# soasme/LTX-Video-GPUPoor

Measured on AMD Instinct MI355X. Metric: denoise-steps/sec + VAE-decode frames/sec, LTX-Video 768x512x97f at 1/8 GPU, higher is better.
Workload: dtype bf16

## Files before the change

### include/ltxmi.h

```cpp
#ifndef LTXMI_H
#define LTXMI_H

#include <stddef.h>
#include <stdint.h>

#ifdef __cplusplus
extern "C" {
#endif

typedef enum ltxmi_status {
    LTXMI_OK = 0,
    LTXMI_ERR_INVALID_ARG = -1,
    LTXMI_ERR_UNSUPPORTED = -2,
    LTXMI_ERR_LAUNCH = -3
} ltxmi_status;

const char* ltxmi_version(void);
const char* ltxmi_last_error(void);
const char* ltxmi_arch(void);

typedef enum ltxmi_epilogue {
    LTXMI_EPI_NONE = 0,
    LTXMI_EPI_GELU_TANH = 1,
    LTXMI_EPI_SILU = 2,
    LTXMI_EPI_GATE_RESIDUAL = 3
} ltxmi_epilogue;

typedef struct ltxmi_gemm_args {
    const void* A;  int64_t lda;
    const void* W;  int64_t ldw;
    const void* bias;
    void*       C;  int64_t ldc;
    int32_t M, N, K;
    int32_t epilogue;
    const void* residual; int64_t ldr;
    const void* gate_table;
    const void* gate_temb;
    int64_t     gate_ld;
    int32_t     rows_per_group;
    int32_t     algo;
    float*      rowsumsq; int32_t rowsumsq_cols; int64_t rowsumsq_ld;
    int32_t     a_kblock; int64_t a_kblock_stride;
} ltxmi_gemm_args;

int ltxmi_gemm_bf16(const ltxmi_gemm_args* args, void* stream);

typedef enum ltxmi_norm_kind { LTXMI_NORM_RMS = 0, LTXMI_NORM_LAYER = 1 } ltxmi_norm_kind;

int ltxmi_norm_modulate_bf16(const void* x, int64_t ldx, void* y, int64_t ldy,
                             int32_t rows, int32_t D, float eps, int32_t kind,
                             const void* scale_table, const void* scale_temb,
                             const void* shift_table, const void* shift_temb,
                             int64_t temb_ld, int32_t rows_per_group, void* stream);

int ltxmi_rmsnorm_rope_bf16(void* x, int64_t ldx, int32_t rows, int32_t D,
                            const void* weight, float eps,
                            const void* cos_tab, const void* sin_tab, int64_t ld_tab,
                            int32_t rope_period, void* stream);
int ltxmi_rmsnorm_rope_rstd_bf16(void* x, int64_t ldx, int32_t rows, int32_t D, const void* weight, float eps,
                                 const void* cos_tab, const void* sin_tab, int64_t ld_tab, int32_t rope_period,
                                 const float* rowsumsq, int64_t rowsumsq_ld, int32_t rowsumsq_blocks,
                                 int32_t norm_dim, float norm_eps, float* rstd_out, void* stream);

typedef struct ltxmi_attn_args {
    const void* q; int64_t q_stride_b, q_stride_l;
    const void* k; int64_t k_stride_b, k_stride_l;
    const void* v; int64_t v_stride_b, v_stride_l;
    void*       o; int64_t o_stride_b, o_stride_l;
    const float* key_bias; int64_t bias_stride_b;
    int32_t B, H, Lq, Lk, head_dim;
    float   softmax_scale;
    const float* q_rowsumsq; int64_t q_rowsumsq_stride_b, q_rowsumsq_stride_l; int32_t q_rowsumsq_blocks;
    const void*  q_norm_weight; float q_norm_eps;
    const void*  rope_cos; const void* rope_sin; int64_t rope_stride_b, rope_stride_l;
    int32_t o_segment_len; int64_t o_stride_segment;
    const float* q_rstd; int64_t q_rstd_stride_b, q_rstd_stride_l;
    uint32_t* redo_counter; int32_t force_exact;
    float* lse; int64_t lse_stride_b, lse_stride_h;
} ltxmi_attn_args;

int ltxmi_attention_fwd_bf16(const ltxmi_attn_args* args, void* stream);
int ltxmi_attention_fuses_qnorm(int32_t B, int32_t H, int32_t Lq, int32_t Lk, int32_t head_dim, int32_t has_key_bias);
int ltxmi_attention_kernel_id(int32_t B, int32_t H, int32_t Lq, int32_t Lk, int32_t head_dim, int32_t has_key_bias,
                              int64_t k_stride_l, int64_t v_stride_l);

#define LTXMI_ATTN_MERGE_MAX 8
typedef struct ltxmi_attn_merge_args {
    int32_t n;
    const void*  o_part[LTXMI_ATTN_MERGE_MAX];   int64_t o_part_stride_b[LTXMI_ATTN_MERGE_MAX], o_part_stride_l[LTXMI_ATTN_MERGE_MAX];
    const float* lse_part[LTXMI_ATTN_MERGE_MAX]; int64_t lse_part_stride_b[LTXMI_ATTN_MERGE_MAX], lse_part_stride_h[LTXMI_ATTN_MERGE_MAX];
    void*  o;   int64_t o_stride_b, o_stride_l;
    float* lse; int64_t lse_stride_b, lse_stride_h;
    int32_t B, H, Lq, head_dim;
} ltxmi_attn_merge_args;
int ltxmi_attention_merge_bf16(const ltxmi_attn_merge_args* args, void* stream);

int ltxmi_rowsumsq_rstd_f32(const float* rowsumsq, int64_t rowsumsq_ld, int32_t rowsumsq_blocks, int32_t rows,
                            int32_t norm_dim, float norm_eps, float* rstd_out, void* stream);

int ltxmi_qkv_norm_rope_pack_bf16(const void* qkv, int64_t ld, int32_t B, int32_t Nl, int32_t D, int32_t P,
                                  const void* q_weight, const void* k_weight, float eps, const void* cos_tab,
                                  const void* sin_tab, int64_t ld_tab, int32_t rope_period, void* out, void* stream);

int ltxmi_silu_bf16(const void* x, void* y, int64_t n, void* stream);
int ltxmi_timestep_embedding_bf16(const float* t, void* out, int32_t n, int32_t dim, void* stream);
int ltxmi_stg_blend_bf16(void* a, int64_t lda, const void* v, int64_t ldv,
                         const float* m, int32_t B, int32_t L, int32_t D, void* stream);
int ltxmi_stg_blend_grouped_bf16(void* a, const void* v, int64_t v_stride_g, int64_t v_stride_b, int64_t v_stride_l,
                                 const float* m, int32_t G, int32_t B, int32_t L, int32_t D, void* stream);

typedef struct ltxmi_conv3d_args {
    const void* x; const void* w; const void* bias; void* y;
    int32_t B, T, H, W, Cin, Cout;
    int32_t causal;
    int32_t pad_replicate;
    int32_t d2s;
    const void* residual;
    int32_t res_channels;
    const void* add;
    int32_t stride_t, stride_hw;
    int32_t tpad, out_T;
    int32_t kernel_t, time_pad_zeros;
    int32_t algo;
    int32_t post_norm;
    const float* post_scale;
    const float* post_shift;
    float post_eps;
    void* y_norm;
    void* workspace; int64_t workspace_bytes;
} ltxmi_conv3d_args;

int ltxmi_conv3d_ndhwc_bf16(const ltxmi_conv3d_args* args, void* stream);
int ltxmi_conv3d_fuses_post_norm(const ltxmi_conv3d_args* args);
int64_t ltxmi_conv3d_workspace_bytes(const ltxmi_conv3d_args* args);

int ltxmi_pixelnorm_ada_silu_bf16(const void* x, void* y, int64_t rows, int32_t C,
                                  int64_t rows_per_batch, const float* scale, const float* shift,
                                  int32_t apply_silu, float eps, void* stream);

int ltxmi_add_bf16(const void* a, const void* b, void* y, int64_t n, void* stream);

int ltxmi_layernorm_affine_bf16(const void* x, void* y, int64_t rows, int32_t C,
                                const void* gamma, const void* beta, float eps, void* stream);

int ltxmi_ncdhw_to_ndhwc_bf16(const void* z, void* y, int32_t B, int32_t C, int32_t T, int32_t H,
                              int32_t W, const float* std, const float* mean, void* stream);
int ltxmi_unpatchify_to_ncdhw_bf16(const void* x, void* y, int32_t B, int32_t T, int32_t H, int32_t W,
                                   int32_t C_out, int32_t patch, void* stream);

int ltxmi_patchify_to_ndhwc_bf16(const void* x, void* y, int32_t B, int32_t C, int32_t T, int32_t H,
                                 int32_t W, int32_t patch, int32_t C_pad, void* stream);
int ltxmi_space_to_depth_skip_bf16(const void* conv, const void* x, void* out, int32_t B, int32_t T,
                                   int32_t H, int32_t W, int32_t Cin, int32_t Cconv, int32_t stride_t,
                                   int32_t stride_hw, int32_t group, void* stream);
int ltxmi_ndhwc_to_ncdhw_bf16(const void* x, int64_t ldx, int32_t c0, void* y, int32_t B, int32_t C,
                              int32_t T, int32_t H, int32_t W, const float* std, const float* mean,
                              void* stream);

#define LTXMI_GUIDANCE_WORKSPACE_FLOATS 2048
int ltxmi_guidance_step_bf16(const void* noise_pred, int64_t n, int32_t num_conds,
                             float guidance_scale, float stg_scale, float rescaling_scale,
                             int32_t do_cfg, int32_t do_stg, int32_t do_rescale,
                             void* latents, int32_t latents_bf16, float dt, float* workspace,
                             void* stream);

int ltxmi_guidance_step_masked_bf16(const void* noise_pred, int64_t n, int32_t num_conds,
                                    float guidance_scale, float stg_scale, float rescaling_scale,
                                    int32_t do_cfg, int32_t do_stg, int32_t do_rescale,
                                    void* latents, int32_t latents_bf16, float dt,
                                    const float* cond_mask, int32_t channels, float t,
                                    float* workspace, void* stream);

int ltxmi_image_cond_noise(void* latents, const void* init_latents, const void* noise, int32_t is_bf16,
                           const float* cond_mask, int64_t tokens, int32_t channels, float noise_scale,
                           float t, void* stream);

int ltxmi_groupnorm_silu_bf16(const void* x, void* y, const void* residual, int32_t samples, int64_t S,
                              int32_t C, int32_t groups, const void* gamma, const void* beta, float eps,
                              float* workspace, void* stream);
int ltxmi_pixel_shuffle2d_ndhwc_bf16(const void* x, void* y, int64_t frames, int32_t H, int32_t W, int32_t C,
                                     void* stream);
int ltxmi_tile_blend(const void* a, void* b, int32_t dtype, int64_t outer, int64_t len_a, int64_t len_b,
                     int64_t inner, int32_t extent, void* stream);
int ltxmi_adain_filter(const void* latents, const void* reference, void* out, int32_t is_bf16, int32_t planes,
                       int64_t n, int64_t n_ref, float factor, void* stream);

#ifdef __cplusplus
}
#endif
#endif
```

### ltx-video-gpupoor_amd/csrc/api.hip

```cpp
#include <stdarg.h>
#include <string.h>

#include "common.h"

namespace ltxmi {

static thread_local char g_err[512] = "";

void set_error(const char* fmt, ...) {
    va_list ap;
    va_start(ap, fmt);
    vsnprintf(g_err, sizeof(g_err), fmt, ap);
    va_end(ap);
}

int check_launch(const char* what) {
    const hipError_t e = hipGetLastError();
    if (e != hipSuccess) {
        set_error("%s: launch failed: %s", what, hipGetErrorString(e));
        return LTXMI_ERR_LAUNCH;
    }
    return LTXMI_OK;
}

int reserve_lds(const void* kernel, int bytes, unsigned long long* done, const char* what) {
    int dev = 0;
    if (hipGetDevice(&dev) != hipSuccess) {
        set_error("%s: cannot query the current device", what);
        return LTXMI_ERR_LAUNCH;
    }
    const bool tracked = dev >= 0 && dev < 64;
    const unsigned long long bit = tracked ? (1ull << dev) : 0ull;
    if (tracked && (__atomic_load_n(done, __ATOMIC_ACQUIRE) & bit)) return LTXMI_OK;
    const hipError_t e = hipFuncSetAttribute(kernel, hipFuncAttributeMaxDynamicSharedMemorySize, bytes);
    if (e != hipSuccess) {
        set_error("%s: cannot reserve %d bytes of LDS: %s", what, bytes, hipGetErrorString(e));
        return LTXMI_ERR_LAUNCH;
    }
    if (tracked) __atomic_fetch_or(done, bit, __ATOMIC_RELEASE);
    return LTXMI_OK;
}

int device_cu_count(const char* what) {
    static int cus[64] = {};
    int dev = 0;
    if (hipGetDevice(&dev) != hipSuccess) {
        set_error("%s: cannot query the current device", what);
        return -1;
    }
    const bool tracked = dev >= 0 && dev < 64;
    if (tracked) {
        const int c = __atomic_load_n(&cus[dev], __ATOMIC_ACQUIRE);
        if (c > 0) return c;
    }
    int n = 0;
    if (hipDeviceGetAttribute(&n, hipDeviceAttributeMultiprocessorCount, dev) != hipSuccess || n <= 0) {
        set_error("%s: cannot query the CU count of device %d", what, dev);
        return -1;
    }
    if (tracked) __atomic_store_n(&cus[dev], n, __ATOMIC_RELEASE);
    return n;
}

}

extern "C" const char* ltxmi_version(void) { return "ltxmi 0.6.0 (round 5)"; }
extern "C" const char* ltxmi_last_error(void) { return ltxmi::g_err; }
extern "C" const char* ltxmi_arch(void) { return "gfx950"; }
```

### ltx-video-gpupoor_amd/csrc/attention.h

```cpp
#pragma once
#include "common.h"

namespace ltxmi {

struct AttnParams {
    const uint16_t* q; int64_t q_sb, q_sl;
    const uint16_t* k; int64_t k_sb, k_sl;
    const uint16_t* v; int64_t v_sb, v_sl;
    uint16_t* o; int64_t o_sb, o_sl;
    const float* bias; int64_t bias_sb;
    int B, H, Lq, Lk;
    float scale_log2e;
    int q_tiles;
    const float* q_ss; int64_t q_ss_sb, q_ss_sl; int q_ss_n;
    const float* q_rstd; int64_t q_rstd_sb, q_rstd_sl;
    const uint16_t* q_w; float q_eps;
    const uint16_t* rope_cos; const uint16_t* rope_sin; int64_t rope_sb, rope_sl;
    int o_seg; int64_t o_sseg;
    uint32_t* redo_count; int force_exact;
    float* lse; int64_t lse_sb, lse_sh;

    __host__ __device__ __forceinline__ bool q_on_load() const { return q_ss != nullptr || q_rstd != nullptr; }
    __device__ __forceinline__ float q_row_rstd(int b, int row, int HD) const {
        if (q_rstd) return q_rstd[(int64_t)b * q_rstd_sb + (int64_t)row * q_rstd_sl];
        const float* ss = q_ss + (int64_t)b * q_ss_sb + (int64_t)row * q_ss_sl;
        float s2 = 0.f;
        if ((q_ss_n & 3) == 0 && (((uintptr_t)ss) & 15) == 0) {
            const f32x4* ss4 = (const f32x4*)ss;
            for (int j = 0; j < (q_ss_n >> 2); ++j) {
                const f32x4 v4 = ss4[j];
                s2 += (v4[0] + v4[1]) + (v4[2] + v4[3]);
            }
        } else {
            for (int j = 0; j < q_ss_n; ++j) s2 += ss[j];
        }
        return rsqrtf(s2 / (float)HD + q_eps);
    }

    __device__ __forceinline__ void store_lse(int b, int head, int row, float m_log2, float l, bool removed) const {
        constexpr float LN2 = 0.6931471805599453f;
        lse[(int64_t)b * lse_sb + (int64_t)head * lse_sh + row] = removed ? -INFINITY : (m_log2 + __log2f(l)) * LN2;
    }

    __device__ __forceinline__ int64_t o_row(int row) const {
        if (o_seg <= 0) return (int64_t)row * o_sl;
        const int sg = row / o_seg;
        return (int64_t)sg * o_sseg + (int64_t)(row - sg * o_seg) * o_sl;
    }
};

enum AttnKernel : int {
    ATTN_DH64 = 0, ATTN_DH64_BIAS = 1, ATTN_DH64_QB2 = 2, ATTN_PIPE = 3,
    ATTN_DH128 = 4, ATTN_DH128_BIAS = 5, ATTN_PIPE128 = 6, ATTN_CROSS = 7,
};
constexpr int ATTN_CROSS_MAX_KEYS = 256;
constexpr float ATTN_BIAS_FLOOR = -1e30f;
constexpr float ATTN_ROW_REMOVED = 0.99f * ATTN_BIAS_FLOOR;

int launch_attn_pipe(AttnParams p, hipStream_t stream);
int launch_attn_pipe128(AttnParams p, hipStream_t stream);
int launch_attn_cross(AttnParams p, hipStream_t stream);

}
```

### ltx-video-gpupoor_amd/csrc/attention.hip

```cpp
#include <type_traits>

#include "attention.h"

namespace ltxmi {

constexpr int KV_TILE = 64;
constexpr int Q_PER_WAVE = 32;
constexpr int Q_PER_WG = 128;
constexpr float LOG2E = 1.4426950408889634f;
constexpr int ATTN_QB_BIG = 2;

template <int DH>
struct AttnCfg {
    static constexpr int ROW_BYTES = DH * 2;
    static constexpr int TILE_BYTES = KV_TILE * DH * 2;
    static constexpr int CHUNKS_PER_ROW = DH / 8;
    static constexpr int LD_PER_THREAD = (KV_TILE * CHUNKS_PER_ROW) / 256;
    static constexpr int KSTEPS = DH / 16;
    static constexpr int DBLK = DH / 32;
    static constexpr int BIAS_BYTES = KV_TILE * 4;
    static constexpr int STAGE_BYTES = 2 * TILE_BYTES + BIAS_BYTES;
    static constexpr int SMEM = 2 * STAGE_BYTES;
    __device__ static __forceinline__ int k_swz(int row) {
        return DH == 64 ? ((row >> 1) & 7) : (row & 15);
    }
};


template <int DH, bool HAS_BIAS, int QB>
__global__ __launch_bounds__(256, (QB == 2 || DH == 128) ? 2 : 1) void attn_fwd_kernel(AttnParams p) {
    using C = AttnCfg<DH>;
    constexpr int QW = Q_PER_WAVE * QB;
    constexpr bool FOLD = !HAS_BIAS && DH == 128;
    extern __shared__ __attribute__((aligned(16))) char smem[];

    const int tid = threadIdx.x;
    const int lane = tid & 63;
    const int wave = __builtin_amdgcn_readfirstlane(tid >> 6);
    const int r = lane & 31;
    const int hh = lane >> 5;

    const int nwg = gridDim.x, orig = blockIdx.x;
    const int xcd = orig & 7, qn = nwg >> 3, rn = nwg & 7;
    const int work = (xcd < rn ? xcd * (qn + 1) : rn * (qn + 1) + (xcd - rn) * qn) + (orig >> 3);
    const int bh = work / p.q_tiles, qt = work % p.q_tiles;
    const int b = bh / p.H, head = bh % p.H;

    const uint16_t* qb = p.q + (int64_t)b * p.q_sb + head * DH;
    const uint16_t* kb_ = p.k + (int64_t)b * p.k_sb + head * DH;
    const uint16_t* vb = p.v + (int64_t)b * p.v_sb + head * DH;
    uint16_t* ob = p.o + (int64_t)b * p.o_sb + head * DH;
    const float* biasb = HAS_BIAS ? p.bias + (int64_t)b * p.bias_sb : nullptr;

    int q_row[QB];
    bf16x8 qf[QB][C::KSTEPS];
#pragma unroll
    for (int i = 0; i < QB; ++i) {
        q_row[i] = qt * (4 * QW) + wave * QW + 32 * i + r;
        const int q_ld = q_row[i] < p.Lq ? q_row[i] : p.Lq - 1;
        const float rstd = p.q_on_load() ? p.q_row_rstd(b, q_ld, p.H * DH) : 0.f;
#pragma unroll
        for (int s = 0; s < C::KSTEPS; ++s) {
            qf[i][s] = *(const bf16x8*)(qb + (int64_t)q_ld * p.q_sl + 16 * s + 8 * hh);
            if (p.q_on_load()) {
                const int col = head * DH + 16 * s + 8 * hh;
                const bf16x8 wv = *(const bf16x8*)(p.q_w + col);
                float o[8];
#pragma unroll
                for (int e = 0; e < 8; ++e) o[e] = (float)qf[i][s][e] * rstd * (float)wv[e];
                if (p.rope_cos) {
                    const int64_t trow = (int64_t)b * p.rope_sb + (int64_t)q_ld * p.rope_sl;
                    const bf16x8 cv = *(const bf16x8*)(p.rope_cos + trow + col), sv = *(const bf16x8*)(p.rope_sin + trow + col);
#pragma unroll
                    for (int e = 0; e < 8; e += 2) {
                        const float r0 = o[e] * (float)cv[e] - o[e + 1] * (float)sv[e];
                        const float r1 = o[e + 1] * (float)cv[e + 1] + o[e] * (float)sv[e + 1];
                        o[e] = r0;
                        o[e + 1] = r1;
                    }
                }
#pragma unroll
                for (int e = 0; e < 8; ++e) qf[i][s][e] = (__bf16)o[e];
            }
            if (FOLD) {
#pragma unroll
                for (int e = 0; e < 8; ++e) qf[i][s][e] = (__bf16)((float)qf[i][s][e] * p.scale_log2e);
            }
        }
    }

    int st_key[C::LD_PER_THREAD], st_koff[C::LD_PER_THREAD], st_voff[C::LD_PER_THREAD], st_col[C::LD_PER_THREAD];
#pragma unroll
    for (int i = 0; i < C::LD_PER_THREAD; ++i) {
        const int c = tid + 256 * i;
        const int key = c / C::CHUNKS_PER_ROW, dc = c % C::CHUNKS_PER_ROW;
        st_key[i] = key;
        st_col[i] = dc * 8;
        st_koff[i] = key * C::ROW_BYTES + ((dc ^ C::k_swz(key)) << 4);
        st_voff[i] = C::TILE_BYTES + ((key >> 3) * C::DBLK + (dc >> 2)) * 512 + (key & 7) * 64 + (dc & 3) * 16;
    }
    u32x4 kreg[C::LD_PER_THREAD], vreg[C::LD_PER_THREAD];
    float breg = 0.f;

    uint32_t k_goff[C::LD_PER_THREAD], v_goff[C::LD_PER_THREAD];
#pragma unroll
    for (int i = 0; i < C::LD_PER_THREAD; ++i) {
        k_goff[i] = (uint32_t)(((int64_t)st_key[i] * p.k_sl + st_col[i]) * 2);
        v_goff[i] = (uint32_t)(((int64_t)st_key[i] * p.v_sl + st_col[i]) * 2);
    }
    auto load_tile = [&](int k0, auto tail_tag) {
        constexpr bool TAIL = decltype(tail_tag)::value;
        if (!TAIL) {
            const char* kt = (const char*)(kb_ + (int64_t)k0 * p.k_sl);
            const char* vt = (const char*)(vb + (int64_t)k0 * p.v_sl);
#pragma unroll
            for (int i = 0; i < C::LD_PER_THREAD; ++i) {
                kreg[i] = *(const u32x4*)(kt + k_goff[i]);
                vreg[i] = *(const u32x4*)(vt + v_goff[i]);
            }
        } else {
#pragma unroll
            for (int i = 0; i < C::LD_PER_THREAD; ++i) {
                int key = k0 + st_key[i];
                key = key < p.Lk ? key : p.Lk - 1;
                kreg[i] = *(const u32x4*)(kb_ + (int64_t)key * p.k_sl + st_col[i]);
                vreg[i] = *(const u32x4*)(vb + (int64_t)key * p.v_sl + st_col[i]);
            }
        }
        if (HAS_BIAS && tid < KV_TILE) {
            const int key = k0 + tid;
            breg = key < p.Lk ? fmaxf(biasb[key] * LOG2E, ATTN_BIAS_FLOOR) : 0.f;
        }
    };
    auto write_tile = [&](int buf) {
        char* s = smem + buf * C::STAGE_BYTES;
#pragma unroll
        for (int i = 0; i < C::LD_PER_THREAD; ++i) {
            *(u32x4*)(s + st_koff[i]) = kreg[i];
            *(u32x4*)(s + st_voff[i]) = vreg[i];
        }
        if (HAS_BIAS && tid < KV_TILE) *(float*)(s + 2 * C::TILE_BYTES + tid * 4) = breg;
    };

    int k_rd[2];
#pragma unroll
    for (int kb = 0; kb < 2; ++kb) k_rd[kb] = (32 * kb + r) * C::ROW_BYTES;
    const int k_sw0 = C::k_swz(r);
    const int g16 = lane >> 4, i16 = lane & 15;
    const int v_rd = C::TILE_BYTES + (4 * (g16 >> 1) + (i16 >> 2)) * 64 + (16 * (g16 & 1) + 4 * (i16 & 3)) * 2;

    f32x16 oT[QB][C::DBLK];
    float m_run[QB];
    f32x4 lT[QB];
    bf16x8 ones;
    {
        const bool on = ((lane & 15) == 0 && ((lane >> 4) & 1) == 0) || ((lane & 15) == 1 && ((lane >> 4) & 1) == 1);
#pragma unroll
        for (int e = 0; e < 8; ++e) ones[e] = on ? (__bf16)1.0f : (__bf16)0.0f;
    }
    bf16x8 kaug, maug[QB];
#pragma unroll
    for (int e = 0; e < 8; ++e) kaug[e] = (hh == 0 && e < 2) ? (__bf16)1.0f : (__bf16)0.0f;
#pragma unroll
    for (int i = 0; i < QB; ++i) {
        m_run[i] = FOLD ? 0.f : -INFINITY;
#pragma unroll
        for (int e = 0; e < 8; ++e) maug[i][e] = (__bf16)0.0f;
        lT[i] = f32x4{0.f, 0.f, 0.f, 0.f};
#pragma unroll
        for (int d = 0; d < C::DBLK; ++d)
#pragma unroll
            for (int e = 0; e < 16; ++e) oT[i][d][e] = 0.f;
    }
    const float c = p.scale_log2e;

    const int nt = (p.Lk + KV_TILE - 1) / KV_TILE;
    const int n_full = p.Lk / KV_TILE;

    auto tile_body = [&](int t, auto tail_tag) {
        constexpr bool TAIL = decltype(tail_tag)::value;
        const int cur = t & 1;
        const char* s = smem + cur * C::STAGE_BYTES;

        f32x16 sT[QB][2];
#pragma unroll
        for (int i = 0; i < QB; ++i)
#pragma unroll
            for (int kb = 0; kb < 2; ++kb) {
#pragma unroll
                for (int e = 0; e < 16; ++e) sT[i][kb][e] = 0.f;
                if (FOLD) sT[i][kb] = __builtin_amdgcn_mfma_f32_32x32x16_bf16(kaug, maug[i], sT[i][kb], 0, 0, 0);
#pragma unroll
                for (int ks = 0; ks < C::KSTEPS; ++ks) {
                    const bf16x8 kf = *(const bf16x8*)(s + k_rd[kb] + (((2 * ks + hh) ^ k_sw0) << 4));
                    sT[i][kb] = __builtin_amdgcn_mfma_f32_32x32x16_bf16(kf, qf[i][ks], sT[i][kb], 0, 0, 0);
                }
            }

#pragma unroll
// ... 20 lines not shown
                        if (key >= p.Lk) sT[i][kb][e] = -INFINITY;
                    }
            }
            float mt;
            {
                auto max3 = [](float a, float b, float c3) { return fmaxf(fmaxf(a, b), c3); };
                float l1[11];
#pragma unroll
                for (int g = 0; g < 5; ++g) {
                    l1[g] = max3(sT[i][0][3 * g], sT[i][0][3 * g + 1], sT[i][0][3 * g + 2]);
                    l1[5 + g] = max3(sT[i][1][3 * g], sT[i][1][3 * g + 1], sT[i][1][3 * g + 2]);
                }
                l1[10] = max3(sT[i][0][15], sT[i][1][15], l1[0]);
                const float a = max3(l1[1], l1[2], l1[3]), b2 = max3(l1[4], l1[5], l1[6]), c2 = max3(l1[7], l1[8], l1[9]);
                mt = fmaxf(max3(a, b2, c2), l1[10]);
            }
            {
                const auto sw = __builtin_amdgcn_permlane32_swap(__float_as_uint(mt), __float_as_uint(mt), false, false);
                mt = fmaxf(__uint_as_float(sw[0]), __uint_as_float(sw[1]));
            }
            float nmoff = 0.f;
            if (FOLD) {
                const bool first = (t == 0);
                if (first || __any(mt > 0.f)) {
                    asm volatile("; max-moved branch (kept a real branch: not if-converted)" ::: "memory");
                    const float dq = (first || mt > 0.f) ? ceilf(mt * 4.0f) * 0.25f : 0.f;
#pragma unroll
                    for (int kb = 0; kb < 2; ++kb)
#pragma unroll
                        for (int e = 0; e < 16; ++e) sT[i][kb][e] -= dq;
                    if (!first) {
                        const float alpha = fast_exp2(-dq);
                        lT[i][0] *= alpha;
                        lT[i][1] *= __shfl(alpha, (lane + 16) & 63, 64);
#pragma unroll
                        for (int d = 0; d < C::DBLK; ++d)
#pragma unroll
                            for (int e = 0; e < 16; ++e) oT[i][d][e] *= alpha;
                    }
                    m_run[i] += dq;
                    const float nm = -m_run[i];
                    const __bf16 mh = (__bf16)nm;
                    const __bf16 ml = (__bf16)(nm - (float)mh);
                    maug[i][0] = hh == 0 ? mh : (__bf16)0.0f;
                    maug[i][1] = hh == 0 ? ml : (__bf16)0.0f;
                }
            } else {
                const float m_new = fmaxf(m_run[i], mt);
                if (__any(m_new != m_run[i])) {
                    asm volatile("; rescale branch (kept a real branch: not if-converted)" ::: "memory");
                    const float alpha = HAS_BIAS ? fast_exp2(m_run[i] - m_new) : fast_exp2((m_run[i] - m_new) * c);
                    lT[i][0] *= alpha;
                    lT[i][1] *= __shfl(alpha, (lane + 16) & 63, 64);
#pragma unroll
                    for (int d = 0; d < C::DBLK; ++d)
#pragma unroll
                        for (int e = 0; e < 16; ++e) oT[i][d][e] *= alpha;
                    m_run[i] = m_new;
                }
                nmoff = HAS_BIAS ? -m_run[i] : -m_run[i] * c;
            }

            bf16x8 pf[4];
#pragma unroll
            for (int kb = 0; kb < 2; ++kb) {
#pragma unroll
                for (int e = 0; e < 16; ++e) {
                    sT[i][kb][e] = fast_exp2(FOLD ? sT[i][kb][e] : (HAS_BIAS ? sT[i][kb][e] + nmoff : __builtin_fmaf(sT[i][kb][e], c, nmoff)));
                }
#pragma unroll
                for (int h2 = 0; h2 < 2; ++h2)
#pragma unroll
                    for (int e = 0; e < 8; ++e) pf[2 * kb + h2][e] = (__bf16)sT[i][kb][8 * h2 + e];
            }

#pragma unroll
            for (int sp = 0; sp < 4; ++sp) {
                lT[i] = __builtin_amdgcn_mfma_f32_16x16x32_bf16(ones, pf[sp], lT[i], 0, 0, 0);
#pragma unroll
                for (int d = 0; d < C::DBLK; ++d) {
                    const char* base = s + v_rd + (2 * sp * C::DBLK + d) * 512;
                    const s16x4 lo = __builtin_amdgcn_ds_read_tr16_b64_v4i16(
                        (__attribute__((address_space(3))) s16x4*)(base));
                    const s16x4 hi = __builtin_amdgcn_ds_read_tr16_b64_v4i16(
                        (__attribute__((address_space(3))) s16x4*)(base + C::DBLK * 512));
                    typedef __attribute__((ext_vector_type(8))) short s16x8;
                    const s16x8 both = __builtin_shufflevector(lo, hi, 0, 1, 2, 3, 4, 5, 6, 7);
                    const bf16x8 vf = __builtin_bit_cast(bf16x8, both);
                    oT[i][d] = __builtin_amdgcn_mfma_f32_32x32x16_bf16(vf, pf[sp], oT[i][d], 0, 0, 0);
                }
            }
        }
    };

    using no_tail = std::integral_constant<bool, false>;
    using with_tail = std::integral_constant<bool, true>;
    if (n_full > 0) load_tile(0, no_tail{}); else load_tile(0, with_tail{});
    write_tile(0);
    __syncthreads();

    for (int t = 0; t < n_full; ++t) {
        const bool has_next = t + 1 < nt;
        if (has_next) {
            if (t + 1 < n_full) load_tile((t + 1) * KV_TILE, no_tail{});
            else load_tile((t + 1) * KV_TILE, with_tail{});
        }
        tile_body(t, no_tail{});
        if (has_next) write_tile((t & 1) ^ 1);
        __syncthreads();
    }
    if (n_full < nt) tile_body(n_full, with_tail{});

#pragma unroll
    for (int i = 0; i < QB; ++i) {
        const float l0 = __shfl(lT[i][0], r & 15, 64), l1 = __shfl(lT[i][1], r & 15, 64);
        const float l = (r & 16) ? l1 : l0;
        const float inv = 1.0f / l;
        if (p.lse != nullptr) {
            const float m2 = (HAS_BIAS || FOLD) ? m_run[i] : m_run[i] * c;
            if (hh == 0 && q_row[i] < p.Lq) p.store_lse(b, head, q_row[i], m2, l, HAS_BIAS && m_run[i] <= ATTN_ROW_REMOVED);
        }
        char* scr = smem + wave * (32 * C::ROW_BYTES);
        if (i == 0) __syncthreads();
#pragma unroll
        for (int d = 0; d < C::DBLK; ++d)
#pragma unroll
            for (int g = 0; g < 4; ++g) {
                u32x2 w;
                w[0] = pack_bf16(oT[i][d][4 * g + 0] * inv, oT[i][d][4 * g + 1] * inv);
                w[1] = pack_bf16(oT[i][d][4 * g + 2] * inv, oT[i][d][4 * g + 3] * inv);
                const int chunk = 4 * d + g;
                *(u32x2*)(scr + r * C::ROW_BYTES + ((chunk ^ (r & 7)) << 4) + hh * 8) = w;
            }
        constexpr int LPR = C::CHUNKS_PER_ROW;
        constexpr int RPI = 64 / LPR;
        const int q0 = qt * (4 * QW) + wave * QW + 32 * i;
#pragma unroll
        for (int t = 0; t < 32 / RPI; ++t) {
            const int row = t * RPI + lane / LPR, chunk = lane % LPR;
            const u32x4 w = *(const u32x4*)(scr + row * C::ROW_BYTES + ((chunk ^ (row & 7)) << 4));
            if (q0 + row < p.Lq) *(u32x4*)(ob + p.o_row(q0 + row) + chunk * 8) = w;
        }
    }
}

template <int DH, bool HAS_BIAS, int QB>
static int launch(AttnParams p, hipStream_t stream) {
    using C = AttnCfg<DH>;
    auto kern = attn_fwd_kernel<DH, HAS_BIAS, QB>;
    static unsigned long long lds_done = 0;
    if (const int rc = reserve_lds((const void*)kern, C::SMEM, &lds_done, "ltxmi_attention_fwd_bf16")) return rc;
    const int q_per_wg = Q_PER_WG * QB;
    p.q_tiles = (p.Lq + q_per_wg - 1) / q_per_wg;
    const int64_t grid = (int64_t)p.B * p.H * p.q_tiles;
    hipLaunchKernelGGL(kern, dim3((unsigned)grid), dim3(256), C::SMEM, stream, p);
    return check_launch("ltxmi_attention_fwd_bf16");
}

static AttnKernel attn_select(int B, int H, int Lq, int Lk, int head_dim, bool has_bias, int64_t k_sl, int64_t v_sl) {
    const int64_t wg256 = (int64_t)B * H * ((Lq + 255) / 256);
    const int64_t rows = (int64_t)Lk + 4 * 64;
    const bool span_ok = (rows * k_sl + head_dim) * 2 < (1ll << 31) && (rows * v_sl + head_dim) * 2 < (1ll << 31);
    if (head_dim == 128) {
        if (!has_bias && wg256 >= 128 && Lk >= 1024 && span_ok) return ATTN_PIPE128;
        return has_bias ? ATTN_DH128_BIAS : ATTN_DH128;
    }
    if (Lk <= ATTN_CROSS_MAX_KEYS && Lq >= 1024) return ATTN_CROSS;
    if (!has_bias && wg256 >= 192 && span_ok) return ATTN_PIPE;
    if (!has_bias && wg256 >= 512) return ATTN_DH64_QB2;
    return has_bias ? ATTN_DH64_BIAS : ATTN_DH64;
}

}

using namespace ltxmi;

extern "C" int ltxmi_attention_fwd_bf16(const ltxmi_attn_args* a, void* stream) {
    LTXMI_REQUIRE(a && a->q && a->k && a->v && a->o, LTXMI_ERR_INVALID_ARG, "ltxmi_attention_fwd_bf16: NULL argument");
    LTXMI_REQUIRE(a->B > 0 && a->H > 0 && a->Lq > 0 && a->Lk > 0, LTXMI_ERR_INVALID_ARG,
                  "ltxmi_attention_fwd_bf16: non-positive shape B=%d H=%d Lq=%d Lk=%d", a->B, a->H, a->Lq, a->Lk);
    LTXMI_REQUIRE(a->head_dim == 64 || a->head_dim == 128, LTXMI_ERR_UNSUPPORTED,
                  "ltxmi_attention_fwd_bf16: head_dim %d not in {64, 128}", a->head_dim);
    const int64_t strides[] = {a->q_stride_b, a->q_stride_l, a->k_stride_b, a->k_stride_l,
                               a->v_stride_b, a->v_stride_l, a->o_stride_b, a->o_stride_l};
    for (int64_t s : strides)
        LTXMI_REQUIRE(s % 8 == 0, LTXMI_ERR_UNSUPPORTED, "ltxmi_attention_fwd_bf16: strides must be multiples of 8 elements");
    LTXMI_REQUIRE((((uintptr_t)a->q | (uintptr_t)a->k | (uintptr_t)a->v | (uintptr_t)a->o) & 15) == 0,
                  LTXMI_ERR_UNSUPPORTED, "ltxmi_attention_fwd_bf16: q/k/v/o must be 16-byte aligned");
    LTXMI_REQUIRE((int64_t)a->B * a->H * ((a->Lq + Q_PER_WG - 1) / Q_PER_WG) < (1ll << 31), LTXMI_ERR_UNSUPPORTED,
                  "ltxmi_attention_fwd_bf16: grid too large");
    AttnParams p;
    p.q = (const uint16_t*)a->q; p.q_sb = a->q_stride_b; p.q_sl = a->q_stride_l;
    p.k = (const uint16_t*)a->k; p.k_sb = a->k_stride_b; p.k_sl = a->k_stride_l;
    p.v = (const uint16_t*)a->v; p.v_sb = a->v_stride_b; p.v_sl = a->v_stride_l;
    p.o = (uint16_t*)a->o; p.o_sb = a->o_stride_b; p.o_sl = a->o_stride_l;
    p.bias = a->key_bias; p.bias_sb = a->bias_stride_b;
    p.B = a->B; p.H = a->H; p.Lq = a->Lq; p.Lk = a->Lk;
    p.scale_log2e = a->softmax_scale * LOG2E;
    p.q_tiles = (a->Lq + Q_PER_WG - 1) / Q_PER_WG;
    p.q_ss = a->q_rowsumsq; p.q_ss_sb = a->q_rowsumsq_stride_b; p.q_ss_sl = a->q_rowsumsq_stride_l;
    p.q_ss_n = a->q_rowsumsq_blocks;
    p.q_rstd = a->q_rstd; p.q_rstd_sb = a->q_rstd_stride_b; p.q_rstd_sl = a->q_rstd_stride_l;
    p.q_w = (const uint16_t*)a->q_norm_weight; p.q_eps = a->q_norm_eps;
    p.rope_cos = (const uint16_t*)a->rope_cos; p.rope_sin = (const uint16_t*)a->rope_sin;
    p.rope_sb = a->rope_stride_b; p.rope_sl = a->rope_stride_l;
    p.o_seg = a->o_segment_len; p.o_sseg = a->o_stride_segment;
    p.redo_count = a->redo_counter; p.force_exact = a->force_exact != 0;
    LTXMI_REQUIRE(a->o_segment_len >= 0 && a->o_stride_segment % 8 == 0, LTXMI_ERR_INVALID_ARG,
                  "ltxmi_attention_fwd_bf16: bad output segment geometry");
    p.lse = a->lse; p.lse_sb = a->lse_stride_b; p.lse_sh = a->lse_stride_h;
    if (a->lse)
        LTXMI_REQUIRE((((uintptr_t)a->lse) & 3) == 0 && a->lse_stride_h >= a->Lq &&
                          (a->B == 1 ? a->lse_stride_b >= 0 : a->lse_stride_b >= (int64_t)a->H * a->lse_stride_h),
                      LTXMI_ERR_INVALID_ARG,
                      "ltxmi_attention_fwd_bf16: lse must be 4-byte aligned with lse_stride_h >= Lq and lse_stride_b >= H * lse_stride_h");
    if (a->q_rowsumsq || a->q_rstd) {
        LTXMI_REQUIRE(a->q_norm_weight && (((uintptr_t)a->q_norm_weight) & 15) == 0 &&
                          (a->q_rstd ? (((uintptr_t)a->q_rstd) & 3) == 0
                                     : (a->q_rowsumsq_blocks == a->H * a->head_dim / 64 && (((uintptr_t)a->q_rowsumsq) & 3) == 0)),
                      LTXMI_ERR_INVALID_ARG, "ltxmi_attention_fwd_bf16: bad q_rowsumsq / q_rstd / q_norm_weight geometry");
        LTXMI_REQUIRE((a->rope_cos == nullptr) == (a->rope_sin == nullptr), LTXMI_ERR_INVALID_ARG,
                      "ltxmi_attention_fwd_bf16: rope_cos and rope_sin must both be given or both be NULL");
        if (a->rope_cos)
            LTXMI_REQUIRE((((uintptr_t)a->rope_cos | (uintptr_t)a->rope_sin) & 15) == 0 && a->rope_stride_l % 8 == 0 &&
                              a->rope_stride_b % 8 == 0,
                          LTXMI_ERR_INVALID_ARG, "ltxmi_attention_fwd_bf16: RoPE tables must be 16-byte aligned rows");
    }
    hipStream_t s = (hipStream_t)stream;
    switch (attn_select(a->B, a->H, a->Lq, a->Lk, a->head_dim, a->key_bias != nullptr, a->k_stride_l, a->v_stride_l)) {
        case ATTN_DH64: return launch<64, false, 1>(p, s);
        case ATTN_DH64_BIAS: return launch<64, true, 1>(p, s);
        case ATTN_DH64_QB2: return launch<64, false, ATTN_QB_BIG>(p, s);
        case ATTN_PIPE: return launch_attn_pipe(p, s);
        case ATTN_DH128: return launch<128, false, 1>(p, s);
        case ATTN_DH128_BIAS: return launch<128, true, 1>(p, s);
        case ATTN_PIPE128: return launch_attn_pipe128(p, s);
        case ATTN_CROSS: return launch_attn_cross(p, s);
    }
}

extern "C" int ltxmi_attention_kernel_id(int32_t B, int32_t H, int32_t Lq, int32_t Lk, int32_t head_dim, int32_t has_key_bias,
                                         int64_t k_stride_l, int64_t v_stride_l) {
    if (B <= 0 || H <= 0 || Lq <= 0 || Lk <= 0 || k_stride_l <= 0 || v_stride_l <= 0) return -1;
    if (head_dim != 64 && head_dim != 128) return -1;
    return attn_select(B, H, Lq, Lk, head_dim, has_key_bias != 0, k_stride_l, v_stride_l);
}

extern "C" int ltxmi_attention_fuses_qnorm(int32_t B, int32_t H, int32_t Lq, int32_t Lk, int32_t head_dim, int32_t has_key_bias) {
    return (B > 0 && H > 0 && Lq > 0 && Lk > 0 && (head_dim == 64 || head_dim == 128) && (H * head_dim) % 64 == 0) ? 1 : 0;
}
```

### ltx-video-gpupoor_amd/csrc/attention_cross.hip

```cpp
#include <type_traits>

#include "attention.h"

namespace ltxmi {

namespace cross {

#ifndef LTXMI_XATTN_STAGGER
#define LTXMI_XATTN_STAGGER 32
#endif

constexpr int DH = 64;
constexpr int KV_TILE = 64;
constexpr int MAX_TILES = 4;
constexpr int ROW_BYTES = DH * 2;
constexpr int TILE_BYTES = KV_TILE * DH * 2;
constexpr int K_OFF = 0, V_OFF = MAX_TILES * TILE_BYTES, BIAS_OFF = 2 * MAX_TILES * TILE_BYTES;
constexpr int SCR_OFF = BIAS_OFF + MAX_TILES * KV_TILE * 16;
constexpr int SCR_BYTES = 32 * 64;
constexpr int QW_OFF = SCR_OFF + 4 * SCR_BYTES;
constexpr int SMEM = QW_OFF + DH * 2;
constexpr int ROWS_PER_IT = 128;
constexpr float LOG2E = 1.4426950408889634f;

__device__ __forceinline__ int k_swz(int row) { return (row >> 1) & 7; }

template <int NT>
__global__ __launch_bounds__(256, 2) void attn_cross_kernel(AttnParams p, int groups, int rows_per_group, int stagger_from) {
    extern __shared__ __attribute__((aligned(16))) char smem[];
    const int tid = threadIdx.x;
    const int lane = tid & 63;
    const int wave = __builtin_amdgcn_readfirstlane(tid >> 6);
    const int r = lane & 31, hh = lane >> 5;

    const int nwg = gridDim.x, orig = blockIdx.x;
    const int xcd = orig & 7, qn = nwg >> 3, rn = nwg & 7;
    const int work = (xcd < rn ? xcd * (qn + 1) : rn * (qn + 1) + (xcd - rn) * qn) + (orig >> 3);
    const int bh = work / groups, grp = work % groups;
    const int b = bh / p.H, head = bh % p.H;
    const int row_begin = grp * rows_per_group;
    const int row_end = min(p.Lq, row_begin + rows_per_group);
    if (row_begin >= row_end) return;
    const int n_it = (row_end - row_begin + ROWS_PER_IT - 1) / ROWS_PER_IT;

    const uint16_t* qb = p.q + (int64_t)b * p.q_sb + head * DH;
    const uint16_t* kb_ = p.k + (int64_t)b * p.k_sb + head * DH;
    const uint16_t* vb = p.v + (int64_t)b * p.v_sb + head * DH;
    uint16_t* ob = p.o + (int64_t)b * p.o_sb + head * DH;
    constexpr int nt = NT;

    {
        u32x4 kreg[NT][2], vreg[NT][2];
#pragma unroll
        for (int t = 0; t < NT; ++t) {
#pragma unroll
                for (int i = 0; i < 2; ++i) {
                    const int c = tid + 256 * i;
                    int key = t * KV_TILE + (c >> 3);
                    key = key < p.Lk ? key : p.Lk - 1;
                    kreg[t][i] = *(const u32x4*)(kb_ + (int64_t)key * p.k_sl + (c & 7) * 8);
                    vreg[t][i] = *(const u32x4*)(vb + (int64_t)key * p.v_sl + (c & 7) * 8);
                }
            }
        if (tid < MAX_TILES * KV_TILE) {
            float bv = ATTN_BIAS_FLOOR;
            if (tid < p.Lk) bv = p.bias ? fmaxf(p.bias[(int64_t)b * p.bias_sb + tid] * (LOG2E / p.scale_log2e), ATTN_BIAS_FLOOR) : 0.f;
            const __bf16 hi = (__bf16)bv;
            const __bf16 lo = (__bf16)(bv - (float)hi);
            u32x4 w = {0u, 0u, 0u, 0u};
            w[0] = (uint32_t)__builtin_bit_cast(uint16_t, hi) | ((uint32_t)__builtin_bit_cast(uint16_t, lo) << 16);
            *(u32x4*)(smem + BIAS_OFF + tid * 16) = w;
        }
#pragma unroll
        for (int t = 0; t < NT; ++t) {
#pragma unroll
                for (int i = 0; i < 2; ++i) {
                    const int c = tid + 256 * i;
                    const int key = c >> 3, dc = c & 7;
                    *(u32x4*)(smem + K_OFF + t * TILE_BYTES + key * ROW_BYTES + ((dc ^ k_swz(key)) << 4)) = kreg[t][i];
                    *(u32x4*)(smem + V_OFF + t * TILE_BYTES + ((key >> 3) * 2 + (dc >> 2)) * 512 + (key & 7) * 64 + (dc & 3) * 16) = vreg[t][i];
                }
            }
    }
    if (p.q_on_load() && tid < 8) *(u32x4*)(smem + QW_OFF + tid * 16) = *(const u32x4*)(p.q_w + head * DH + tid * 8);
    __syncthreads();

    const int k_rd0 = r * ROW_BYTES, k_rd1 = (32 + r) * ROW_BYTES;
    const int k_sw0 = k_swz(r);
    const int g16 = lane >> 4, i16 = lane & 15;
    const int v_rd = (4 * (g16 >> 1) + (i16 >> 2)) * 64 + (16 * (g16 & 1) + 4 * (i16 & 3)) * 2;
    bf16x8 ones;
    {
        const bool on = ((lane & 15) == 0 && ((lane >> 4) & 1) == 0) || ((lane & 15) == 1 && ((lane >> 4) & 1) == 1);
#pragma unroll
        for (int e = 0; e < 8; ++e) ones[e] = on ? (__bf16)1.0f : (__bf16)0.0f;
    }
    const float c = p.scale_log2e;
    char* scr = smem + SCR_OFF + wave * SCR_BYTES;

    bf16x8 qraw[4], qf[4];
    float q_rstd = 0.f;
    int q_ld = 0;
    auto load_q = [&](int it) {
        const int row = row_begin + it * ROWS_PER_IT + wave * 32 + r;
        q_ld = row < p.Lq ? row : p.Lq - 1;
#pragma unroll
        for (int s = 0; s < 4; ++s) qraw[s] = *(const bf16x8*)(qb + (int64_t)q_ld * p.q_sl + 16 * s + 8 * hh);
        if (p.q_on_load()) q_rstd = p.q_row_rstd(b, q_ld, p.H * DH);
    };
    auto finish_q = [&]() {
        if (p.q_on_load()) {
            const int64_t trow = (int64_t)b * p.rope_sb + (int64_t)q_ld * p.rope_sl;
#pragma unroll
            for (int s = 0; s < 4; ++s) {
                const bf16x8 wv = *(const bf16x8*)(smem + QW_OFF + (16 * s + 8 * hh) * 2);
                float o[8];
#pragma unroll
                for (int e = 0; e < 8; ++e) o[e] = (float)qraw[s][e] * q_rstd * (float)wv[e];
                if (p.rope_cos) {
                    const int col = head * DH + 16 * s + 8 * hh;
                    const bf16x8 cv = *(const bf16x8*)(p.rope_cos + trow + col), sv = *(const bf16x8*)(p.rope_sin + trow + col);
#pragma unroll
                    for (int e = 0; e < 8; e += 2) {
                        const float r0 = o[e] * (float)cv[e] - o[e + 1] * (float)sv[e];
                        const float r1 = o[e + 1] * (float)cv[e + 1] + o[e] * (float)sv[e + 1];
                        o[e] = r0;
                        o[e + 1] = r1;
                    }
                }
#pragma unroll
                for (int e = 0; e < 8; ++e) qf[s][e] = (__bf16)o[e];
            }
        } else {
#pragma unroll
            for (int s = 0; s < 4; ++s) qf[s] = qraw[s];
        }
    };
    load_q(0);
    finish_q();
    if (n_it > 1) load_q(1);
    if (blockIdx.x >= (unsigned)stagger_from) __builtin_amdgcn_s_sleep(LTXMI_XATTN_STAGGER);

    for (int it = 0; it < n_it; ++it) {
        const int q0 = row_begin + it * ROWS_PER_IT + wave * 32;

        constexpr int NG = 2 * NT;
        f32x16 sT[NG];
        bf16x8 kfr[5];
        bf16x8 qaug;
        {
            uint32_t w0 = hh == 0 ? 0x3f803f80u : 0u, w1 = 0u;
            asm volatile("" : "+v"(w0), "+v"(w1));
            const u32x4 w = {w0, w1, w1, w1};
            qaug = __builtin_bit_cast(bf16x8, w);
        }
        auto read_k1 = [&](int g, int j) {
            if (j == 0) {
                kfr[0] = *(const bf16x8*)(smem + BIAS_OFF + (32 * g + r) * 16);
            } else {
                const char* ks = smem + K_OFF + (g >> 1) * TILE_BYTES + ((g & 1) ? k_rd1 : k_rd0);
                kfr[j] = *(const bf16x8*)(ks + (((2 * (j - 1) + hh) ^ k_sw0) << 4));
            }
        };
        auto max3 = [](float a, float b2, float c3) { return fmaxf(fmaxf(a, b2), c3); };
        float mt = -INFINITY;
        auto group_max = [&](int g) {
            const f32x16& x = sT[g];
            const float a = max3(x[0], x[1], x[2]), b2 = max3(x[3], x[4], x[5]), c2 = max3(x[6], x[7], x[8]);
            const float d2 = max3(x[9], x[10], x[11]), e2 = max3(x[12], x[13], x[14]);
            mt = max3(max3(a, b2, c2), max3(d2, e2, x[15]), mt);
            asm volatile("" : "+v"(mt));
        };
#pragma unroll
        for (int j = 0; j < 5; ++j) read_k1(0, j);
#pragma unroll
        for (int g = 0; g < NG; ++g) {
#pragma unroll
            for (int j = 0; j < 5; ++j) {
                if (j == 0) {
                    const f32x16 z16 = {0.f, 0.f, 0.f, 0.f, 0.f, 0.f, 0.f, 0.f, 0.f, 0.f, 0.f, 0.f, 0.f, 0.f, 0.f, 0.f};
                    sT[g] = __builtin_amdgcn_mfma_f32_32x32x16_bf16(kfr[0], qaug, z16, 0, 0, 0);
                } else {
                    sT[g] = __builtin_amdgcn_mfma_f32_32x32x16_bf16(kfr[j], qf[j - 1], sT[g], 0, 0, 0);
                }
                if (g + 1 < NG) read_k1(g + 1, j);
                __builtin_amdgcn_sched_barrier(0);
            }
            if (g >= 1) group_max(g - 1);
        }
        if (it + 1 < n_it) finish_q();
        if (it + 2 < n_it) load_q(it + 2);
        group_max(NG - 1);
        {
            const auto sw = __builtin_amdgcn_permlane32_swap(__float_as_uint(mt), __float_as_uint(mt), false, false);
            mt = fmaxf(__uint_as_float(sw[0]), __uint_as_float(sw[1]));
        }
        const float nmc = -mt * c;

        f32x16 oT[2];
        f32x4 lT;
        const f32x16 z16 = {0.f, 0.f, 0.f, 0.f, 0.f, 0.f, 0.f, 0.f, 0.f, 0.f, 0.f, 0.f, 0.f, 0.f, 0.f, 0.f};
        const f32x4 z4 = {0.f, 0.f, 0.f, 0.f};
        typedef __attribute__((ext_vector_type(8))) short s16x8;
        auto read_v = [&](int t, int sp, bf16x8 (&dst)[2]) {
            const char* vs = smem + V_OFF + t * TILE_BYTES + v_rd;
#pragma unroll
            for (int d = 0; d < 2; ++d) {
                const char* base = vs + (2 * sp * 2 + d) * 512;
                const s16x4 lo = __builtin_amdgcn_ds_read_tr16_b64_v4i16((__attribute__((address_space(3))) s16x4*)(base));
                const s16x4 hi = __builtin_amdgcn_ds_read_tr16_b64_v4i16((__attribute__((address_space(3))) s16x4*)(base + 2 * 512));
                const s16x8 both = __builtin_shufflevector(lo, hi, 0, 1, 2, 3, 4, 5, 6, 7);
                dst[d] = __builtin_bit_cast(bf16x8, both);
            }
        };
        auto make_p = [&](int t, int sp2, bf16x8& dst) {
            const f32x16& x = sT[2 * t + (sp2 >> 1)];
            const f32x2 c2v = {c, c}, m2v = {nmc, nmc};
#pragma unroll
            for (int e = 0; e < 8; e += 2) {
                const f32x2 y = f32x2{x[8 * (sp2 & 1) + e], x[8 * (sp2 & 1) + e + 1]} * c2v + m2v;
                dst[e] = (__bf16)fast_exp2(y[0]);
                dst[e + 1] = (__bf16)fast_exp2(y[1]);
            }
            asm volatile("" : "+v"(dst));
        };
        bf16x8 pfr[2][4], vfr[2][2];
#pragma unroll
        for (int sp = 0; sp < 4; ++sp) make_p(0, sp, pfr[0][sp]);
        read_v(0, 0, vfr[0]);
#pragma unroll
        for (int t = 0; t < NT; ++t) {
#pragma unroll
            for (int sp = 0; sp < 4; ++sp) {
                const int st = 4 * t + sp;
                if (st + 1 < 4 * NT) read_v((st + 1) >> 2, (st + 1) & 3, vfr[(st + 1) & 1]);
                const bf16x8& pf = pfr[t & 1][sp];
                lT = __builtin_amdgcn_mfma_f32_16x16x32_bf16(ones, pf, st == 0 ? z4 : lT, 0, 0, 0);
                oT[0] = __builtin_amdgcn_mfma_f32_32x32x16_bf16(vfr[st & 1][0], pf, st == 0 ? z16 : oT[0], 0, 0, 0);
                oT[1] = __builtin_amdgcn_mfma_f32_32x32x16_bf16(vfr[st & 1][1], pf, st == 0 ? z16 : oT[1], 0, 0, 0);
                if (t + 1 < NT) make_p(t + 1, sp, pfr[(t + 1) & 1][sp]);
                __builtin_amdgcn_sched_barrier(0);
            }
        }

        const float l0 = __shfl(lT[0], r & 15, 64), l1v = __shfl(lT[1], r & 15, 64);
        const float lrow = (r & 16) ? l1v : l0;
        const float inv = 1.0f / lrow;
        if (p.lse != nullptr) {
            if (hh == 0 && q0 + r < row_end) p.store_lse(b, head, q0 + r, -nmc, lrow, -nmc / c <= ATTN_ROW_REMOVED);
        }
#pragma unroll
        for (int d = 0; d < 2; ++d) {
#pragma unroll
            for (int g = 0; g < 4; ++g) {
                u32x2 w;
                w[0] = pack_bf16(oT[d][4 * g + 0] * inv, oT[d][4 * g + 1] * inv);
                w[1] = pack_bf16(oT[d][4 * g + 2] * inv, oT[d][4 * g + 3] * inv);
                *(u32x2*)(scr + r * 64 + ((g ^ (r & 3)) << 4) + hh * 8) = w;
            }
#pragma unroll
            for (int t2 = 0; t2 < 2; ++t2) {
                const int row = t2 * 16 + (lane >> 2), chunk = lane & 3;
                const u32x4 w = *(const u32x4*)(scr + row * 64 + ((chunk ^ (row & 3)) << 4));
                if (q0 + row < row_end) *(u32x4*)(ob + p.o_row(q0 + row) + 32 * d + chunk * 8) = w;
            }
        }
    }
}

}

static_assert(cross::MAX_TILES * cross::KV_TILE == ATTN_CROSS_MAX_KEYS, "attn_select hands this kernel up to ATTN_CROSS_MAX_KEYS keys");

int launch_attn_cross(AttnParams p, hipStream_t stream) {
    const int n_cu = device_cu_count("ltxmi_attention_fwd_bf16");
    if (n_cu <= 0) return LTXMI_ERR_LAUNCH;
    const int slots = 2 * n_cu, bh = p.B * p.H;
    int groups = slots / bh;
    if (groups < 1) groups = 1;
    const int max_groups = (p.Lq + 2 * cross::ROWS_PER_IT - 1) / (2 * cross::ROWS_PER_IT);
    if (groups > max_groups) groups = max_groups;
    int rows = (p.Lq + groups - 1) / groups;
    rows = (rows + cross::ROWS_PER_IT - 1) / cross::ROWS_PER_IT * cross::ROWS_PER_IT;
    groups = (p.Lq + rows - 1) / rows;
    const int64_t grid = (int64_t)bh * groups;
    const int nt = (p.Lk + cross::KV_TILE - 1) / cross::KV_TILE;
#define LTXMI_XATTN_LAUNCH(N)                                                                                              \
    {                                                                                                                      \
        static unsigned long long lds_done = 0;                                                                            \
        if (const int rc = reserve_lds((const void*)cross::attn_cross_kernel<N>, cross::SMEM, &lds_done,                   \
                                       "ltxmi_attention_fwd_bf16"))                                                        \
            return rc;                                                                                                     \
        hipLaunchKernelGGL(cross::attn_cross_kernel<N>, dim3((unsigned)grid), dim3(256), cross::SMEM, stream, p, groups,   \
                           rows, n_cu);                                                                                    \
    }
    switch (nt) {
        case 1: LTXMI_XATTN_LAUNCH(1) break;
        case 2: LTXMI_XATTN_LAUNCH(2) break;
        case 3: LTXMI_XATTN_LAUNCH(3) break;
        default: LTXMI_XATTN_LAUNCH(4) break;
    }
#undef LTXMI_XATTN_LAUNCH
    return check_launch("ltxmi_attention_fwd_bf16");
}

}
```

### ltx-video-gpupoor_amd/csrc/attention_pipe.hip

```cpp
#include <type_traits>

#include "attention.h"

namespace ltxmi {

namespace pipe {

#ifdef LTXMI_ATTN_STAMPS
#define STAMP(i)                                                                               \
    do {                                                                                       \
        unsigned long long t_;                                                                 \
        __builtin_amdgcn_sched_barrier(0);                                                     \
        asm volatile("s_memtime %0\n\ts_waitcnt lgkmcnt(0)" : "=s"(t_)::"memory");             \
        __builtin_amdgcn_sched_barrier(0);                                                     \
        st.acc[i] += t_ - st.prev;                                                             \
        st.prev = t_;                                                                          \
    } while (0)
struct Stamps { unsigned long long prev; unsigned long long acc[8]; };
__device__ unsigned long long* g_attn_stamps = nullptr;
#else
#define STAMP(i) do { } while (0)
struct Stamps {};
#endif

constexpr int DH = 64;
constexpr int KV_TILE = 64;
constexpr int ROW_BYTES = DH * 2;
constexpr int TILE_BYTES = KV_TILE * DH * 2;
constexpr int RING = 4;
constexpr int SMEM = 2 * RING * TILE_BYTES;
constexpr int Q_PER_WG = 256;

struct Blk {
    f32x16 s[2];
    f32x16 o[2];
    u32x4 pf[4];
    bf16x8 q[4];
    f32x4 l;
    float m;
};

struct Lane {
    int lane, r, hh;
    int k_rd[2];
    int k_sw0;
    int v_rd;
};

__device__ __forceinline__ bf16x8 k_fragment(const char* slot, const Lane& L, int j) {
    return *(const bf16x8*)(slot + L.k_rd[j >> 2] + (((2 * (j & 3) + L.hh) ^ L.k_sw0) << 4));
}

template <bool STEADY, bool QSCALED, typename Hook>
__device__ __forceinline__ void segment(Blk& X, Blk& Y, bf16x8 (&kf)[8], const char* ks_next, const char* vs, const Lane& L,
                                        const bf16x8& ones, float c, int key0, int Lk, Stamps& st, int st0, Hook&& hook) {
#pragma unroll
    for (int sp = 0; sp < 4; ++sp) Y.l = __builtin_amdgcn_mfma_f32_16x16x32_bf16(ones, __builtin_bit_cast(bf16x8, Y.pf[sp]), Y.l, 0, 0, 0);

    if (key0 + KV_TILE > Lk) {
        asm volatile("; ragged key tile (a wave-uniform branch, not a template instance)" ::: "memory");
#pragma unroll
        for (int kb = 0; kb < 2; ++kb)
#pragma unroll
            for (int e = 0; e < 16; ++e) {
                const int key = key0 + 32 * kb + (e & 3) + 8 * (e >> 2) + 4 * L.hh;
                if (key >= Lk) X.s[kb][e] = -INFINITY;
            }
    }
    if (!STEADY) {
        float mt;
        {
            auto max3 = [](float a, float b, float c3) { return fmaxf(fmaxf(a, b), c3); };
            float l1[11];
#pragma unroll
            for (int g = 0; g < 5; ++g) {
                l1[g] = max3(X.s[0][3 * g], X.s[0][3 * g + 1], X.s[0][3 * g + 2]);
                l1[5 + g] = max3(X.s[1][3 * g], X.s[1][3 * g + 1], X.s[1][3 * g + 2]);
            }
            l1[10] = max3(X.s[0][15], X.s[1][15], l1[0]);
            const float a = max3(l1[1], l1[2], l1[3]), b2 = max3(l1[4], l1[5], l1[6]), c2 = max3(l1[7], l1[8], l1[9]);
            mt = fmaxf(max3(a, b2, c2), l1[10]);
            const auto sw = __builtin_amdgcn_permlane32_swap(__float_as_uint(mt), __float_as_uint(mt), false, false);
            mt = fmaxf(__uint_as_float(sw[0]), __uint_as_float(sw[1]));
        }
        const float m_new = fmaxf(X.m, mt);
        if (__any(m_new != X.m)) {
            asm volatile("; rescale branch (kept a real branch: not if-converted)" ::: "memory");
            const float alpha = fast_exp2(QSCALED ? X.m - m_new : (X.m - m_new) * c);
            X.l[0] *= alpha;
            X.l[1] *= __shfl(alpha, (L.lane + 16) & 63, 64);
#pragma unroll
            for (int d = 0; d < 2; ++d)
#pragma unroll
                for (int e = 0; e < 16; ++e) X.o[d][e] *= alpha;
            X.m = m_new;
        }
    }
    const float nmoff = STEADY ? 0.f : QSCALED ? -X.m : -X.m * c;
    __builtin_amdgcn_sched_barrier(0);
    STAMP(st0);

    bf16x8 vf[8];
    float pp0 = 0.f, pp1 = 0.f;
    typedef __attribute__((ext_vector_type(8))) short s16x8;
#pragma unroll
    for (int j = 0; j < 16; ++j) {
        if (j < 8) {
            const int kb = j >> 2, s = j & 3;
            if (s == 0) {
#pragma unroll
                for (int e = 0; e < 16; ++e) Y.s[kb][e] = 0.f;
            }
            Y.s[kb] = __builtin_amdgcn_mfma_f32_32x32x16_bf16(kf[j], Y.q[s], Y.s[kb], 0, 0, 0);
            const char* base = vs + L.v_rd + (2 * (j >> 1) * 2 + (j & 1)) * 512;
            const s16x4 lo = __builtin_amdgcn_ds_read_tr16_b64_v4i16((__attribute__((address_space(3))) s16x4*)(base));
            const s16x4 hi = __builtin_amdgcn_ds_read_tr16_b64_v4i16((__attribute__((address_space(3))) s16x4*)(base + 2 * 512));
            const s16x8 both = __builtin_shufflevector(lo, hi, 0, 1, 2, 3, 4, 5, 6, 7);
            vf[j] = __builtin_bit_cast(bf16x8, both);
        } else {
            const int jj = j - 8, sp = jj >> 1, d = jj & 1;
            Y.o[d] = __builtin_amdgcn_mfma_f32_32x32x16_bf16(vf[jj], __builtin_bit_cast(bf16x8, Y.pf[sp]), Y.o[d], 0, 0, 0);
            kf[jj] = k_fragment(ks_next, L, jj);
        }
        hook(j);
        const int kb = j >> 3, e0 = 2 * (j & 7);
        auto bits = [&](float sc) { return QSCALED ? (STEADY ? sc : sc + nmoff) : (STEADY ? sc * c : __builtin_fmaf(sc, c, nmoff)); };
        const float p0 = fast_exp2(bits(X.s[kb][e0]));
        const float p1 = fast_exp2(bits(X.s[kb][e0 + 1]));
        if (j > 0) {
            const int jp = j - 1, kbp = jp >> 3, ep = 2 * (jp & 7);
            uint32_t pw = pack_bf16(pp0, pp1);
            asm volatile("" : "+v"(pw));
            X.pf[2 * kbp + (ep >> 3)][(ep & 7) >> 1] = pw;
        }
        pp0 = p0;
        pp1 = p1;
        __builtin_amdgcn_sched_barrier(0);
    }
    X.pf[3][3] = pack_bf16(pp0, pp1);
    STAMP(st0 + 1);
}

template <bool REDO, bool QSCALED>
__device__ __forceinline__ bool attn_pipe_item(const AttnParams& p, const int tid, char* smem) {
    char* kring = smem;
    char* vring = smem + RING * TILE_BYTES;

    Lane L;
    L.lane = tid & 63;
    const int wave = __builtin_amdgcn_readfirstlane(tid >> 6);
    L.r = L.lane & 31;
    L.hh = L.lane >> 5;

    const int nwg = gridDim.x, orig = blockIdx.x;
    const int xcd = orig & 7, qn = nwg >> 3, rn = nwg & 7;
    const int work = (xcd < rn ? xcd * (qn + 1) : rn * (qn + 1) + (xcd - rn) * qn) + (orig >> 3);
    const int bh = work / p.q_tiles, qt = work % p.q_tiles;
    const int b = bh / p.H, head = bh % p.H;

    const uint16_t* qb = p.q + (int64_t)b * p.q_sb + head * DH;
    const uint16_t* kb_ = p.k + (int64_t)b * p.k_sb + head * DH;
    const uint16_t* vb = p.v + (int64_t)b * p.v_sb + head * DH;
    uint16_t* ob = p.o + (int64_t)b * p.o_sb + head * DH;

    auto make_desc = [](const void* base, int64_t bytes) {
        const uint64_t a = (uint64_t)base;
        return u32x4{(uint32_t)a, (uint32_t)(a >> 32) & 0xffffu, (uint32_t)bytes, 0x00020000u};
    };
    const u32x4 k_desc = make_desc(kb_, ((int64_t)(p.Lk - 1) * p.k_sl + DH) * 2);
    const u32x4 v_desc = make_desc(vb, ((int64_t)(p.Lk - 1) * p.v_sl + DH) * 2);
    uint32_t k_voff[2], v_voff[2];
#pragma unroll
    for (int j = 0; j < 2; ++j) {
        const int piece = 2 * wave + j;
        const int krow = 8 * piece + (L.lane >> 3);
        const int kchunk = (L.lane & 7) ^ ((krow >> 1) & 7);
        k_voff[j] = (uint32_t)((krow * (int)p.k_sl + 8 * kchunk) * 2);
        const int vrow = 8 * piece + ((L.lane >> 2) & 7);
        const int vchunk = 4 * (L.lane >> 5) + (L.lane & 3);
        v_voff[j] = (uint32_t)((vrow * (int)p.v_sl + 8 * vchunk) * 2);
    }
    const uint32_t k_tile_step = (uint32_t)(KV_TILE * (int)p.k_sl * 2), v_tile_step = (uint32_t)(KV_TILE * (int)p.v_sl * 2);
    const uint32_t lds0 = (uint32_t)(uintptr_t)((__attribute__((address_space(3))) char*)smem);
    auto dma2 = [&](const u32x4& desc, uint32_t lds_addr, uint32_t voff0, uint32_t voff1) {
        uint32_t keep;
        asm volatile(
            "s_mov_b32 %0, m0\n\t"
            "s_mov_b32 m0, %3\n\t"
            "s_nop 0\n\t"
            "buffer_load_dwordx4 %1, %4, 0 offen lds\n\t"
            "s_add_u32 m0, m0, 0x400\n\t"
            "s_nop 0\n\t"
            "buffer_load_dwordx4 %2, %4, 0 offen lds\n\t"
            "s_mov_b32 m0, %0"
            : "=&s"(keep)
            : "v"(voff0), "v"(voff1), "s"(lds_addr), "s"(desc)
            : "memory", "scc");
    };
    auto dma1 = [&](const u32x4& desc, uint32_t lds_addr, uint32_t voff) {
        uint32_t keep;
        asm volatile(
            "s_mov_b32 %0, m0\n\t"
            "s_mov_b32 m0, %2\n\t"
            "s_nop 0\n\t"
            "buffer_load_dwordx4 %1, %3, 0 offen lds\n\t"
            "s_mov_b32 m0, %0"
            : "=&s"(keep)
            : "v"(voff), "s"(lds_addr), "s"(desc)
            : "memory");
    };
    auto dma_k1 = [&](int t, int i) {
        const uint32_t dst = lds0 + (uint32_t)((t & (RING - 1)) * TILE_BYTES + (2 * wave + i) * 1024);
        dma1(k_desc, dst, k_voff[i] + (uint32_t)t * k_tile_step);
    };
    auto dma_v1 = [&](int t, int i) {
        const uint32_t dst = lds0 + (uint32_t)((RING + (t & (RING - 1))) * TILE_BYTES + (2 * wave + i) * 1024);
        dma1(v_desc, dst, v_voff[i] + (uint32_t)t * v_tile_step);
    };
    auto dma_k = [&](int t) {
        const uint32_t dst = lds0 + (uint32_t)((t & (RING - 1)) * TILE_BYTES + 2 * wave * 1024);
        const uint32_t toff = (uint32_t)t * k_tile_step;
        dma2(k_desc, dst, k_voff[0] + toff, k_voff[1] + toff);
    };
    auto dma_v = [&](int t) {
        const uint32_t dst = lds0 + (uint32_t)((RING + (t & (RING - 1))) * TILE_BYTES + 2 * wave * 1024);
        const uint32_t toff = (uint32_t)t * v_tile_step;
        dma2(v_desc, dst, v_voff[0] + toff, v_voff[1] + toff);
    };

    const int nt = (p.Lk + KV_TILE - 1) / KV_TILE;

    L.k_rd[0] = L.r * ROW_BYTES;
    L.k_rd[1] = (32 + L.r) * ROW_BYTES;
    L.k_sw0 = (L.r >> 1) & 7;
    {
        const int g16 = L.lane >> 4, i16 = L.lane & 15;
        L.v_rd = (4 * (g16 >> 1) + (i16 >> 2)) * 64 + (16 * (g16 & 1) + 4 * (i16 & 3)) * 2;
    }

    Blk A, Bk;
    bf16x8 ones;
    {
        const bool on = ((L.lane & 15) == 0 && ((L.lane >> 4) & 1) == 0) || ((L.lane & 15) == 1 && ((L.lane >> 4) & 1) == 1);
#pragma unroll
        for (int e = 0; e < 8; ++e) ones[e] = on ? (__bf16)1.0f : (__bf16)0.0f;
    }
    const float c = p.scale_log2e;
    auto init = [&](Blk& X, int blk) {
        const int row = qt * Q_PER_WG + wave * 64 + 32 * blk + L.r;
        const int q_ld = row < p.Lq ? row : p.Lq - 1;
#pragma unroll
        for (int s = 0; s < 4; ++s) X.q[s] = *(const bf16x8*)(qb + (int64_t)q_ld * p.q_sl + 16 * s + 8 * L.hh);
        if (QSCALED) {
            const float rstd = p.q_row_rstd(b, q_ld, p.H * DH);
            const int64_t trow = (int64_t)b * p.rope_sb + (int64_t)q_ld * p.rope_sl;
#pragma unroll
            for (int s = 0; s < 4; ++s) {
                const int col = head * DH + 16 * s + 8 * L.hh;
                const bf16x8 wv = *(const bf16x8*)(p.q_w + col);
                float o[8];
#pragma unroll
                for (int e = 0; e < 8; ++e) o[e] = (float)X.q[s][e] * rstd * (float)wv[e];
                if (p.rope_cos) {
                    const bf16x8 cv = *(const bf16x8*)(p.rope_cos + trow + col), sv = *(const bf16x8*)(p.rope_sin + trow + col);
#pragma unroll
                    for (int e = 0; e < 8; e += 2) {
                        const float r0 = o[e] * (float)cv[e] - o[e + 1] * (float)sv[e];
                        const float r1 = o[e + 1] * (float)cv[e + 1] + o[e] * (float)sv[e + 1];
                        o[e] = r0;
                        o[e + 1] = r1;
                    }
                }
#pragma unroll
                for (int e = 0; e < 8; ++e) X.q[s][e] = (__bf16)(QSCALED ? o[e] * c : o[e]);
            }
        }
        X.m = -INFINITY;
        X.l = f32x4{0.f, 0.f, 0.f, 0.f};
#pragma unroll
        for (int i = 0; i < 4; ++i) X.pf[i] = u32x4{0u, 0u, 0u, 0u};
#pragma unroll
        for (int d = 0; d < 2; ++d)
#pragma unroll
            for (int e = 0; e < 16; ++e) { X.o[d][e] = 0.f; X.s[d][e] = 0.f; }
    };
    volatile int* redo_flag = (volatile int*)(smem + SMEM);
    if (!REDO && tid == 0) *redo_flag = 0;
    const bool wave_idle = qt * Q_PER_WG + wave * 64 >= p.Lq;
    if ((blockIdx.x >> 8) & 1) __builtin_amdgcn_s_setprio(1);
    Stamps st;
#ifdef LTXMI_ATTN_STAMPS
    unsigned long long rt0_ = 0;
#endif
    dma_k(0); dma_v(0); dma_k(1); dma_v(1); dma_k(2);
    init(A, 0);
    init(Bk, 1);
    {
        const u32x4 z = {0u, 0u, 0u, 0u};
        *(u32x4*)(vring + 3 * TILE_BYTES + tid * 32) = z;
        *(u32x4*)(vring + 3 * TILE_BYTES + tid * 32 + 16) = z;
    }
    __builtin_amdgcn_s_waitcnt(0x0070);
    __builtin_amdgcn_s_barrier();
    __builtin_amdgcn_sched_barrier(0);

#ifdef LTXMI_ATTN_STAMPS
    for (int i = 0; i < 8; ++i) st.acc[i] = 0;
    { unsigned long long t0_; asm volatile("s_memtime %0\n\ts_waitcnt lgkmcnt(0)" : "=s"(t0_)::"memory"); st.prev = t0_; }
    asm volatile("s_memrealtime %0\n\ts_waitcnt lgkmcnt(0)" : "=s"(rt0_)::"memory");
#endif
    const int t_exact = REDO ? nt : 0;
// ... 7 lines not shown
    } else {
        bf16x8 kf[8];
#pragma unroll
        for (int j = 0; j < 8; ++j) kf[j] = k_fragment(kring, L, j);
#pragma unroll
        for (int j = 0; j < 8; ++j) A.s[j >> 2] = __builtin_amdgcn_mfma_f32_32x32x16_bf16(kf[j], A.q[j & 3], A.s[j >> 2], 0, 0, 0);

        using exact_form = std::integral_constant<bool, false>;
        using steady_form = std::integral_constant<bool, true>;
        auto iteration = [&](int t, auto steady_tag) {
            constexpr bool STEADY = decltype(steady_tag)::value;
            __builtin_amdgcn_s_barrier();
            __builtin_amdgcn_sched_barrier(0);
            STAMP(0);
            STAMP(1);
            segment<STEADY, QSCALED>(A, Bk, kf, kring + ((t + 1) & 3) * TILE_BYTES, vring + ((t + 3) & 3) * TILE_BYTES, L, ones, c, t * KV_TILE, p.Lk, st, 2,
                          [&](int j) { if (j == 3) dma_k1(t + 3, 0); else if (j == 11) dma_k1(t + 3, 1); });
            segment<STEADY, QSCALED>(Bk, A, kf, kring + ((t + 1) & 3) * TILE_BYTES, vring + (t & 3) * TILE_BYTES, L, ones, c, t * KV_TILE, p.Lk, st, 4,
                          [&](int j) { if (j == 3) dma_v1(t + 2, 0); else if (j == 11) dma_v1(t + 2, 1); });
            asm volatile("s_waitcnt vmcnt(4)" ::: "memory");
            __builtin_amdgcn_sched_barrier(0);
            STAMP(6);
        };
        int t = 0;
        for (; t < t_exact; ++t) iteration(t, exact_form{});
        if (!REDO)
            for (; t < nt; ++t) iteration(t, steady_form{});
    }

#ifdef LTXMI_ATTN_STAMPS
    unsigned long long rt1_;
    asm volatile("s_memrealtime %0\n\ts_waitcnt lgkmcnt(0)" : "=s"(rt1_)::"memory");
    if (g_attn_stamps && L.lane == 0 && blockIdx.x < 4096 && !wave_idle) {
        for (int i = 0; i < 7; ++i) g_attn_stamps[(blockIdx.x * 4 + wave) * 8 + i] = st.acc[i];
        g_attn_stamps[(blockIdx.x * 4 + wave) * 8 + 7] = (unsigned long long)nt | ((rt1_ - rt0_) << 32);
    }
#endif
    if (!wave_idle) {
        const char* vs = vring + ((nt - 1) & 3) * TILE_BYTES;
#pragma unroll
        for (int sp = 0; sp < 4; ++sp) Bk.l = __builtin_amdgcn_mfma_f32_16x16x32_bf16(ones, __builtin_bit_cast(bf16x8, Bk.pf[sp]), Bk.l, 0, 0, 0);
        typedef __attribute__((ext_vector_type(8))) short s16x8;
#pragma unroll
        for (int sp = 0; sp < 4; ++sp)
#pragma unroll
            for (int d = 0; d < 2; ++d) {
                const char* base = vs + L.v_rd + (2 * sp * 2 + d) * 512;
                const s16x4 lo = __builtin_amdgcn_ds_read_tr16_b64_v4i16((__attribute__((address_space(3))) s16x4*)(base));
                const s16x4 hi = __builtin_amdgcn_ds_read_tr16_b64_v4i16((__attribute__((address_space(3))) s16x4*)(base + 2 * 512));
                const s16x8 both = __builtin_shufflevector(lo, hi, 0, 1, 2, 3, 4, 5, 6, 7);
                Bk.o[d] = __builtin_amdgcn_mfma_f32_32x32x16_bf16(__builtin_bit_cast(bf16x8, both), __builtin_bit_cast(bf16x8, Bk.pf[sp]), Bk.o[d], 0, 0, 0);
            }
    }
    asm volatile("s_waitcnt vmcnt(0) lgkmcnt(0)" ::: "memory");
    if (!REDO) {
    bool outgrown = false;
    if (t_exact < nt && !wave_idle) {
        constexpr uint32_t OUTGROWN_EXP = (127u + 100u) << 23, VANISHED_EXP = (127u - 100u) << 23;
        uint32_t worst = 0;
        auto scan = [&](const Blk& X) {
            worst |= (uint32_t)((__float_as_uint(X.l[0]) & 0x7f800000u) >= OUTGROWN_EXP);
            worst |= (uint32_t)((__float_as_uint(X.l[1]) & 0x7f800000u) >= OUTGROWN_EXP);
            if (L.lane < 16) {
                worst |= (uint32_t)((__float_as_uint(X.l[0]) & 0x7f800000u) < VANISHED_EXP);
                worst |= (uint32_t)((__float_as_uint(X.l[1]) & 0x7f800000u) < VANISHED_EXP);
            }
#pragma unroll
            for (int d = 0; d < 2; ++d)
#pragma unroll
                for (int e = 0; e < 16; ++e) worst |= (uint32_t)((__float_as_uint(X.o[d][e]) & 0x7f800000u) >= OUTGROWN_EXP);
        };
        scan(A);
        scan(Bk);
        outgrown = __any(worst != 0);
    }
    if (outgrown && L.lane == 0) *redo_flag = 1;
    __builtin_amdgcn_s_barrier();
    __builtin_amdgcn_sched_barrier(0);
    const int redo = *redo_flag;
    __builtin_amdgcn_s_barrier();
    if (redo != 0) return true;
    } else {
        __builtin_amdgcn_s_barrier();
        __builtin_amdgcn_sched_barrier(0);
    }

    auto store = [&](Blk& X, int blk) {
        const float l0 = __shfl(X.l[0], L.r & 15, 64), l1 = __shfl(X.l[1], L.r & 15, 64);
        const float lrow = (L.r & 16) ? l1 : l0;
        const float inv = 1.0f / lrow;
        if (p.lse != nullptr) {
            const int row = qt * Q_PER_WG + wave * 64 + 32 * blk + L.r;
            if (L.hh == 0 && row < p.Lq) p.store_lse(b, head, row, REDO ? (QSCALED ? X.m : X.m * c) : 0.f, lrow, false);
        }
        char* scr = smem + (wave * 2 + blk) * (32 * ROW_BYTES);
#pragma unroll
        for (int d = 0; d < 2; ++d)
#pragma unroll
            for (int g = 0; g < 4; ++g) {
                u32x2 w;
                w[0] = pack_bf16(X.o[d][4 * g + 0] * inv, X.o[d][4 * g + 1] * inv);
                w[1] = pack_bf16(X.o[d][4 * g + 2] * inv, X.o[d][4 * g + 3] * inv);
                const int chunk = 4 * d + g;
                *(u32x2*)(scr + L.r * ROW_BYTES + ((chunk ^ (L.r & 7)) << 4) + L.hh * 8) = w;
            }
        const int q0 = qt * Q_PER_WG + wave * 64 + 32 * blk;
#pragma unroll
        for (int t = 0; t < 4; ++t) {
            const int row = t * 8 + (L.lane >> 3), chunk = L.lane & 7;
            const u32x4 w = *(const u32x4*)(scr + row * ROW_BYTES + ((chunk ^ (row & 7)) << 4));
            if (q0 + row < p.Lq) *(u32x4*)(ob + p.o_row(q0 + row) + chunk * 8) = w;
        }
    };
    store(A, 0);
    store(Bk, 1);
    return false;
}

template <int OCC, bool QSCALED, bool FORCE_EXACT>
__global__ __launch_bounds__(256, OCC) void attn_pipe_kernel(AttnParams p) {
    extern __shared__ __attribute__((aligned(16))) char smem[];
    const int tid = threadIdx.x;
    if (FORCE_EXACT) {
        attn_pipe_item<true, QSCALED>(p, tid, smem);
        return;
    }
    if (!attn_pipe_item<false, QSCALED>(p, tid, smem)) return;
    int tid2 = tid;
    asm volatile("" : "+v"(tid2));
    if (p.redo_count != nullptr && tid2 == 0) atomicAdd(p.redo_count, 1u);
    attn_pipe_item<true, QSCALED>(p, tid2, smem);
}

}

#ifdef LTXMI_ATTN_STAMPS
extern "C" int ltxmi_debug_set_attn_stamps(void* buf) {
    unsigned long long* b = (unsigned long long*)buf;
    return (int)hipMemcpyToSymbol(HIP_SYMBOL(pipe::g_attn_stamps), &b, sizeof(b));
}
#endif

#ifndef LTXMI_ATTN_PIPE_OCC
#define LTXMI_ATTN_PIPE_OCC 2
#endif

int launch_attn_pipe(AttnParams p, hipStream_t stream) {
    const bool qscaled = p.q_on_load();
    auto kern = p.force_exact ? (qscaled ? pipe::attn_pipe_kernel<LTXMI_ATTN_PIPE_OCC, true, true> : pipe::attn_pipe_kernel<LTXMI_ATTN_PIPE_OCC, false, true>)
                              : (qscaled ? pipe::attn_pipe_kernel<LTXMI_ATTN_PIPE_OCC, true, false> : pipe::attn_pipe_kernel<LTXMI_ATTN_PIPE_OCC, false, false>);
    static unsigned long long lds_done[4] = {0, 0, 0, 0};
    if (const int rc = reserve_lds((const void*)kern, pipe::SMEM + 16, &lds_done[(p.force_exact ? 2 : 0) + qscaled], "ltxmi_attention_fwd_bf16")) return rc;
    p.q_tiles = (p.Lq + pipe::Q_PER_WG - 1) / pipe::Q_PER_WG;
    const int64_t grid = (int64_t)p.B * p.H * p.q_tiles;
    hipLaunchKernelGGL(kern, dim3((unsigned)grid), dim3(256), pipe::SMEM + 16, stream, p);
    return check_launch("ltxmi_attention_fwd_bf16");
}

}
```

### ltx-video-gpupoor_amd/csrc/attention_pipe128.hip

```cpp
#include <type_traits>

#include "attention.h"

namespace ltxmi {

namespace pipe128 {

constexpr int DH = 128;
constexpr int KV_TILE = 64;
constexpr int ROW_BYTES = DH * 2;
constexpr int TILE_BYTES = KV_TILE * DH * 2;
constexpr int RING = 4;
constexpr int SMEM = 2 * RING * TILE_BYTES;
constexpr int Q_PER_WG = 256;
constexpr int NS = DH / 16;
constexpr int ND = DH / 32;
constexpr int NCH = 2 * NS + 4 * ND;
constexpr int PIECES = TILE_BYTES / 1024 / 4;

struct Blk {
    f32x16 s[2];
    f32x16 o[ND];
    u32x4 pf[4];
    bf16x8 q[NS];
    f32x4 l;
    float m;
    float mt;
};

struct Lane {
    int lane, r, hh;
    int koff[8];
    int v_rd;
};

__device__ __forceinline__ bf16x8 kread(const char* slot, const Lane& L, int i) {
    return *(const bf16x8*)(slot + L.koff[i & 7] + (i >> 3) * (32 * ROW_BYTES));
}
__device__ __forceinline__ bf16x8 vread(const char* slot, const Lane& L, int i) {
    typedef __attribute__((ext_vector_type(8))) short s16x8;
    const char* base = slot + L.v_rd + ((2 * (i >> 2)) * 4 + (i & 3)) * 512;
    const s16x4 lo = __builtin_amdgcn_ds_read_tr16_b64_v4i16((__attribute__((address_space(3))) s16x4*)(base));
    const s16x4 hi = __builtin_amdgcn_ds_read_tr16_b64_v4i16((__attribute__((address_space(3))) s16x4*)(base + 4 * 512));
    const s16x8 both = __builtin_shufflevector(lo, hi, 0, 1, 2, 3, 4, 5, 6, 7);
    return __builtin_bit_cast(bf16x8, both);
}

__device__ __forceinline__ void mfma_s0(f32x16& acc, const bf16x8& k, const bf16x8& q) {
    asm("v_mfma_f32_32x32x16_bf16 %0, %1, %2, 0" : "=&v"(acc) : "v"(k), "a"(q));
}
__device__ __forceinline__ void mfma_s(f32x16& acc, const bf16x8& k, const bf16x8& q) {
    asm("v_mfma_f32_32x32x16_bf16 %0, %1, %2, %0" : "+v"(acc) : "v"(k), "a"(q));
}
__device__ __forceinline__ void mfma_o(f32x16& acc, const bf16x8& vt, const bf16x8& pt) {
    asm("v_mfma_f32_32x32x16_bf16 %0, %1, %2, %0" : "+a"(acc) : "v"(vt), "v"(pt));
}
template <int N>
__device__ __forceinline__ void settle_o(f32x16 (&o)[N]) {
    static_assert(N == 4, "four O^T blocks");
    asm volatile("s_nop 15\n\ts_nop 7" : "+a"(o[0]), "+a"(o[1]), "+a"(o[2]), "+a"(o[3]));
}
template <bool EXACT, typename Hook>
__device__ __forceinline__ void segment(Blk& X, Blk& Y, bf16x8 (&kq)[4], const char* ks_cur, const char* ks_next, const char* vs,
                                        const Lane& L, const bf16x8& ones, float c, int key0_y, int Lk, Hook&& hook) {
    if (EXACT) {
        const float m_new = fmaxf(X.m, X.mt);
        if (__any(m_new != X.m)) {
            asm volatile("; rescale branch (kept a real branch: not if-converted)" ::: "memory");
            const float alpha = fast_exp2((X.m - m_new) * c);
            X.l[0] *= alpha;
            X.l[1] *= __shfl(alpha, (L.lane + 16) & 63, 64);
            settle_o(X.o);
#pragma unroll
            for (int d = 0; d < ND; ++d)
#pragma unroll
                for (int e = 0; e < 16; ++e) X.o[d][e] *= alpha;
            X.m = m_new;
        }
    }
    const float nmoff = -X.m * c;
    __builtin_amdgcn_sched_barrier(0);

    bf16x8 f[NCH];
#pragma unroll
    for (int i = 0; i < 4; ++i) f[i] = kq[i];
    float pa = 0.f, pb = 0.f;
    float mt = -INFINITY;
#pragma unroll
    for (int j = 0; j < NCH; ++j) {
        if (j < 2 * NS) {
            const int kb = j / NS, s = j % NS;
            if (s == 0) mfma_s0(Y.s[kb], f[j], Y.q[s]);
            else mfma_s(Y.s[kb], f[j], Y.q[s]);
        } else {
            const int jj = j - 2 * NS, sp = jj / ND, d = jj % ND;
            mfma_o(Y.o[d], f[j], __builtin_bit_cast(bf16x8, Y.pf[sp]));
        }
        {
            const int cn = j + 4;
            if (cn < 2 * NS) f[cn] = kread(ks_cur, L, cn);
            else if (cn < NCH) f[cn] = vread(vs, L, cn - 2 * NS);
            else kq[cn - NCH] = kread(ks_next, L, cn - NCH);
        }
        if (j == 1) Y.l = __builtin_amdgcn_mfma_f32_16x16x32_bf16(ones, __builtin_bit_cast(bf16x8, Y.pf[3]), Y.l, 0, 0, 0);
        if (j == 9 || j == 17 || j == 25)
            X.l = __builtin_amdgcn_mfma_f32_16x16x32_bf16(ones, __builtin_bit_cast(bf16x8, X.pf[(j - 9) >> 3]), X.l, 0, 0, 0);
        hook(j);
        const float p = fast_exp2(__builtin_fmaf(X.s[j >> 4][j & 15], c, nmoff));
        if ((j & 1) == 0) {
            if (j >= 2) {
                const int jp = j / 2 - 1;
                uint32_t pw = pack_bf16(pa, pb);
                asm volatile("" : "+v"(pw));
                X.pf[2 * (jp >> 3) + ((jp & 7) >> 2)][jp & 3] = pw;
            }
            pa = p;
        } else {
            pb = p;
        }
        if (j >= 2 * NS) {
            const int jm = j - 2 * NS, kbm = jm >> 3, em = 2 * (jm & 7);
            if (em == 0 && key0_y + KV_TILE > Lk) {
                asm volatile("; ragged key tile (kept a real branch)" ::: "memory");
#pragma unroll
                for (int e = 0; e < 16; ++e) {
                    const int key = key0_y + 32 * kbm + (e & 3) + 8 * (e >> 2) + 4 * L.hh;
                    if (key >= Lk) Y.s[kbm][e] = -INFINITY;
                }
            }
            if (EXACT) {
                mt = fmaxf(fmaxf(mt, Y.s[kbm][em]), Y.s[kbm][em + 1]);
                asm volatile("" : "+v"(mt));
            }
        }
        __builtin_amdgcn_sched_barrier(0);
    }
    X.pf[3][3] = pack_bf16(pa, pb);
    if (EXACT) {
        const auto sw = __builtin_amdgcn_permlane32_swap(__float_as_uint(mt), __float_as_uint(mt), false, false);
        Y.mt = fmaxf(__uint_as_float(sw[0]), __uint_as_float(sw[1]));
    }
}

__global__ __launch_bounds__(256, 1) void attn_pipe128_kernel(AttnParams p) {
    extern __shared__ __attribute__((aligned(16))) char smem[];
    char* kring = smem;
    char* vring = smem + RING * TILE_BYTES;

    const int tid = threadIdx.x;
    Lane L;
    L.lane = tid & 63;
    const int wave = __builtin_amdgcn_readfirstlane(tid >> 6);
    L.r = L.lane & 31;
    L.hh = L.lane >> 5;

    const int nwg = gridDim.x, orig = blockIdx.x;
    const int xcd = orig & 7, qn = nwg >> 3, rn = nwg & 7;
    const int work = (xcd < rn ? xcd * (qn + 1) : rn * (qn + 1) + (xcd - rn) * qn) + (orig >> 3);
    const int bh = work / p.q_tiles, qt = work % p.q_tiles;
    const int b = bh / p.H, head = bh % p.H;

    const uint16_t* qb = p.q + (int64_t)b * p.q_sb + head * DH;
    const uint16_t* kb_ = p.k + (int64_t)b * p.k_sb + head * DH;
    const uint16_t* vb = p.v + (int64_t)b * p.v_sb + head * DH;
    uint16_t* ob = p.o + (int64_t)b * p.o_sb + head * DH;

    auto make_desc = [](const void* base, int64_t bytes) {
        const uint64_t a = (uint64_t)base;
        return u32x4{(uint32_t)a, (uint32_t)(a >> 32) & 0xffffu, (uint32_t)bytes, 0x00020000u};
    };
    const u32x4 k_desc = make_desc(kb_, ((int64_t)(p.Lk - 1) * p.k_sl + DH) * 2);
    const u32x4 v_desc = make_desc(vb, ((int64_t)(p.Lk - 1) * p.v_sl + DH) * 2);
    uint32_t k_voff[PIECES], v_voff[PIECES];
#pragma unroll
    for (int j = 0; j < PIECES; ++j) {
        const int piece = PIECES * wave + j;
        const int krow = 4 * piece + (L.lane >> 4);
        const int kchunk = (L.lane & 15) ^ (krow & 15);
        k_voff[j] = (uint32_t)((krow * (int)p.k_sl + 8 * kchunk) * 2);
        const int vrow = 8 * (piece >> 1) + ((L.lane >> 2) & 7);
        const int vchunk = 8 * (piece & 1) + 4 * (L.lane >> 5) + (L.lane & 3);
        v_voff[j] = (uint32_t)((vrow * (int)p.v_sl + 8 * vchunk) * 2);
    }
    const uint32_t k_tile_step = (uint32_t)(KV_TILE * (int)p.k_sl * 2), v_tile_step = (uint32_t)(KV_TILE * (int)p.v_sl * 2);
    const uint32_t lds0 = (uint32_t)(uintptr_t)((__attribute__((address_space(3))) char*)smem);
    auto dma1 = [&](const u32x4& desc, uint32_t lds_addr, uint32_t voff) {
        uint32_t keep;
        asm volatile(
            "s_mov_b32 %0, m0\n\t"
            "s_mov_b32 m0, %2\n\t"
            "s_nop 0\n\t"
            "buffer_load_dwordx4 %1, %3, 0 offen lds\n\t"
            "s_mov_b32 m0, %0"
            : "=&s"(keep)
            : "v"(voff), "s"(lds_addr), "s"(desc)
            : "memory");
    };
    auto dma_k1 = [&](int t, int i) {
        const uint32_t dst = lds0 + (uint32_t)((t & (RING - 1)) * TILE_BYTES + (PIECES * wave + i) * 1024);
        dma1(k_desc, dst, k_voff[i] + (uint32_t)t * k_tile_step);
    };
    auto dma_v1 = [&](int t, int i) {
        const uint32_t dst = lds0 + (uint32_t)((RING + (t & (RING - 1))) * TILE_BYTES + (PIECES * wave + i) * 1024);
        dma1(v_desc, dst, v_voff[i] + (uint32_t)t * v_tile_step);
    };
    auto dma_k = [&](int t) {
#pragma unroll
        for (int i = 0; i < PIECES; ++i) dma_k1(t, i);
    };
    auto dma_v = [&](int t) {
#pragma unroll
        for (int i = 0; i < PIECES; ++i) dma_v1(t, i);
    };

    const int nt = (p.Lk + KV_TILE - 1) / KV_TILE;
#pragma unroll
    for (int s8 = 0; s8 < 8; ++s8) L.koff[s8] = L.r * ROW_BYTES + (((2 * s8 + L.hh) ^ (L.r & 15)) << 4);
    {
        const int g16 = L.lane >> 4, i16 = L.lane & 15;
        L.v_rd = (4 * (g16 >> 1) + (i16 >> 2)) * 64 + (16 * (g16 & 1) + 4 * (i16 & 3)) * 2;
    }

    Blk A, Bk;
    bf16x8 ones;
    {
        const bool on = ((L.lane & 15) == 0 && ((L.lane >> 4) & 1) == 0) || ((L.lane & 15) == 1 && ((L.lane >> 4) & 1) == 1);
#pragma unroll
        for (int e = 0; e < 8; ++e) ones[e] = on ? (__bf16)1.0f : (__bf16)0.0f;
    }
    auto init = [&](Blk& X, int blk) {
        const int row = qt * Q_PER_WG + wave * 64 + 32 * blk + L.r;
        const int q_ld = row < p.Lq ? row : p.Lq - 1;
#pragma unroll
        for (int s = 0; s < NS; ++s) X.q[s] = *(const bf16x8*)(qb + (int64_t)q_ld * p.q_sl + 16 * s + 8 * L.hh);
        if (p.q_on_load()) {
            const float rstd = p.q_row_rstd(b, q_ld, p.H * DH);
            const int64_t trow = (int64_t)b * p.rope_sb + (int64_t)q_ld * p.rope_sl;
#pragma unroll
            for (int s = 0; s < NS; ++s) {
                const int col = head * DH + 16 * s + 8 * L.hh;
                const bf16x8 wv = *(const bf16x8*)(p.q_w + col);
                float o[8];
#pragma unroll
                for (int e = 0; e < 8; ++e) o[e] = (float)X.q[s][e] * rstd * (float)wv[e];
                if (p.rope_cos) {
                    const bf16x8 cv = *(const bf16x8*)(p.rope_cos + trow + col), sv = *(const bf16x8*)(p.rope_sin + trow + col);
#pragma unroll
                    for (int e = 0; e < 8; e += 2) {
                        const float r0 = o[e] * (float)cv[e] - o[e + 1] * (float)sv[e];
                        const float r1 = o[e + 1] * (float)cv[e + 1] + o[e] * (float)sv[e + 1];
                        o[e] = r0;
                        o[e + 1] = r1;
                    }
                }
#pragma unroll
                for (int e = 0; e < 8; ++e) X.q[s][e] = (__bf16)o[e];
            }
        }
        X.m = -INFINITY;
        X.mt = -INFINITY;
        X.l = f32x4{0.f, 0.f, 0.f, 0.f};
#pragma unroll
        for (int i = 0; i < 4; ++i) X.pf[i] = u32x4{0u, 0u, 0u, 0u};
#pragma unroll
        for (int d = 0; d < ND; ++d)
#pragma unroll
            for (int e = 0; e < 16; ++e) X.o[d][e] = 0.f;
#pragma unroll
        for (int kb = 0; kb < 2; ++kb)
#pragma unroll
            for (int e = 0; e < 16; ++e) X.s[kb][e] = 0.f;
    };
    const float c = p.scale_log2e;
    volatile int* redo_flag = (volatile int*)(smem + SMEM);
    if (tid == 0) *redo_flag = 0;
    for (int attempt = p.force_exact ? 1 : 0; attempt < 2; ++attempt) {
        if (attempt == 1 && !p.force_exact && p.redo_count != nullptr && tid == 0) atomicAdd(p.redo_count, 1u);
        dma_k(0); dma_v(0); dma_k(1); dma_v(1); dma_k(2);
        init(A, 0);
        init(Bk, 1);
#pragma unroll
        for (int s8 = 0; s8 < NS; ++s8) {
            asm volatile("" : "+a"(A.q[s8]));
            asm volatile("" : "+a"(Bk.q[s8]));
        }
        {
            const u32x4 z = {0u, 0u, 0u, 0u};
#pragma unroll
            for (int i = 0; i < TILE_BYTES / (256 * 16); ++i) *(u32x4*)(vring + 3 * TILE_BYTES + (i * 256 + tid) * 16) = z;
        }
        __builtin_amdgcn_s_waitcnt(0x0070);
        __builtin_amdgcn_s_barrier();
        __builtin_amdgcn_sched_barrier(0);

        bf16x8 kq[4];
#pragma unroll
        for (int j = 0; j < 2 * NS; ++j) {
            const bf16x8 kfj = kread(kring, L, j);
            if (j % NS == 0) mfma_s0(A.s[j / NS], kfj, A.q[j % NS]);
            else mfma_s(A.s[j / NS], kfj, A.q[j % NS]);
            if (j < 4) kq[j] = kfj;
        }
        {
            float mt = -INFINITY;
            asm volatile("s_nop 15\n\ts_nop 7" : "+v"(A.s[0]), "+v"(A.s[1]));
#pragma unroll
            for (int kb2 = 0; kb2 < 2; ++kb2)
#pragma unroll
                for (int e = 0; e < 16; ++e) {
                    if (p.Lk < KV_TILE) {
                        const int key = 32 * kb2 + (e & 3) + 8 * (e >> 2) + 4 * L.hh;
                        if (key >= p.Lk) A.s[kb2][e] = -INFINITY;
                    }
                    mt = fmaxf(mt, A.s[kb2][e]);
                }
            const auto sw = __builtin_amdgcn_permlane32_swap(__float_as_uint(mt), __float_as_uint(mt), false, false);
            A.mt = fmaxf(__uint_as_float(sw[0]), __uint_as_float(sw[1]));
        }

        auto iteration = [&](int t, auto exact_tag) __attribute__((always_inline)) {
            constexpr bool EXACT = decltype(exact_tag)::value;
            __builtin_amdgcn_s_barrier();
            __builtin_amdgcn_sched_barrier(0);
            const char* k_t = kring + (t & 3) * TILE_BYTES;
            const char* k_t1 = kring + ((t + 1) & 3) * TILE_BYTES;
            segment<EXACT>(A, Bk, kq, k_t, k_t1, vring + ((t + 3) & 3) * TILE_BYTES, L, ones, c, t * KV_TILE, p.Lk,
                           [&](int j) { if ((j & 7) == 3) dma_k1(t + 3, j >> 3); });
            segment<EXACT>(Bk, A, kq, k_t1, k_t1, vring + (t & 3) * TILE_BYTES, L, ones, c, (t + 1) * KV_TILE, p.Lk,
                           [&](int j) { if ((j & 7) == 3) dma_v1(t + 2, j >> 3); });
            asm volatile("s_waitcnt vmcnt(8)" ::: "memory");
            __builtin_amdgcn_sched_barrier(0);
        };
        const int t_exact = attempt == 0 ? (nt < 2 ? nt : 2) : nt;
        int t = 0;
        for (; t < t_exact; ++t) iteration(t, std::integral_constant<bool, true>{});
        for (; t < nt; ++t) iteration(t, std::integral_constant<bool, false>{});

        {
            const char* vs = vring + ((nt - 1) & 3) * TILE_BYTES;
            Bk.l = __builtin_amdgcn_mfma_f32_16x16x32_bf16(ones, __builtin_bit_cast(bf16x8, Bk.pf[3]), Bk.l, 0, 0, 0);
#pragma unroll
            for (int i = 0; i < 4 * ND; ++i) mfma_o(Bk.o[i % ND], vread(vs, L, i), __builtin_bit_cast(bf16x8, Bk.pf[i / ND]));
        }
        asm volatile("s_waitcnt vmcnt(0) lgkmcnt(0)" ::: "memory");
        bool outgrown = false;
        if (attempt == 0 && t_exact < nt) {
            constexpr uint32_t OUTGROWN_EXP = (127u + 100u) << 23;
            settle_o(A.o);
            settle_o(Bk.o);
            uint32_t worst = 0;
            auto scan = [&](const Blk& X) {
                worst |= (uint32_t)((__float_as_uint(X.l[0]) & 0x7f800000u) >= OUTGROWN_EXP);
                worst |= (uint32_t)((__float_as_uint(X.l[1]) & 0x7f800000u) >= OUTGROWN_EXP);
#pragma unroll
                for (int d = 0; d < ND; ++d)
#pragma unroll
                    for (int e = 0; e < 16; ++e) worst |= (uint32_t)((__float_as_uint(X.o[d][e]) & 0x7f800000u) >= OUTGROWN_EXP);
            };
            scan(A);
            scan(Bk);
            outgrown = __any(worst != 0);
        }
        if (outgrown && L.lane == 0) *redo_flag = 1;
        __builtin_amdgcn_s_barrier();
        __builtin_amdgcn_sched_barrier(0);
        const int redo = *redo_flag;
        __builtin_amdgcn_s_barrier();
        if (attempt == 1 || redo == 0) break;
    }


    auto store = [&](Blk& X, int blk) {
        settle_o(X.o);
        const float l0 = __shfl(X.l[0], L.r & 15, 64), l1 = __shfl(X.l[1], L.r & 15, 64);
        const float lrow = (L.r & 16) ? l1 : l0;
        const float inv = 1.0f / lrow;
        if (p.lse != nullptr) {
            const int row = qt * Q_PER_WG + wave * 64 + 32 * blk + L.r;
            if (L.hh == 0 && row < p.Lq) p.store_lse(b, head, row, X.m * c, lrow, false);
        }
        char* scr = smem + (wave * 2 + blk) * (32 * ROW_BYTES);
#pragma unroll
        for (int d = 0; d < ND; ++d)
#pragma unroll
            for (int g = 0; g < 4; ++g) {
                u32x2 w;
                w[0] = pack_bf16(X.o[d][4 * g + 0] * inv, X.o[d][4 * g + 1] * inv);
                w[1] = pack_bf16(X.o[d][4 * g + 2] * inv, X.o[d][4 * g + 3] * inv);
                const int chunk = 4 * d + g;
                *(u32x2*)(scr + L.r * ROW_BYTES + ((chunk ^ (L.r & 15)) << 4) + L.hh * 8) = w;
            }
        const int q0 = qt * Q_PER_WG + wave * 64 + 32 * blk;
#pragma unroll
        for (int t = 0; t < 8; ++t) {
            const int row = t * 4 + (L.lane >> 4), chunk = L.lane & 15;
            const u32x4 w = *(const u32x4*)(scr + row * ROW_BYTES + ((chunk ^ (row & 15)) << 4));
            if (q0 + row < p.Lq) *(u32x4*)(ob + p.o_row(q0 + row) + chunk * 8) = w;
        }
    };
    store(A, 0);
    store(Bk, 1);
}

}

int launch_attn_pipe128(AttnParams p, hipStream_t stream) {
    auto kern = pipe128::attn_pipe128_kernel;
    static unsigned long long lds_done = 0;
    if (const int rc = reserve_lds((const void*)kern, pipe128::SMEM + 16, &lds_done, "ltxmi_attention_fwd_bf16")) return rc;
    p.q_tiles = (p.Lq + pipe128::Q_PER_WG - 1) / pipe128::Q_PER_WG;
    const int64_t grid = (int64_t)p.B * p.H * p.q_tiles;
    hipLaunchKernelGGL(kern, dim3((unsigned)grid), dim3(256), pipe128::SMEM + 16, stream, p);
    return check_launch("ltxmi_attention_fwd_bf16");
}

}
```

### ltx-video-gpupoor_amd/ltxmi/_lib.py

```python
import ctypes
import os

import torch

_HERE = os.path.dirname(os.path.abspath(__file__))
LIB_PATH = os.environ.get("LTXMI_LIB") or os.path.join(_HERE, "libltxmi.so")

c_void_p, c_int, c_int64, c_float = ctypes.c_void_p, ctypes.c_int32, ctypes.c_int64, ctypes.c_float


class GemmArgs(ctypes.Structure):
    _fields_ = [("A", c_void_p), ("lda", c_int64), ("W", c_void_p), ("ldw", c_int64), ("bias", c_void_p),
                ("C", c_void_p), ("ldc", c_int64), ("M", c_int), ("N", c_int), ("K", c_int),
                ("epilogue", c_int), ("residual", c_void_p), ("ldr", c_int64), ("gate_table", c_void_p),
                ("gate_temb", c_void_p), ("gate_ld", c_int64), ("rows_per_group", c_int), ("algo", c_int),
                ("rowsumsq", c_void_p), ("rowsumsq_cols", c_int), ("rowsumsq_ld", c_int64),
                ("a_kblock", c_int), ("a_kblock_stride", c_int64)]


class AttnArgs(ctypes.Structure):
    _fields_ = [("q", c_void_p), ("q_stride_b", c_int64), ("q_stride_l", c_int64),
                ("k", c_void_p), ("k_stride_b", c_int64), ("k_stride_l", c_int64),
                ("v", c_void_p), ("v_stride_b", c_int64), ("v_stride_l", c_int64),
                ("o", c_void_p), ("o_stride_b", c_int64), ("o_stride_l", c_int64),
                ("key_bias", c_void_p), ("bias_stride_b", c_int64),
                ("B", c_int), ("H", c_int), ("Lq", c_int), ("Lk", c_int), ("head_dim", c_int),
                ("softmax_scale", c_float),
                ("q_rowsumsq", c_void_p), ("q_rowsumsq_stride_b", c_int64), ("q_rowsumsq_stride_l", c_int64),
                ("q_rowsumsq_blocks", c_int), ("q_norm_weight", c_void_p), ("q_norm_eps", c_float),
                ("rope_cos", c_void_p), ("rope_sin", c_void_p), ("rope_stride_b", c_int64), ("rope_stride_l", c_int64),
                ("o_segment_len", c_int), ("o_stride_segment", c_int64),
                ("q_rstd", c_void_p), ("q_rstd_stride_b", c_int64), ("q_rstd_stride_l", c_int64),
                ("redo_counter", c_void_p), ("force_exact", c_int),
                ("lse", c_void_p), ("lse_stride_b", c_int64), ("lse_stride_h", c_int64)]


ATTN_MERGE_MAX = 8


class AttnMergeArgs(ctypes.Structure):
    _fields_ = [("n", c_int),
                ("o_part", c_void_p * ATTN_MERGE_MAX), ("o_part_stride_b", c_int64 * ATTN_MERGE_MAX),
                ("o_part_stride_l", c_int64 * ATTN_MERGE_MAX),
                ("lse_part", c_void_p * ATTN_MERGE_MAX), ("lse_part_stride_b", c_int64 * ATTN_MERGE_MAX),
                ("lse_part_stride_h", c_int64 * ATTN_MERGE_MAX),
                ("o", c_void_p), ("o_stride_b", c_int64), ("o_stride_l", c_int64),
                ("lse", c_void_p), ("lse_stride_b", c_int64), ("lse_stride_h", c_int64),
                ("B", c_int), ("H", c_int), ("Lq", c_int), ("head_dim", c_int)]


class Conv3dArgs(ctypes.Structure):
    _fields_ = [("x", c_void_p), ("w", c_void_p), ("bias", c_void_p), ("y", c_void_p),
                ("B", c_int), ("T", c_int), ("H", c_int), ("W", c_int), ("Cin", c_int), ("Cout", c_int),
                ("causal", c_int), ("pad_replicate", c_int), ("d2s", c_int), ("residual", c_void_p),
                ("res_channels", c_int), ("add", c_void_p),
                ("stride_t", c_int), ("stride_hw", c_int), ("tpad", c_int), ("out_T", c_int),
                ("kernel_t", c_int), ("time_pad_zeros", c_int), ("algo", c_int),
                ("post_norm", c_int), ("post_scale", c_void_p), ("post_shift", c_void_p), ("post_eps", c_float),
                ("y_norm", c_void_p), ("workspace", c_void_p), ("workspace_bytes", c_int64)]


SIGNATURES = {
    "ltxmi_version": (ctypes.c_char_p, []),
    "ltxmi_last_error": (ctypes.c_char_p, []),
    "ltxmi_arch": (ctypes.c_char_p, []),
    "ltxmi_gemm_bf16": (c_int, [ctypes.POINTER(GemmArgs), c_void_p]),
    "ltxmi_norm_modulate_bf16": (c_int, [c_void_p, c_int64, c_void_p, c_int64, c_int, c_int, c_float, c_int,
                                         c_void_p, c_void_p, c_void_p, c_void_p, c_int64, c_int, c_void_p]),
    "ltxmi_rmsnorm_rope_bf16": (c_int, [c_void_p, c_int64, c_int, c_int, c_void_p, c_float, c_void_p, c_void_p,
                                        c_int64, c_int, c_void_p]),
    "ltxmi_rmsnorm_rope_rstd_bf16": (c_int, [c_void_p, c_int64, c_int, c_int, c_void_p, c_float, c_void_p, c_void_p,
                                             c_int64, c_int, c_void_p, c_int64, c_int, c_int, c_float, c_void_p, c_void_p]),
    "ltxmi_rowsumsq_rstd_f32": (c_int, [c_void_p, c_int64, c_int, c_int, c_int, c_float, c_void_p, c_void_p]),
    "ltxmi_qkv_norm_rope_pack_bf16": (c_int, [c_void_p, c_int64, c_int, c_int, c_int, c_int, c_void_p, c_void_p, c_float,
                                              c_void_p, c_void_p, c_int64, c_int, c_void_p, c_void_p]),
    "ltxmi_attention_fwd_bf16": (c_int, [ctypes.POINTER(AttnArgs), c_void_p]),
    "ltxmi_attention_merge_bf16": (c_int, [ctypes.POINTER(AttnMergeArgs), c_void_p]),
    "ltxmi_attention_fuses_qnorm": (c_int, [c_int, c_int, c_int, c_int, c_int, c_int]),
    "ltxmi_attention_kernel_id": (c_int, [c_int, c_int, c_int, c_int, c_int, c_int, c_int64, c_int64]),
    "ltxmi_silu_bf16": (c_int, [c_void_p, c_void_p, c_int64, c_void_p]),
    "ltxmi_timestep_embedding_bf16": (c_int, [c_void_p, c_void_p, c_int, c_int, c_void_p]),
    "ltxmi_stg_blend_bf16": (c_int, [c_void_p, c_int64, c_void_p, c_int64, c_void_p, c_int, c_int, c_int, c_void_p]),
    "ltxmi_stg_blend_grouped_bf16": (c_int, [c_void_p, c_void_p, c_int64, c_int64, c_int64, c_void_p, c_int, c_int, c_int, c_int,
                                             c_void_p]),
    "ltxmi_conv3d_ndhwc_bf16": (c_int, [ctypes.POINTER(Conv3dArgs), c_void_p]),
    "ltxmi_conv3d_fuses_post_norm": (c_int, [ctypes.POINTER(Conv3dArgs)]),
    "ltxmi_conv3d_workspace_bytes": (c_int64, [ctypes.POINTER(Conv3dArgs)]),
    "ltxmi_pixelnorm_ada_silu_bf16": (c_int, [c_void_p, c_void_p, c_int64, c_int, c_int64, c_void_p, c_void_p,
                                              c_int, c_float, c_void_p]),
    "ltxmi_add_bf16": (c_int, [c_void_p, c_void_p, c_void_p, c_int64, c_void_p]),
    "ltxmi_layernorm_affine_bf16": (c_int, [c_void_p, c_void_p, c_int64, c_int, c_void_p, c_void_p, c_float,
                                            c_void_p]),
    "ltxmi_ncdhw_to_ndhwc_bf16": (c_int, [c_void_p, c_void_p, c_int, c_int, c_int, c_int, c_int, c_void_p,
                                          c_void_p, c_void_p]),
    "ltxmi_unpatchify_to_ncdhw_bf16": (c_int, [c_void_p, c_void_p, c_int, c_int, c_int, c_int, c_int, c_int,
                                               c_void_p]),
    "ltxmi_guidance_step_masked_bf16": (c_int, [c_void_p, c_int64, c_int, c_float, c_float, c_float, c_int, c_int,
                                                c_int, c_void_p, c_int, c_float, c_void_p, c_int, c_float, c_void_p,
                                                c_void_p]),
    "ltxmi_image_cond_noise": (c_int, [c_void_p, c_void_p, c_void_p, c_int, c_void_p, c_int64, c_int, c_float,
                                       c_float, c_void_p]),
    "ltxmi_groupnorm_silu_bf16": (c_int, [c_void_p, c_void_p, c_void_p, c_int, c_int64, c_int, c_int, c_void_p,
                                          c_void_p, c_float, c_void_p, c_void_p]),
    "ltxmi_pixel_shuffle2d_ndhwc_bf16": (c_int, [c_void_p, c_void_p, c_int64, c_int, c_int, c_int, c_void_p]),
    "ltxmi_adain_filter": (c_int, [c_void_p, c_void_p, c_void_p, c_int, c_int, c_int64, c_int64, c_float, c_void_p]),
    "ltxmi_tile_blend": (c_int, [c_void_p, c_void_p, c_int, c_int64, c_int64, c_int64, c_int64, c_int, c_void_p]),
    "ltxmi_patchify_to_ndhwc_bf16": (c_int, [c_void_p, c_void_p, c_int, c_int, c_int, c_int, c_int, c_int, c_int,
                                             c_void_p]),
    "ltxmi_space_to_depth_skip_bf16": (c_int, [c_void_p, c_void_p, c_void_p, c_int, c_int, c_int, c_int, c_int,
                                               c_int, c_int, c_int, c_int, c_void_p]),
    "ltxmi_ndhwc_to_ncdhw_bf16": (c_int, [c_void_p, c_int64, c_int, c_void_p, c_int, c_int, c_int, c_int, c_int,
                                          c_void_p, c_void_p, c_void_p]),
    "ltxmi_guidance_step_bf16": (c_int, [c_void_p, c_int64, c_int, c_float, c_float, c_float, c_int, c_int, c_int,
                                         c_void_p, c_int, c_float, c_void_p, c_void_p]),
}


def _load():
    if not os.path.exists(LIB_PATH):
        raise ImportError(
            f"ltxmi: {LIB_PATH} is missing -- build it with `make -C ltx-video-gpupoor_amd/csrc` "
            "(or `python -c 'import __graft_entry__ as g; g.build()'`). There is no fallback path.")
    lib = ctypes.CDLL(LIB_PATH)
    for name, (res, args) in SIGNATURES.items():
        fn = getattr(lib, name)
        fn.restype = res
        fn.argtypes = args
    return lib


lib = _load()


class LtxmiError(RuntimeError):
    pass


def check(status, what):
    if status != 0:
        raise LtxmiError(f"{what} failed ({status}): {lib.ltxmi_last_error().decode()}")
```

### ltx-video-gpupoor_amd/ltxmi/attention.py

```python
from enum import Enum, auto
from typing import Optional

import torch
from torch import nn

from . import ops
from .attention_seam import pay_attention

BF16 = torch.bfloat16


FUSE_CROSS_ATTENTION_Q = True


class SkipLayerStrategy(Enum):
    AttentionSkip = auto()
    AttentionValues = auto()
    Residual = auto()
    TransformerBlock = auto()


def reshape_hidden_states(hidden_states, latent_frames):
    return hidden_states.reshape(hidden_states.shape[0], latent_frames, -1, hidden_states.shape[-1])


def restore_hidden_states_shape(hidden_states):
    return hidden_states.reshape(hidden_states.shape[0], -1, hidden_states.shape[-1])


class RMSNorm(nn.Module):

    def __init__(self, dim, eps: float, elementwise_affine: bool = True):
        super().__init__()
        self.eps = eps
        self.dim = dim
        if elementwise_affine:
            self.weight = nn.Parameter(torch.ones(dim))
        else:
            self.register_parameter("weight", None)


class _NoAffineLayerNorm(nn.Module):
    def __init__(self, dim, eps: float, elementwise_affine: bool = False):
        super().__init__()
        if elementwise_affine:
            raise NotImplementedError("ltxmi: standardisation norms with affine parameters are not on this path")
        self.eps = eps
        self.dim = dim


class GELUProj(nn.Module):

    def __init__(self, dim_in, dim_out, approximate="tanh", bias=True):
        super().__init__()
        self.proj = nn.Linear(dim_in, dim_out, bias=bias)
        self.approximate = approximate


class FeedForward(nn.Module):

    def __init__(self, dim, dim_out=None, mult=4, dropout=0.0, activation_fn="geglu", final_dropout=False,
                 inner_dim=None, bias=True):
        super().__init__()
        if activation_fn != "gelu-approximate":
            raise NotImplementedError(f"ltxmi: activation_fn '{activation_fn}' is not on this path "
                                      "(LTX-Video uses 'gelu-approximate')")
        inner_dim = int(dim * mult) if inner_dim is None else inner_dim
        dim_out = dim if dim_out is None else dim_out
        self.net = nn.ModuleList([GELUProj(dim, inner_dim, "tanh", bias), nn.Dropout(dropout),
                                  nn.Linear(inner_dim, dim_out, bias=bias)])

    def forward(self, hidden_states, scale: float = 1.0):
        h = ops.gemm(hidden_states, self.net[0].proj.weight, self.net[0].proj.bias, epilogue=ops.EPI_GELU_TANH)
        out = ops.gemm(h, self.net[2].weight, self.net[2].bias)
        return out.view(*hidden_states.shape[:-1], out.shape[-1])


class Attention(nn.Module):

    def __init__(self, query_dim, cross_attention_dim=None, heads=8, dim_head=64, dropout=0.0, bias=False,
                 upcast_attention=False, upcast_softmax=False, out_bias=True, scale_qk=True, qk_norm=None,
                 eps=1e-5, rescale_output_factor=1.0, residual_connection=False, processor=None, out_dim=None,
                 use_tpu_flash_attention=False, use_rope=False, **unsupported):
        super().__init__()
        for k, v in unsupported.items():
            if v not in (None, False, 32):
                raise NotImplementedError(f"ltxmi.Attention: argument {k}={v} is not on this path")
        if use_tpu_flash_attention:
            raise NotImplementedError("ltxmi.Attention: TPU flash attention does not exist on MI355X")
        self.inner_dim = out_dim if out_dim is not None else dim_head * heads
        self.query_dim = query_dim
        self.use_bias = bias
        self.is_cross_attention = cross_attention_dim is not None
        self.cross_attention_dim = cross_attention_dim if cross_attention_dim is not None else query_dim
        self.rescale_output_factor = rescale_output_factor
        self.residual_connection = residual_connection
        self.out_dim = out_dim if out_dim is not None else query_dim
        self.use_tpu_flash_attention = False
        self.use_rope = use_rope
        self.scale = dim_head ** -0.5 if scale_qk else 1.0
        self.heads = out_dim // dim_head if out_dim is not None else heads
        if qk_norm is None:
            self.q_norm, self.k_norm = nn.Identity(), nn.Identity()
        elif qk_norm == "rms_norm":
            self.q_norm = RMSNorm(dim_head * heads, eps=1e-5)
            self.k_norm = RMSNorm(dim_head * heads, eps=1e-5)
        else:
            raise NotImplementedError(f"ltxmi.Attention: qk_norm '{qk_norm}' is not on this path")
        self.to_q = nn.Linear(query_dim, self.inner_dim, bias=bias)
        self.to_k = nn.Linear(self.cross_attention_dim, self.inner_dim, bias=bias)
        self.to_v = nn.Linear(self.cross_attention_dim, self.inner_dim, bias=bias)
        self.to_out = nn.ModuleList([nn.Linear(self.inner_dim, self.out_dim, bias=out_bias), nn.Dropout(dropout)])
        self._packs = {}
        self.set_processor(processor if processor is not None else AttnProcessor2_0())

    def set_processor(self, processor) -> None:
        self.processor = processor

    def get_processor(self, return_deprecated_lora: bool = False):
        return self.processor

    def _pack(self, slot, mods):
        srcs = [t for m in mods for t in (m.weight, m.bias) if t is not None]
        key = tuple((t.data_ptr(), ops.tensor_version(t), t.dtype, t.device) for t in srcs)
        hit = self._packs.get(slot)
        if hit is None or hit[0] != key:
            with torch.no_grad():
                w = torch.cat([m.weight for m in mods], dim=0).contiguous()
                b = torch.cat([m.bias for m in mods], dim=0).contiguous() if mods[0].bias is not None else None
            hit = (key, w, b)
            self._packs[slot] = hit
        return hit[1], hit[2]

    def packed_qkv(self):
        if self.cross_attention_dim != self.query_dim:
            raise ValueError("ltxmi.Attention.packed_qkv: query and key/value inputs differ")
        return self._pack("qkv", [self.to_q, self.to_k, self.to_v])

    def packed_kv(self):
        return self._pack("kv", [self.to_k, self.to_v])

    def invalidate_packed(self):
        self._packs = {}
        self.__dict__.pop("_text_kv_cache", None)

    def _load_from_state_dict(self, *a, **k):
        self.invalidate_packed()
        return super()._load_from_state_dict(*a, **k)

    def _apply(self, fn, *a, **k):
        self.invalidate_packed()
        return super()._apply(fn, *a, **k)

    def forward(self, hidden_states, freqs_cis=None, encoder_hidden_states=None, attention_mask=None,
                skip_layer_mask=None, skip_layer_strategy=None, fused_residual=None, **cross_attention_kwargs):
        wrapper = hidden_states if isinstance(hidden_states, list) else [hidden_states]
        return self.processor(self, wrapper, freqs_cis=freqs_cis, encoder_hidden_states=encoder_hidden_states,
                              attention_mask=attention_mask, skip_layer_mask=skip_layer_mask,
                              skip_layer_strategy=skip_layer_strategy, fused_residual=fused_residual)


def _host_mask(mask):
    if mask is None:
        return None
    host = getattr(mask, "_ltxmi_host", None)
    return host if host is not None else [float(x) for x in mask.flatten().tolist()]


class AttnProcessor2_0:

    def attend(self, qkv_list, is_cross, **kw):
        return pay_attention(qkv_list, **kw)

    def __call__(self, attn: Attention, hidden_states_wrapper, freqs_cis, encoder_hidden_states=None,
                 attention_mask=None, temb=None, skip_layer_mask=None, skip_layer_strategy=None,
                 fused_residual=None, *args, **kwargs):
        hidden_states = hidden_states_wrapper[0]
        hidden_states_wrapper.clear()
        if hidden_states.dim() != 3:
            raise NotImplementedError("ltxmi.AttnProcessor2_0: only [B, N, D] inputs are on this path")
        B, N, _ = hidden_states.shape
        D = attn.inner_dim
        H = attn.heads
        dh = D // H
        x2 = hidden_states.reshape(B * N, -1)
        is_cross = encoder_hidden_states is not None
        if is_cross:
            wkv, bkv = attn.packed_kv()
        else:
            wqkv, bqkv = attn.packed_qkv()
        if not isinstance(attn.q_norm, RMSNorm):
            raise NotImplementedError("ltxmi.AttnProcessor2_0: qk_norm=None is not on this path")

        q_fused = None
        if not is_cross:
            fuse_q = ops.attention_fuses_qnorm(B, H, N, N, dh) and D % 64 == 0 and attention_mask is None
            ss = torch.empty((B * N, D // 64), dtype=torch.float32, device=x2.device) if fuse_q else None
            qkv = ops.gemm(x2, wqkv, bqkv, rowsumsq=ss, rowsumsq_cols=D if fuse_q else 0)
            q2, k2, v2 = qkv[:, :D], qkv[:, D:2 * D], qkv[:, 2 * D:]
            cos = sin = None
            period = 0
            if attn.use_rope:
                cos, sin = freqs_cis
                if cos.shape[0] not in (1, B):
                    raise ValueError("freqs_cis batch must be 1 or the batch size")
                cos2, sin2 = cos.reshape(-1, D), sin.reshape(-1, D)
                period = cos2.shape[0]
                cos, sin = cos2, sin2
            if fuse_q:
                rstd = torch.empty((B * N,), dtype=torch.float32, device=x2.device)
                ops.rmsnorm_rope_(k2, attn.k_norm.weight, attn.k_norm.eps, cos, sin, period,
                                  rstd_of=(ss, D, attn.q_norm.eps, rstd))
                q_fused = ((rstd, attn.q_norm.weight, attn.q_norm.eps), (cos, sin, period) if cos is not None else None)
            else:
                ops.rmsnorm_rope_(q2, attn.q_norm.weight, attn.q_norm.eps, cos, sin, period)
                ops.rmsnorm_rope_(k2, attn.k_norm.weight, attn.k_norm.eps, cos, sin, period)
            Lk = N
            q4 = qkv.view(B, N, 3, H, dh)[:, :, 0]
            k4 = qkv.view(B, N, 3, H, dh)[:, :, 1]
            v4 = qkv.view(B, N, 3, H, dh)[:, :, 2]
            v3 = qkv.view(B, N, 3 * D)[:, :, 2 * D:]
        else:
            Bk, Lk, _ = encoder_hidden_states.shape
            fuse_q = FUSE_CROSS_ATTENTION_Q and D % 64 == 0 and bool(ops.attention_fuses_qnorm(B, H, N, Lk, dh, attention_mask is not None))
            ss = torch.empty((B * N, D // 64), dtype=torch.float32, device=x2.device) if fuse_q else None
            q2 = ops.gemm(x2, attn.to_q.weight, attn.to_q.bias, rowsumsq=ss, rowsumsq_cols=D if fuse_q else 0)
            ehs = encoder_hidden_states
            key = (ehs.data_ptr(), tuple(ehs.shape), ops.tensor_version(ehs), wkv.data_ptr(), ops.tensor_version(wkv),
                   attn.k_norm.weight.data_ptr(), ops.tensor_version(attn.k_norm.weight))
            cache = attn.__dict__.setdefault("_text_kv_cache", {})
            hit = cache.get(key) if ops.STEP_INVARIANT_CACHING else None
            if hit is None:
                ready = attn.__dict__.get("_text_kv_ready")
                if ready is not None:
                    full, full_version, kv_full = ready
                    row_bytes = full.stride(0) * full.element_size()
                    off = ehs.data_ptr() - full.data_ptr()
                    if (row_bytes > 0 and off >= 0 and off % row_bytes == 0 and ehs.shape[1:] == full.shape[1:]
                            and off // row_bytes + Bk <= full.shape[0] and ehs.dtype == full.dtype and ehs.is_contiguous()
                            and ops.tensor_version(full) == full_version):
                        r0 = off // row_bytes
                        hit = (kv_full[r0 * Lk:(r0 + Bk) * Lk],)
            if hit is None:
                kv = ops.gemm(ehs.reshape(Bk * Lk, -1), wkv, bkv)
                ops.rmsnorm_rope_(kv[:, :D], attn.k_norm.weight, attn.k_norm.eps)
                if len(cache) >= 4:
                    cache.clear()
                if ops.STEP_INVARIANT_CACHING:
                    cache[key] = (kv, ehs, wkv)
            else:
                kv = hit[0]
            if fuse_q:
                q_fused = ((ops.rowsumsq_rstd(ss, D, attn.q_norm.eps), attn.q_norm.weight, attn.q_norm.eps), None)
            else:
                ops.rmsnorm_rope_(q2, attn.q_norm.weight, attn.q_norm.eps)
            q4 = q2.view(B, N, H, dh)
            k4 = kv.view(Bk, Lk, 2, H, dh)[:, :, 0]
            v4 = kv.view(Bk, Lk, 2, H, dh)[:, :, 1]
            v3 = kv.view(Bk, Lk, 2 * D)[:, :, D:]

        host_mask = _host_mask(skip_layer_mask) if skip_layer_mask is not None else None
        skip_attention = (host_mask is not None and skip_layer_strategy == SkipLayerStrategy.AttentionValues
                          and len(host_mask) == 1 and host_mask[0] == 0)
        if skip_attention:
            a3 = v3.contiguous()
        else:
            mask4 = None
            if attention_mask is not None:
                if attention_mask.dim() != 3 or attention_mask.shape[1] != 1:
                    raise NotImplementedError("ltxmi.AttnProcessor2_0: attention_mask must be a [B,1,Lk] bias")
                mask4 = attention_mask.reshape(B, 1, 1, Lk)
            a4 = self.attend([q4, k4, v4], is_cross, attention_mask=mask4, softmax_scale=attn.scale,
                             q_norm=q_fused[0] if q_fused else None, rope=q_fused[1] if q_fused else None)
            a3 = a4.view(B, N, D)
            if host_mask is not None and any(m != 1.0 for m in host_mask):
                m_dev = skip_layer_mask.reshape(B).to(torch.float32)
                if skip_layer_strategy == SkipLayerStrategy.AttentionValues:
                    ops.stg_blend_(a3, v3, m_dev)
                elif skip_layer_strategy == SkipLayerStrategy.AttentionSkip:
                    ops.stg_blend_(a3, hidden_states, m_dev)

        w_o, b_o = attn.to_out[0].weight, attn.to_out[0].bias
        if fused_residual is not None:
            residual, gate_table, gate_temb, rpg = fused_residual
            ops.gemm(a3.reshape(B * N, D), w_o, b_o, out=residual.reshape(B * N, -1),
                     epilogue=ops.EPI_GATE_RESIDUAL, residual=residual.reshape(B * N, -1),
                     gate_table=gate_table, gate_temb=gate_temb, rows_per_group=rpg)
            return residual
        out = ops.gemm(a3.reshape(B * N, D), w_o, b_o).view(B, N, -1)
        if attn.residual_connection or attn.rescale_output_factor != 1.0:
            raise NotImplementedError("ltxmi.AttnProcessor2_0: residual_connection / rescale_output_factor")
        return out


class BasicTransformerBlock(nn.Module):

    def __init__(self, dim, num_attention_heads, attention_head_dim, dropout=0.0, cross_attention_dim=None,
                 activation_fn="geglu", num_embeds_ada_norm=None, attention_bias=False, only_cross_attention=False,
                 double_self_attention=False, upcast_attention=False, norm_elementwise_affine=True,
                 adaptive_norm="single_scale_shift", standardization_norm="layer_norm", norm_eps=1e-5,
                 qk_norm=None, final_dropout=False, attention_type="default", ff_inner_dim=None, ff_bias=True,
                 attention_out_bias=True, use_tpu_flash_attention=False, use_rope=False):
        super().__init__()
        if adaptive_norm != "single_scale_shift" or only_cross_attention or double_self_attention:
            raise NotImplementedError("ltxmi.BasicTransformerBlock: only the AdaLN-Zero "
                                      "(single_scale_shift) self+cross block is on this path")
        assert standardization_norm in ("layer_norm", "rms_norm")
        self.adaptive_norm = adaptive_norm
        self.norm_kind = ops.NORM_RMS if standardization_norm == "rms_norm" else ops.NORM_LAYER
        make_norm = RMSNorm if standardization_norm == "rms_norm" else _NoAffineLayerNorm
        if norm_elementwise_affine:
            raise NotImplementedError("ltxmi.BasicTransformerBlock: norm_elementwise_affine=True is not on this path")
        self.norm1 = make_norm(dim, eps=norm_eps, elementwise_affine=False)
        self.attn1 = Attention(query_dim=dim, heads=num_attention_heads, dim_head=attention_head_dim,
                               dropout=dropout, bias=attention_bias, cross_attention_dim=None,
                               out_bias=attention_out_bias, qk_norm=qk_norm, use_rope=use_rope)
        if cross_attention_dim is not None:
            self.attn2 = Attention(query_dim=dim, cross_attention_dim=cross_attention_dim,
                                   heads=num_attention_heads, dim_head=attention_head_dim, dropout=dropout,
                                   bias=attention_bias, out_bias=attention_out_bias, qk_norm=qk_norm,
                                   use_rope=use_rope)
        else:
            self.attn2 = None
        self.norm2 = make_norm(dim, norm_eps, False)
        self.ff = FeedForward(dim, dropout=dropout, activation_fn=activation_fn, final_dropout=final_dropout,
                              inner_dim=ff_inner_dim, bias=ff_bias)
        self.scale_shift_table = nn.Parameter(torch.randn(6, dim) / dim ** 0.5)

    def prepare_shared_state(self):
        self.attn1.packed_qkv()
        if self.attn2 is not None:
            self.attn2.packed_kv()

    def forward(self, hidden_states, freqs_cis=None, attention_mask=None, encoder_hidden_states=None,
                encoder_attention_mask=None, timestep=None, cross_attention_kwargs=None, class_labels=None,
                added_cond_kwargs=None, skip_layer_mask=None, skip_layer_strategy: Optional[SkipLayerStrategy] = None):
        if attention_mask is not None:
            raise NotImplementedError("ltxmi.BasicTransformerBlock: a self-attention mask is not on this path")
        B, N, D = hidden_states.shape
        assert timestep.ndim == 3
        T1 = timestep.shape[1]
        if N % T1 != 0:
            raise ValueError(f"per-frame modulation needs tokens ({N}) divisible by frames ({T1})")
        rpg = N // T1
        host_mask = _host_mask(skip_layer_mask)
        if host_mask is not None and min(host_mask) == 1.0:
            skip_layer_mask, host_mask = None, None
        table = self.scale_shift_table
        temb = timestep.reshape(B * T1, 6 * D)
        h2 = hidden_states.view(B * N, D)

        def chunk(i):
            return table[i], temb[:, i * D:(i + 1) * D]

        norm_h = torch.empty_like(hidden_states)
        sc_t, sc_e = chunk(1)
        sh_t, sh_e = chunk(0)
        ops.norm_modulate(h2, norm_h.view(B * N, D), self.norm1.eps, self.norm_kind, sc_t, sc_e, sh_t, sh_e, rpg)
        g_t, g_e = chunk(2)
        self.attn1([norm_h], freqs_cis=freqs_cis, skip_layer_mask=skip_layer_mask,
                   skip_layer_strategy=skip_layer_strategy, fused_residual=(hidden_states, g_t, g_e, rpg))
        del norm_h

        if self.attn2 is not None:
            self.attn2([hidden_states], freqs_cis=freqs_cis, encoder_hidden_states=encoder_hidden_states,
                       attention_mask=encoder_attention_mask, fused_residual=(hidden_states, None, None, 1))

        block_skip = (host_mask is not None and skip_layer_strategy == SkipLayerStrategy.TransformerBlock)
        if block_skip:
            original = hidden_states.clone()

        norm_h = torch.empty_like(hidden_states)
        sc_t, sc_e = chunk(4)
        sh_t, sh_e = chunk(3)
        ops.norm_modulate(h2, norm_h.view(B * N, D), self.norm2.eps, self.norm_kind, sc_t, sc_e, sh_t, sh_e, rpg)
        ff1 = ops.gemm(norm_h.view(B * N, D), self.ff.net[0].proj.weight, self.ff.net[0].proj.bias,
                       epilogue=ops.EPI_GELU_TANH)
        del norm_h
        g_t, g_e = chunk(5)
        ops.gemm(ff1, self.ff.net[2].weight, self.ff.net[2].bias, out=h2, epilogue=ops.EPI_GATE_RESIDUAL,
                 residual=h2, gate_table=g_t, gate_temb=g_e, rows_per_group=rpg)
        del ff1

        if block_skip:
            ops.stg_blend_(hidden_states, original, skip_layer_mask.reshape(B).to(torch.float32))
        return hidden_states
```

### ltx-video-gpupoor_amd/ltxmi/attention_seam.py

```python
import torch

from . import ops


def _key_bias_from_mask(attention_mask, B, Lk):
    m = attention_mask
    if m.dim() != 4 or m.shape[0] != B or m.shape[-1] != Lk:
        raise ValueError(f"pay_attention: attention_mask must be [B, 1|Lq, 1|H, Lk], got {tuple(m.shape)}")
    for d in (1, 2):
        if m.shape[d] != 1 and m.stride(d) != 0:
            raise NotImplementedError(
                "pay_attention: only key biases broadcast over queries and heads are supported "
                f"(mask dim {d} has size {m.shape[d]} with stride {m.stride(d)})")
    key = (m.data_ptr(), tuple(m.shape), tuple(m.stride()), m.dtype, ops.tensor_version(m))
    hit = _BIAS_CACHE.get(key)
    if hit is None:
        if len(_BIAS_CACHE) >= 4:
            _BIAS_CACHE.clear()
        hit = _BIAS_CACHE[key] = (m[:, 0, 0, :].to(torch.float32).contiguous(), m)
    return hit[0]


_BIAS_CACHE = {}


@torch.compiler.disable()
def pay_attention(qkv_list, dropout_p=0., softmax_scale=None, causal=False, window_size=(-1, -1),
                  deterministic=False, version=None, force_attention=None, attention_mask=None,
                  cross_attn=False, q_lens=None, k_lens=None, q_norm=None, rope=None):
    q, k, v = qkv_list
    qkv_list.clear()
    if (q_norm is not None or rope is not None) and (q_lens is not None or k_lens is not None):
        raise NotImplementedError("pay_attention: q_norm / rope on load with q_lens / k_lens")
    if causal or tuple(window_size) != (-1, -1) or dropout_p != 0.:
        raise NotImplementedError("pay_attention: causal / windowed / dropout attention is not on this path")
    if force_attention not in (None, "sdpa"):
        raise NotImplementedError(f"pay_attention: backend '{force_attention}' does not exist here (single HIP backend)")
    out_dtype = q.dtype
    if v.dtype != torch.bfloat16:
        raise TypeError(f"pay_attention: bf16 only on this path, got {v.dtype}")
    q = q.to(v.dtype)
    k = k.to(v.dtype)
    b, lq, lk = q.size(0), q.size(1), k.size(1)
    final_padding = 0

    if b > 1 and k_lens is not None:
        assert attention_mask is None and q_lens is None
        k_lens = [int(x) for x in k_lens]
        chunk_sizes, k_sizes = [], []
        cur, cnt = k_lens[0], 1
        for kl in k_lens[1:]:
            if kl == cur:
                cnt += 1
            else:
                chunk_sizes.append(cnt)
                k_sizes.append(cur)
                cur, cnt = kl, 1
        chunk_sizes.append(cnt)
        k_sizes.append(cur)
        if len(chunk_sizes) > 1 or k_lens[0] != k.shape[1]:
            outs = []
            for sq, sk, sv, sz in zip(torch.split(q, chunk_sizes), torch.split(k, chunk_sizes),
                                      torch.split(v, chunk_sizes), k_sizes):
                outs.append(pay_attention([sq, sk[:, :sz], sv[:, :sz]], softmax_scale=softmax_scale))
            return torch.cat(outs, dim=0)
    elif q_lens is not None or k_lens is not None:
        assert b == 1
        szq = int(q_lens[0]) if q_lens is not None else lq
        szk = int(k_lens[0]) if k_lens is not None else lk
        final_padding = lq - szq
        q, k, v = q[:, :szq], k[:, :szk], v[:, :szk]

    bias = None if attention_mask is None else _key_bias_from_mask(attention_mask, b, k.size(1))
    x = ops.attention(q, k, v, key_bias=bias, softmax_scale=softmax_scale, q_norm=q_norm, rope=rope)
    x = x.type(out_dtype)
    if final_padding > 0:
        x = torch.cat([x, torch.empty((x.shape[0], final_padding, *x.shape[-2:]), dtype=x.dtype, device=x.device)], 1)
    return x
```

### ltx-video-gpupoor_amd/ltxmi/ops.py

```python
import ctypes
import math

import torch

from . import _lib
from ._lib import lib, check

BF16 = torch.bfloat16

EPI_NONE, EPI_GELU_TANH, EPI_SILU, EPI_GATE_RESIDUAL = 0, 1, 2, 3
NORM_RMS, NORM_LAYER = 0, 1


def _stream():
    return ctypes.c_void_p(torch.cuda.current_stream().cuda_stream)


_watch = None
_events = {}


def watch_launches(keys):
    global _watch
    _watch = set(keys) if keys else None
# ... 10 lines not shown

def launch_times_ms():
    return {k: [a.elapsed_time(b) for a, b in v] for k, v in _events.items()}


def _prof_begin(key, key2=None):
    if _watch is None:
        return None
    if key not in _watch:
        if key2 is None or key2 not in _watch:
            return None
        key = key2
    e0, e1 = torch.cuda.Event(enable_timing=True), torch.cuda.Event(enable_timing=True)
    e0.record()
    return key, e0, e1


def _prof_end(tok):
    if tok is not None:
        tok[2].record()
        _events.setdefault(tok[0], []).append((tok[1], tok[2]))


def _ptr(t):
    return None if t is None else ctypes.c_void_p(t.data_ptr())


def _chk_bf16(*ts):
    for t in ts:
        if t is None:
            continue
        if t.dtype != BF16 or not t.is_cuda:
            raise TypeError(f"ltxmi: expected a CUDA bfloat16 tensor, got {t.dtype} on {t.device}")


def _rows(t):
    if t.stride(-1) != 1:
        raise ValueError("ltxmi: innermost dimension must be contiguous")
    t2 = t.reshape(-1, t.shape[-1]) if t.is_contiguous() else t
    if t2.dim() != 2:
        raise ValueError("ltxmi: expected a 2-D tensor or a contiguous N-D tensor")
    return t2, t2.shape[0], t2.stride(0)


def tensor_version(t):
    try:
        return t._version
    except RuntimeError:
        return -1


def gemm(a, w, bias=None, out=None, epilogue=EPI_NONE, residual=None, gate_table=None, gate_temb=None,
         rows_per_group=1, algo=0, rowsumsq=None, rowsumsq_cols=0, a_kblock=0, a_kblock_stride=0):
    _chk_bf16(a, w, bias, out, residual, gate_table, gate_temb)
    a2, M, lda = _rows(a)
    N, K = w.shape
    if a_kblock:
        if a2.shape[1] != a_kblock or K % a_kblock:
            raise ValueError(f"ltxmi.gemm: K-blocked a must be [M, {a_kblock}] with K={K} a multiple of the block")
    elif a2.shape[1] != K:
        raise ValueError(f"ltxmi.gemm: a is [{M},{a2.shape[1]}] but w is [{N},{K}]")
    if out is None:
        out = torch.empty((M, N), dtype=BF16, device=a.device)
    o2, Mo, ldc = _rows(out)
    if Mo != M or o2.shape[1] != N:
        raise ValueError("ltxmi.gemm: bad out shape")
    args = _lib.GemmArgs()
    args.A, args.lda = a2.data_ptr(), lda
    args.W, args.ldw = w.data_ptr(), w.stride(0)
    args.bias = bias.data_ptr() if bias is not None else None
    args.C, args.ldc = o2.data_ptr(), ldc
    args.M, args.N, args.K = M, N, K
    args.epilogue = epilogue
    if residual is not None:
        r2, Mr, ldr = _rows(residual)
        args.residual, args.ldr = r2.data_ptr(), ldr
    if gate_table is not None:
        args.gate_table = gate_table.data_ptr()
        args.gate_temb = gate_temb.data_ptr()
        args.gate_ld = gate_temb.stride(0) if gate_temb.dim() == 2 else 0
    args.rows_per_group = rows_per_group
    args.algo = algo
    args.a_kblock, args.a_kblock_stride = a_kblock, a_kblock_stride
    if rowsumsq is not None:
        if rowsumsq.dtype != torch.float32 or rowsumsq.dim() != 2 or rowsumsq.shape[0] != M or rowsumsq.stride(1) != 1 \
                or rowsumsq.shape[1] * 64 < rowsumsq_cols:
            raise ValueError("ltxmi.gemm: rowsumsq must be fp32 [M, >= rowsumsq_cols/64]")
        args.rowsumsq, args.rowsumsq_cols, args.rowsumsq_ld = rowsumsq.data_ptr(), rowsumsq_cols, rowsumsq.stride(0)
    tok = _prof_begin(("gemm", M, N, K, epilogue))
    check(lib.ltxmi_gemm_bf16(ctypes.byref(args), _stream()), "ltxmi_gemm_bf16")
    _prof_end(tok)
    return out


def norm_modulate(x, out, eps, kind, scale_table, scale_temb, shift_table, shift_temb, rows_per_group):
    _chk_bf16(x, out, scale_table, scale_temb, shift_table, shift_temb)
    x2, rows, ldx = _rows(x)
    o2, _, ldy = _rows(out)
    D = x2.shape[1]
    if scale_temb.stride(0) != shift_temb.stride(0):
        raise ValueError("ltxmi.norm_modulate: scale/shift tables must share a row stride")
    check(lib.ltxmi_norm_modulate_bf16(_ptr(x2), ldx, _ptr(o2), ldy, rows, D, eps, kind,
                                       _ptr(scale_table), _ptr(scale_temb), _ptr(shift_table), _ptr(shift_temb),
                                       scale_temb.stride(0), rows_per_group, _stream()),
          "ltxmi_norm_modulate_bf16")
    return out


def rmsnorm_rope_(x, weight, eps, cos=None, sin=None, rope_period=0, rstd_of=None):
    _chk_bf16(x, weight, cos, sin)
    x2, rows, ldx = _rows(x)
    D = x2.shape[1]
    ld_tab = 0
    if cos is not None:
        if cos.dim() != 2 or cos.shape != sin.shape or cos.stride(0) != sin.stride(0):
            raise ValueError("ltxmi.rmsnorm_rope_: cos/sin must be matching 2-D tables")
        ld_tab = cos.stride(0)
        rope_period = rope_period or cos.shape[0]
    if rstd_of is not None:
        ss, norm_dim, norm_eps, out = rstd_of
        if ss.dtype != torch.float32 or out.dtype != torch.float32 or ss.dim() != 2 or ss.shape[0] != rows or \
                ss.stride(1) != 1 or out.shape != (rows,) or not out.is_contiguous():
            raise ValueError("ltxmi.rmsnorm_rope_: rstd_of needs fp32 sums [rows, blocks] and a contiguous fp32 out [rows]")
        check(lib.ltxmi_rmsnorm_rope_rstd_bf16(_ptr(x2), ldx, rows, D, _ptr(weight), eps, _ptr(cos), _ptr(sin), ld_tab,
                                               rope_period, _ptr(ss), ss.stride(0), ss.shape[1], norm_dim, norm_eps,
                                               _ptr(out), _stream()), "ltxmi_rmsnorm_rope_rstd_bf16")
        return x
    check(lib.ltxmi_rmsnorm_rope_bf16(_ptr(x2), ldx, rows, D, _ptr(weight), eps, _ptr(cos), _ptr(sin), ld_tab,
                                      rope_period, _stream()), "ltxmi_rmsnorm_rope_bf16")
    return x


def rowsumsq_rstd(ss, norm_dim, eps, out=None):
    if ss.dtype != torch.float32 or ss.dim() != 2 or ss.stride(1) != 1 or not ss.is_cuda:
        raise ValueError("ltxmi.rowsumsq_rstd: expected CUDA fp32 sums [rows, blocks]")
    rows = ss.shape[0]
    out = torch.empty((rows,), dtype=torch.float32, device=ss.device) if out is None else out
    check(lib.ltxmi_rowsumsq_rstd_f32(_ptr(ss), ss.stride(0), ss.shape[1], rows, norm_dim, eps, _ptr(out), _stream()),
          "ltxmi_rowsumsq_rstd_f32")
    return out


def attention_fuses_qnorm(B, H, Lq, Lk, dh, has_key_bias=False):
    return bool(lib.ltxmi_attention_fuses_qnorm(B, H, Lq, Lk, dh, int(has_key_bias)))


def attention_kernel_id(B, H, Lq, Lk, dh, has_key_bias=False, k_stride_l=None, v_stride_l=None):
    ks = 3 * H * dh if k_stride_l is None else k_stride_l
    vs = ks if v_stride_l is None else v_stride_l
    return int(lib.ltxmi_attention_kernel_id(B, H, Lq, Lk, dh, int(has_key_bias), ks, vs))


def attention(q, k, v, out=None, key_bias=None, softmax_scale=None, q_norm=None, rope=None, out_segments=None,
              redo_counter=None, force_exact=False, return_lse=False, lse=None):
    _chk_bf16(q, k, v, out)
    B, Lq, H, dh = q.shape
    Lk = k.shape[1]
    for t in (q, k, v):
        if t.stride(3) != 1 or t.stride(2) != dh:
            raise ValueError("ltxmi.attention: (heads, head_dim) must be contiguous")
    if out is None:
        if out_segments is not None:
            raise ValueError("ltxmi.attention: out_segments needs an explicit out")
        out = torch.empty((B, Lq, H, dh), dtype=BF16, device=q.device)
    if out.dim() != 4 or out.stride(3) != 1 or out.stride(2) != dh:
        raise ValueError("ltxmi.attention: out must be 4-D with (heads, head_dim) contiguous")
    a = _lib.AttnArgs()
    if out_segments is not None:
        seg_len, seg_stride = out_segments
        if seg_len <= 0 or Lq % seg_len != 0 or tuple(out.shape) != (B, seg_len, H, dh):
            raise ValueError(f"ltxmi.attention: out_segments=({seg_len}, {seg_stride}) needs Lq={Lq} to be a multiple of the "
                             f"segment and out to be segment 0's [B, segment, H, dh] view, got {tuple(out.shape)}")
        a.o_segment_len, a.o_stride_segment = seg_len, seg_stride
    elif tuple(out.shape) != (B, Lq, H, dh):
        raise ValueError(f"ltxmi.attention: out must be [B, Lq, H, dh] = {(B, Lq, H, dh)}, got {tuple(out.shape)}")
    a.q, a.q_stride_b, a.q_stride_l = q.data_ptr(), q.stride(0), q.stride(1)
    a.k, a.k_stride_b, a.k_stride_l = k.data_ptr(), k.stride(0), k.stride(1)
    a.v, a.v_stride_b, a.v_stride_l = v.data_ptr(), v.stride(0), v.stride(1)
    a.o, a.o_stride_b, a.o_stride_l = out.data_ptr(), out.stride(0), out.stride(1)
    if key_bias is not None:
        if key_bias.dtype != torch.float32 or key_bias.shape != (B, Lk) or key_bias.stride(1) != 1:
            raise ValueError("ltxmi.attention: key_bias must be fp32 [B, Lk]")
        a.key_bias, a.bias_stride_b = key_bias.data_ptr(), key_bias.stride(0)
    a.B, a.H, a.Lq, a.Lk, a.head_dim = B, H, Lq, Lk, dh
    a.softmax_scale = softmax_scale if softmax_scale is not None else 1.0 / math.sqrt(dh)
    if q_norm is not None:
        ss, w, eps = q_norm
        nb = H * dh // 64
        _chk_bf16(w)
        if ss.dim() == 1:
            if ss.dtype != torch.float32 or ss.shape != (B * Lq,) or ss.stride(0) != 1 or not ss.is_cuda:
                raise ValueError("ltxmi.attention: q_norm row factors must be a contiguous fp32 [B*Lq]")
            a.q_rstd, a.q_rstd_stride_b, a.q_rstd_stride_l = ss.data_ptr(), Lq, 1
        else:
            if ss.dtype != torch.float32 or ss.dim() != 2 or ss.shape != (B * Lq, nb) or ss.stride(1) != 1:
                raise ValueError("ltxmi.attention: q_norm row sums must be fp32 [B*Lq, H*dh/64]")
            a.q_rowsumsq, a.q_rowsumsq_stride_b, a.q_rowsumsq_stride_l = ss.data_ptr(), Lq * ss.stride(0), ss.stride(0)
            a.q_rowsumsq_blocks = nb
        a.q_norm_weight, a.q_norm_eps = w.data_ptr(), eps
        if rope is not None:
            cos, sin, period = rope
            _chk_bf16(cos, sin)
            if period not in (Lq, B * Lq) or cos.stride(0) != sin.stride(0) or cos.stride(1) != 1:
                raise ValueError("ltxmi.attention: rope tables must be [Lq or B*Lq, H*dh] with one row stride")
            a.rope_cos, a.rope_sin = cos.data_ptr(), sin.data_ptr()
            a.rope_stride_l = cos.stride(0)
            a.rope_stride_b = 0 if period == Lq else Lq * cos.stride(0)
    elif rope is not None:
        raise ValueError("ltxmi.attention: rope needs q_norm")
    if redo_counter is None:
        redo_counter = _redo_counter
    if redo_counter is not None:
        if redo_counter.dtype != torch.int32 or redo_counter.numel() != 1 or not redo_counter.is_cuda:
            raise ValueError("ltxmi.attention: redo_counter must be a CUDA int32 tensor of one element")
        a.redo_counter = redo_counter.data_ptr()
    a.force_exact = int(bool(force_exact))
    if return_lse or lse is not None:
        if lse is None:
            lse = torch.empty((B, H, Lq), dtype=torch.float32, device=q.device)
        _chk_lse(lse, B, H, Lq, "ltxmi.attention: lse")
        a.lse, a.lse_stride_b, a.lse_stride_h = lse.data_ptr(), lse.stride(0), lse.stride(1)
    tok = _prof_begin(("attention", B, H, Lq, Lk, dh))
    check(lib.ltxmi_attention_fwd_bf16(ctypes.byref(a), _stream()), "ltxmi_attention_fwd_bf16")
    _prof_end(tok)
    return (out, lse) if lse is not None else out


def _chk_lse(lse, B, H, Lq, what):
    if lse.dtype != torch.float32 or not lse.is_cuda or tuple(lse.shape) != (B, H, Lq) or lse.stride(2) != 1:
        raise ValueError(f"{what} must be a CUDA fp32 [B, H, Lq] = {(B, H, Lq)} tensor with contiguous tokens")


def attention_merge(outs, lses, out=None, return_lse=False, lse=None):
    n = len(outs)
    if n != len(lses) or not 2 <= n <= _lib.ATTN_MERGE_MAX:
        raise ValueError(f"ltxmi.attention_merge: {n} outputs / {len(lses)} lse tensors, need 2 .. {_lib.ATTN_MERGE_MAX} of each")
    _chk_bf16(*outs, out)
    B, Lq, H, dh = outs[0].shape
    if out is None:
        out = torch.empty((B, Lq, H, dh), dtype=BF16, device=outs[0].device)
    a = _lib.AttnMergeArgs()
    a.n = n
    for i, (o, l) in enumerate(zip(outs, lses)):
        if tuple(o.shape) != (B, Lq, H, dh) or o.stride(3) != 1 or o.stride(2) != dh:
            raise ValueError("ltxmi.attention_merge: partial outputs must be [B, Lq, H, dh] with (heads, head_dim) contiguous")
        _chk_lse(l, B, H, Lq, f"ltxmi.attention_merge: lses[{i}]")
        a.o_part[i], a.o_part_stride_b[i], a.o_part_stride_l[i] = o.data_ptr(), o.stride(0), o.stride(1)
        a.lse_part[i], a.lse_part_stride_b[i], a.lse_part_stride_h[i] = l.data_ptr(), l.stride(0), l.stride(1)
    if tuple(out.shape) != (B, Lq, H, dh) or out.stride(3) != 1 or out.stride(2) != dh:
        raise ValueError("ltxmi.attention_merge: out must be [B, Lq, H, dh] with (heads, head_dim) contiguous")
    a.o, a.o_stride_b, a.o_stride_l = out.data_ptr(), out.stride(0), out.stride(1)
    if return_lse or lse is not None:
        if lse is None:
            lse = torch.empty((B, H, Lq), dtype=torch.float32, device=out.device)
        _chk_lse(lse, B, H, Lq, "ltxmi.attention_merge: lse")
        a.lse, a.lse_stride_b, a.lse_stride_h = lse.data_ptr(), lse.stride(0), lse.stride(1)
    a.B, a.H, a.Lq, a.head_dim = B, H, Lq, dh
    check(lib.ltxmi_attention_merge_bf16(ctypes.byref(a), _stream()), "ltxmi_attention_merge_bf16")
    return (out, lse) if lse is not None else out


def qkv_norm_rope_pack(qkv, B, Nl, D, P, q_weight, k_weight, eps, cos=None, sin=None, rope_period=0, out=None):
    _chk_bf16(qkv, q_weight, k_weight, cos, sin, out)
    x2, rows, ld = _rows(qkv)
    if rows != B * Nl or x2.shape[1] != 3 * D:
        raise ValueError("ltxmi.qkv_norm_rope_pack: qkv must be [B*Nl, 3D]")
    if out is None:
        out = torch.empty((P, Nl, B, 3, D // P), dtype=BF16, device=qkv.device)
    if not out.is_contiguous() or out.numel() != rows * 3 * D:
        raise ValueError("ltxmi.qkv_norm_rope_pack: out must be a contiguous [P, Nl, B, 3, D/P] buffer")
    ld_tab = cos.stride(0) if cos is not None else 0
    check(lib.ltxmi_qkv_norm_rope_pack_bf16(_ptr(x2), ld, B, Nl, D, P, _ptr(q_weight), _ptr(k_weight), eps, _ptr(cos),
                                            _ptr(sin), ld_tab, rope_period, _ptr(out), _stream()),
          "ltxmi_qkv_norm_rope_pack_bf16")
    return out


def stg_blend_grouped_(a, v, m_f32):
    _chk_bf16(a, v)
    G, B, L, Dg = a.shape
    if not a.is_contiguous() or v.dim() != 3 or v.shape[0] != B or v.shape[1] != L or v.shape[2] < G * Dg or v.stride(2) != 1:
        raise ValueError("ltxmi.stg_blend_grouped_: a must be contiguous [G,B,L,Dg], v [B,L,>=G*Dg] with unit channel stride")
    check(lib.ltxmi_stg_blend_grouped_bf16(_ptr(a), _ptr(v), Dg, v.stride(0), v.stride(1), _ptr(m_f32), G, B, L, Dg, _stream()),
          "ltxmi_stg_blend_grouped_bf16")
    return a


def silu(x, out=None):
    _chk_bf16(x, out)
    out = torch.empty_like(x) if out is None else out
    check(lib.ltxmi_silu_bf16(_ptr(x), _ptr(out), x.numel(), _stream()), "ltxmi_silu_bf16")
    return out


def add(a, b, out=None):
    _chk_bf16(a, b, out)
    out = torch.empty_like(a) if out is None else out
    check(lib.ltxmi_add_bf16(_ptr(a), _ptr(b), _ptr(out), a.numel(), _stream()), "ltxmi_add_bf16")
    return out


def timestep_embedding(t_f32, dim=256):
    if t_f32.dtype != torch.float32 or not t_f32.is_cuda or not t_f32.is_contiguous():
        raise TypeError("ltxmi.timestep_embedding: expected a contiguous CUDA fp32 vector")
    out = torch.empty((t_f32.numel(), dim), dtype=BF16, device=t_f32.device)
    check(lib.ltxmi_timestep_embedding_bf16(_ptr(t_f32), _ptr(out), t_f32.numel(), dim, _stream()),
          "ltxmi_timestep_embedding_bf16")
    return out


def stg_blend_(a, v, m_f32):
    _chk_bf16(a, v)
    B, L, D = a.shape
    a2, _, lda = _rows(a)
    v2 = v.reshape(B * L, D) if v.is_contiguous() else v
    if v2.dim() == 3:
        if v2.stride(0) != L * v2.stride(1):
            raise ValueError("ltxmi.stg_blend_: v batch stride must equal L * row stride")
        ldv = v2.stride(1)
    else:
        ldv = v2.stride(0)
    check(lib.ltxmi_stg_blend_bf16(_ptr(a2), lda, _ptr(v2), ldv, _ptr(m_f32), B, L, D, _stream()),
          "ltxmi_stg_blend_bf16")
    return a


CONV_ALGO = 0


CONV_POST_NORM_FUSE = True
CONV_SECOND_OUTPUT_FUSE = True
CONV_SPLIT = True
_conv_workspace = {}


def conv3d(x, w_packed, bias, causal, pad_replicate, d2s=False, residual=None, add=None, out=None,
           stride=(1, 1, 1), tpad=0, out_T=0, kernel_t=3, time_pad_zeros=False, algo=None, post_norm=None, keep_raw=False):
    _chk_bf16(x, w_packed, bias, residual, add, out)
    B, T, H, W, Cin = x.shape
    Cout = w_packed.shape[0]
    if not x.is_contiguous() or not w_packed.is_contiguous():
        raise ValueError("ltxmi.conv3d: x and w must be contiguous")
    st, sh, sw = stride
    if sh != sw:
        raise ValueError("ltxmi.conv3d: height and width strides must be equal")
    front = tpad if tpad > 0 else (2 if causal else 1)
    back = 0 if (tpad > 0 or causal) else 1
    oT = out_T if out_T > 0 else (T + front + back - 3) // st + 1
    if kernel_t == 1:
        oT = T
    if w_packed.shape[1] != 9 * kernel_t * Cin:
        raise ValueError(f"ltxmi.conv3d: packed weight has K={w_packed.shape[1]}, expected {9 * kernel_t * Cin}")
    oH, oW = (H - 1) // sh + 1, (W - 1) // sh + 1
    if out is None:
        if d2s:
            out = torch.empty((B, 2 * T - 1, 2 * H, 2 * W, Cout // 8), dtype=BF16, device=x.device)
        else:
            out = torch.empty((B, oT, oH, oW, Cout), dtype=BF16, device=x.device)
    a = _lib.Conv3dArgs()
    a.x, a.w, a.bias, a.y = x.data_ptr(), w_packed.data_ptr(), (bias.data_ptr() if bias is not None else None), out.data_ptr()
    a.B, a.T, a.H, a.W, a.Cin, a.Cout = B, T, H, W, Cin, Cout
    a.causal, a.pad_replicate, a.d2s = int(causal), int(pad_replicate), int(d2s)
    a.stride_t, a.stride_hw, a.tpad, a.out_T = st, sh, tpad, out_T
    a.kernel_t, a.time_pad_zeros = kernel_t, int(time_pad_zeros)
    a.algo = CONV_ALGO if algo is None else algo
    if residual is not None:
        a.residual, a.res_channels = residual.data_ptr(), residual.shape[-1]
    if add is not None:
        if not add.is_contiguous() or add.shape != (B, oT, oH, oW, Cout):
            raise ValueError("ltxmi.conv3d: `add` must be a contiguous [B,T,H,W,Cout] tensor")
        a.add = add.data_ptr()
    out_norm = None
    if keep_raw and post_norm is None:
        raise ValueError("ltxmi.conv3d: keep_raw is for post_norm")
    if post_norm is not None:
        scale, shift, eps = post_norm
        if (scale is None) != (shift is None) or ((d2s or add is not None) and not keep_raw):
            raise ValueError("ltxmi.conv3d: post_norm needs scale and shift together, and (without keep_raw) the plain store "
# ... 220 lines not shown
```

### ltx-video-gpupoor_amd/ltxmi/transformer3d.py

```python
import contextlib
import math
from dataclasses import dataclass
from typing import Any, Dict, List, Optional

import torch
from torch import nn

from . import ops
from .attention import BasicTransformerBlock, SkipLayerStrategy

BF16 = torch.bfloat16


@dataclass
class Transformer3DModelOutput:
    sample: torch.Tensor


class _TimestepEmbedder(nn.Module):
    def __init__(self, in_channels, dim):
        super().__init__()
        self.linear_1 = nn.Linear(in_channels, dim)
        self.linear_2 = nn.Linear(dim, dim)

# ... 21 lines not shown
        emb = self.emb(timestep_f32)
        return ops.gemm(ops.silu(emb), self.linear.weight, self.linear.bias), emb


class PixArtAlphaTextProjection(nn.Module):
    def __init__(self, in_features, hidden_size):
        super().__init__()
        self.linear_1 = nn.Linear(in_features, hidden_size)
        self.linear_2 = nn.Linear(hidden_size, hidden_size)

    def forward(self, caption):
        h = ops.gemm(caption.reshape(-1, caption.shape[-1]), self.linear_1.weight, self.linear_1.bias,
                     epilogue=ops.EPI_GELU_TANH)
        return ops.gemm(h, self.linear_2.weight, self.linear_2.bias)


class _Config(dict):
    __getattr__ = dict.__getitem__


class Transformer3DModel(nn.Module):
    def __init__(self, num_attention_heads: int = 16, attention_head_dim: int = 88,
                 in_channels: Optional[int] = None, out_channels: Optional[int] = None, num_layers: int = 1,
                 dropout: float = 0.0, norm_num_groups: int = 32, cross_attention_dim: Optional[int] = None,
                 attention_bias: bool = False, num_vector_embeds: Optional[int] = None,
                 activation_fn: str = "geglu", num_embeds_ada_norm: Optional[int] = None,
                 use_linear_projection: bool = False, only_cross_attention: bool = False,
                 double_self_attention: bool = False, upcast_attention: bool = False,
                 adaptive_norm: str = "single_scale_shift", standardization_norm: str = "layer_norm",
                 norm_elementwise_affine: bool = True, norm_eps: float = 1e-5, attention_type: str = "default",
                 caption_channels: int = None, use_tpu_flash_attention: bool = False,
                 qk_norm: Optional[str] = None, positional_embedding_type: str = "rope",
                 positional_embedding_theta: Optional[float] = None,
                 positional_embedding_max_pos: Optional[List[int]] = None,
                 timestep_scale_multiplier: Optional[float] = None, causal_temporal_positioning: bool = False,
                 **ignored):
        super().__init__()
        self.config = _Config({k: v for k, v in locals().items() if k not in ("self", "ignored", "__class__")})
        if use_tpu_flash_attention:
            raise NotImplementedError("TPU flash attention does not exist on MI355X")
        if positional_embedding_type != "rope":
            raise ValueError("Absolute positional embedding is no longer supported")
        if positional_embedding_theta is None or positional_embedding_max_pos is None:
            raise ValueError("rope needs positional_embedding_theta and positional_embedding_max_pos")
        self.num_attention_heads = num_attention_heads
        self.attention_head_dim = attention_head_dim
        inner_dim = num_attention_heads * attention_head_dim
        self.inner_dim = inner_dim
        self.in_channels = in_channels
        self.patchify_proj = nn.Linear(in_channels, inner_dim, bias=True)
        self.positional_embedding_theta = positional_embedding_theta
        self.positional_embedding_max_pos = positional_embedding_max_pos
        self.use_rope = True
        self.timestep_scale_multiplier = timestep_scale_multiplier
        self.transformer_blocks = nn.ModuleList([
            BasicTransformerBlock(inner_dim, num_attention_heads, attention_head_dim, dropout=dropout,
                                  cross_attention_dim=cross_attention_dim, activation_fn=activation_fn,
                                  num_embeds_ada_norm=num_embeds_ada_norm, attention_bias=attention_bias,
                                  only_cross_attention=only_cross_attention,
                                  double_self_attention=double_self_attention, upcast_attention=upcast_attention,
                                  adaptive_norm=adaptive_norm, standardization_norm=standardization_norm,
                                  norm_elementwise_affine=norm_elementwise_affine, norm_eps=norm_eps,
                                  attention_type=attention_type, qk_norm=qk_norm, use_rope=True)
            for _ in range(num_layers)])
        self.out_channels = in_channels if out_channels is None else out_channels
        self.scale_shift_table = nn.Parameter(torch.randn(2, inner_dim) / inner_dim ** 0.5)
        self.proj_out = nn.Linear(inner_dim, self.out_channels)
        self.adaln_single = AdaLayerNormSingle(inner_dim, use_additional_conditions=False)
        self.caption_projection = None
        if caption_channels is not None:
            self.caption_projection = PixArtAlphaTextProjection(caption_channels, inner_dim)

    @property
    def dtype(self):
        return self.patchify_proj.weight.dtype

    @property
    def device(self):
        return self.patchify_proj.weight.device

    @classmethod
    def from_config(cls, config):
        return cls(**{k: v for k, v in dict(config).items() if not k.startswith("_")})

    @classmethod
    def from_pretrained(cls, pretrained_model_path, *args, device="cuda", dtype=torch.bfloat16, **kwargs):
        from .loading import load_transformer
        return load_transformer(pretrained_model_path, device=device, dtype=dtype)

    def load_state_dict(self, state_dict: Dict, *args, **kwargs):
        if any(k.startswith("model.diffusion_model.") for k in state_dict.keys()):
            state_dict = {k.replace("model.diffusion_model.", ""): v for k, v in state_dict.items()
                          if k.startswith("model.diffusion_model.")}
        return super().load_state_dict(state_dict, *args, **kwargs)

    def create_skip_layer_mask(self, batch_size: int, num_conds: int, ptb_index: int,
                               skip_block_list: Optional[List[int]] = None):
        if skip_block_list is None or len(skip_block_list) == 0:
            return None
        num_layers = len(self.transformer_blocks)
        host = torch.ones((num_layers, batch_size * num_conds), dtype=torch.float32)
        for block_idx in skip_block_list:
            host[block_idx, ptb_index::num_conds] = 0
        mask = host.to(device=self.device, dtype=self.dtype)
        mask._ltxmi_host_rows = [[float(x) for x in row] for row in host.tolist()]
        return mask

    def get_fractional_positions(self, indices_grid):
        return torch.stack([indices_grid[:, i] / self.positional_embedding_max_pos[i] for i in range(3)], dim=-1)

    def precompute_freqs_cis(self, indices_grid, spacing="exp"):
        if spacing != "exp":
            raise NotImplementedError("only the default 'exp' spacing is on this path")
        dtype = torch.float32
        dim = self.inner_dim
        theta = self.positional_embedding_theta
        frac = self.get_fractional_positions(indices_grid)
        indices = theta ** torch.linspace(math.log(1, theta), math.log(theta, theta), dim // 6,
                                          device=frac.device, dtype=dtype)
        indices = indices.to(dtype=dtype) * math.pi / 2
        freqs = (indices * (frac.unsqueeze(-1) * 2 - 1)).transpose(-1, -2).flatten(2)
        cos_freq = freqs.cos().repeat_interleave(2, dim=-1)
        sin_freq = freqs.sin().repeat_interleave(2, dim=-1)
        if dim % 6 != 0:
            cos_freq = torch.cat([torch.ones_like(cos_freq[:, :, : dim % 6]), cos_freq], dim=-1)
            sin_freq = torch.cat([torch.zeros_like(cos_freq[:, :, : dim % 6]), sin_freq], dim=-1)
        return cos_freq.to(self.dtype).contiguous(), sin_freq.to(self.dtype).contiguous()

    def _stacked_text_kv(self, ehs):
        blocks = [b for b in self.transformer_blocks if getattr(b, "attn2", None) is not None]
        if not blocks or ehs.dim() != 3 or not ehs.is_contiguous():
            return
        packs = [b.attn2.packed_kv() for b in blocks]
        if any(bk is None for _, bk in packs) or len({tuple(w.shape) for w, _ in packs}) != 1:
            return
        key = tuple((w.data_ptr(), ops.tensor_version(w), bk.data_ptr(), ops.tensor_version(bk)) for w, bk in packs)
        st = self.__dict__.get("_stacked_kv_weights")
        if st is None or st[0] != key:
            with torch.no_grad():
                st = (key, torch.cat([w for w, _ in packs], 0).contiguous(), torch.cat([bk for _, bk in packs], 0).contiguous(),
                      packs)
            self.__dict__["_stacked_kv_weights"] = st
        _, w_all, b_all, _ = st
        Bk, Lk, _ = ehs.shape
        two_d = packs[0][0].shape[0]
        kv_all = ops.gemm(ehs.reshape(Bk * Lk, -1), w_all, b_all)
        for i, b in enumerate(blocks):
            kv = kv_all[:, i * two_d:(i + 1) * two_d]
            ops.rmsnorm_rope_(kv[:, :two_d // 2], b.attn2.k_norm.weight, b.attn2.k_norm.eps)
            b.attn2.__dict__["_text_kv_ready"] = (ehs, ops.tensor_version(ehs), kv)

    def _run_blocks_microbatched(self, hidden_states, slices, freqs_cis, attention_mask, encoder_hidden_states,
                                 encoder_attention_mask, temb, cross_attention_kwargs, class_labels, layer_mask,
                                 skip_layer_strategy, ltxv_model):
        B = hidden_states.shape[0]
        on_gpu = hidden_states.is_cuda
        streams = None
        for block in self.transformer_blocks:
            block.prepare_shared_state()
        if on_gpu:
            main = torch.cuda.current_stream()
            key = (hidden_states.device, len(slices))
            pool = self.__dict__.setdefault("_mb_streams", {})
            streams = pool.get(key)
            if streams is None:
                streams = pool[key] = [torch.cuda.Stream(device=hidden_states.device) for _ in slices]
            for st in streams:
                st.wait_stream(main)

        def rows(t, sl):
            return t if (t is None or t.shape[0] != B) else t[sl]

        interrupted = False
        for block_idx, block in enumerate(self.transformer_blocks):
            for i, sl in enumerate(slices):
                ctx = torch.cuda.stream(streams[i]) if on_gpu else contextlib.nullcontext()
                with ctx:
                    block(hidden_states[sl], freqs_cis=tuple(rows(t, sl) for t in freqs_cis), attention_mask=attention_mask,
                          encoder_hidden_states=rows(encoder_hidden_states, sl),
                          encoder_attention_mask=rows(encoder_attention_mask, sl), timestep=temb[sl],
                          cross_attention_kwargs=cross_attention_kwargs, class_labels=class_labels,
                          skip_layer_mask=layer_mask(block_idx, sl), skip_layer_strategy=skip_layer_strategy)
            if ltxv_model is not None and ltxv_model._interrupt:
                interrupted = True
                break
        if on_gpu:
            for st in streams:
                main.wait_stream(st)
        return interrupted

    def forward(self, hidden_states: torch.Tensor, freqs_cis: list,
                encoder_hidden_states: Optional[torch.Tensor] = None, timestep: Optional[torch.Tensor] = None,
                class_labels: Optional[torch.LongTensor] = None, cross_attention_kwargs: Dict[str, Any] = None,
                attention_mask: Optional[torch.Tensor] = None, encoder_attention_mask: Optional[torch.Tensor] = None,
                skip_layer_mask: Optional[torch.Tensor] = None,
                skip_layer_strategy: Optional[SkipLayerStrategy] = None, latent_shape=None, joint_pass=True,
                ltxv_model=None, mixed=False, return_dict: bool = True, stg_alias_blocks: int = 0,
                _microbatches=None):
        if self.dtype != BF16:
            raise TypeError("ltxmi.Transformer3DModel runs in bfloat16 only: call .to(torch.bfloat16)")
        if mixed:
            raise NotImplementedError("mixed (fp32 residual stream) precision is not on this path")
        if attention_mask is not None:
            raise NotImplementedError("a self-attention mask is not on this path")
        dtype = self.dtype
        hidden_states = hidden_states.to(dtype)
        B, N, _ = hidden_states.shape
        D = self.inner_dim

        if encoder_attention_mask is not None and encoder_attention_mask.ndim == 2:
            encoder_attention_mask = ((1 - encoder_attention_mask.to(dtype)) * -10000.0).unsqueeze(1)

        hidden_states = ops.gemm(hidden_states.reshape(B * N, -1), self.patchify_proj.weight,
                                 self.patchify_proj.bias).view(B, N, D)

        timestep = timestep.to(torch.float32)
        if self.timestep_scale_multiplier:
            timestep = self.timestep_scale_multiplier * timestep
        if timestep.shape[-1] > 1:
            timestep = timestep.reshape(timestep.shape[0], -1, latent_shape[-2] * latent_shape[-1])[:, :, 0]
        temb, embedded_timestep = self.adaln_single(timestep.flatten())
        temb = temb.view(B, -1, 6 * D)
        embedded_timestep = embedded_timestep.view(B, -1, D)

        if self.caption_projection is not None:
            ehs = encoder_hidden_states
            cp = self.caption_projection
            key = (ehs.data_ptr(), tuple(ehs.shape), ehs.dtype, ops.tensor_version(ehs), cp.linear_1.weight.data_ptr(),
                   ops.tensor_version(cp.linear_1.weight), cp.linear_2.weight.data_ptr(), ops.tensor_version(cp.linear_2.weight))
            cache = self.__dict__.setdefault("_caption_cache", {})
            hit = cache.get(key) if ops.STEP_INVARIANT_CACHING else None
            if hit is None:
                if len(cache) >= 4:
                    cache.clear()
                hit = (cp(ehs.to(dtype)).view(B, -1, D), ehs)
                if ops.STEP_INVARIANT_CACHING:
                    cache[key] = hit
            encoder_hidden_states = hit[0]

        if joint_pass and ops.STACKED_TEXT_KV and not ops.STEP_INVARIANT_CACHING and encoder_hidden_states is not None:
            self._stacked_text_kv(encoder_hidden_states)

        host_rows = None
        if skip_layer_mask is not None:
            host_rows = getattr(skip_layer_mask, "_ltxmi_host_rows", None)
            if host_rows is None:
                host_rows = [[float(x) for x in row] for row in skip_layer_mask.float().cpu().tolist()]

        def layer_mask(block_idx, sl=None):
            if skip_layer_mask is None:
                return None
            m = skip_layer_mask[block_idx] if sl is None else skip_layer_mask[block_idx, sl]
            rows = host_rows[block_idx]
            m._ltxmi_host = rows if sl is None else rows[sl]
            return m

        first_block = 0
        if joint_pass and stg_alias_blocks and B >= 2:
            heads, dh = self.num_attention_heads, self.attention_head_dim
            if ops.attention_kernel_id(B, heads, N, N, dh) != ops.attention_kernel_id(B - 1, heads, N, N, dh):
                stg_alias_blocks = 0
        if joint_pass and stg_alias_blocks and B >= 2:
            first_block = min(int(stg_alias_blocks), len(self.transformer_blocks))
            keep = slice(0, B - 1)
            hs = hidden_states[keep]
            for block_idx in range(first_block):
                self.transformer_blocks[block_idx](
                    hs, freqs_cis=freqs_cis, attention_mask=attention_mask,
                    encoder_hidden_states=encoder_hidden_states[keep],
                    encoder_attention_mask=None if encoder_attention_mask is None else encoder_attention_mask[keep],
                    timestep=temb[keep], cross_attention_kwargs=cross_attention_kwargs, class_labels=class_labels,
                    skip_layer_mask=layer_mask(block_idx, keep), skip_layer_strategy=skip_layer_strategy)
                if ltxv_model is not None and ltxv_model._interrupt:
                    return [None]
            hidden_states[B - 1].copy_(hidden_states[B - 2])
        if joint_pass and _microbatches and len(_microbatches) > 1 and first_block == 0:
            if self._run_blocks_microbatched(hidden_states, _microbatches, freqs_cis, attention_mask, encoder_hidden_states,
                                             encoder_attention_mask, temb, cross_attention_kwargs, class_labels,
                                             layer_mask, skip_layer_strategy, ltxv_model):
                return [None]
        elif joint_pass:
            for block_idx, block in enumerate(self.transformer_blocks):
                if block_idx < first_block:
                    continue
                hidden_states = block(hidden_states, freqs_cis=freqs_cis, attention_mask=attention_mask,
                                      encoder_hidden_states=encoder_hidden_states,
                                      encoder_attention_mask=encoder_attention_mask, timestep=temb,
                                      cross_attention_kwargs=cross_attention_kwargs, class_labels=class_labels,
                                      skip_layer_mask=layer_mask(block_idx),
                                      skip_layer_strategy=skip_layer_strategy)
                if ltxv_model is not None and ltxv_model._interrupt:
                    return [None]
        else:
            for block_idx, block in enumerate(self.transformer_blocks):
                for i in range(B):
                    block(hidden_states[i:i + 1], freqs_cis=freqs_cis, attention_mask=attention_mask,
                          encoder_hidden_states=encoder_hidden_states[i:i + 1],
                          encoder_attention_mask=encoder_attention_mask[i:i + 1], timestep=temb[i:i + 1],
                          cross_attention_kwargs=cross_attention_kwargs, class_labels=class_labels,
                          skip_layer_mask=layer_mask(block_idx, slice(i, i + 1)),
                          skip_layer_strategy=skip_layer_strategy)
                    if ltxv_model is not None and ltxv_model._interrupt:
                        return [None]

        for block in self.transformer_blocks:
            if getattr(block, "attn2", None) is not None:
                block.attn2.__dict__.pop("_text_kv_ready", None)

        T1 = embedded_timestep.shape[1]
        emb2 = embedded_timestep.reshape(B * T1, D)
        normed = torch.empty_like(hidden_states)
        ops.norm_modulate(hidden_states.view(B * N, D), normed.view(B * N, D), 1e-6, ops.NORM_LAYER,
                          self.scale_shift_table[1], emb2, self.scale_shift_table[0], emb2, N // T1)
        out = ops.gemm(normed.view(B * N, D), self.proj_out.weight, self.proj_out.bias).view(B, N, -1)
        if not return_dict:
            return (out,)
        return Transformer3DModelOutput(sample=out)
```

Baseline: 16.57.

## Skip masked key tiles and dead batch rows in attention kernels

Adds a small kernel that computes, per batch row, how many key tiles hold unmasked text tokens. The cross-attention kernel then dispatches to a specialization with fewer key tiles. A live-row mask also lets attention launches skip batch rows whose output is unused, shrinking the grid. This cuts wasted work on padded text keys and skipped rows, at the cost of an extra tiny launch (cached across steps), runtime template dispatch, and more per-block indexing.

```diff
diff --git a/include/ltxmi.h b/include/ltxmi.h
--- a/include/ltxmi.h
+++ b/include/ltxmi.h
@@ -80,6 +80,14 @@
 } ltxmi_attn_args;
 
 int ltxmi_attention_fwd_bf16(const ltxmi_attn_args* args, void* stream);
+typedef struct ltxmi_attn_live_args {
+    ltxmi_attn_args attn;
+    const int32_t* key_tiles;
+    uint64_t batch_live_mask;
+} ltxmi_attn_live_args;
+int ltxmi_attention_fwd_live_bf16(const ltxmi_attn_live_args* args, void* stream);
+int ltxmi_key_bias_tile_bound(const float* key_bias, int64_t bias_stride_b, int32_t B, int32_t Lk, float softmax_scale,
+                              float removed_at, int32_t* key_tiles, void* stream);
 int ltxmi_attention_fuses_qnorm(int32_t B, int32_t H, int32_t Lq, int32_t Lk, int32_t head_dim, int32_t has_key_bias);
 int ltxmi_attention_kernel_id(int32_t B, int32_t H, int32_t Lq, int32_t Lk, int32_t head_dim, int32_t has_key_bias,
                               int64_t k_stride_l, int64_t v_stride_l);
diff --git a/ltx-video-gpupoor_amd/csrc/api.hip b/ltx-video-gpupoor_amd/csrc/api.hip
--- a/ltx-video-gpupoor_amd/csrc/api.hip
+++ b/ltx-video-gpupoor_amd/csrc/api.hip
@@ -64,6 +64,6 @@
 
 }
 
-extern "C" const char* ltxmi_version(void) { return "ltxmi 0.6.0 (round 5)"; }
+extern "C" const char* ltxmi_version(void) { return "ltxmi 0.7.0 (round 5)"; }
 extern "C" const char* ltxmi_last_error(void) { return ltxmi::g_err; }
 extern "C" const char* ltxmi_arch(void) { return "gfx950"; }
diff --git a/ltx-video-gpupoor_amd/csrc/attention.h b/ltx-video-gpupoor_amd/csrc/attention.h
--- a/ltx-video-gpupoor_amd/csrc/attention.h
+++ b/ltx-video-gpupoor_amd/csrc/attention.h
@@ -19,6 +19,15 @@
     int o_seg; int64_t o_sseg;
     uint32_t* redo_count; int force_exact;
     float* lse; int64_t lse_sb, lse_sh;
+    const int32_t* key_tiles;
+    uint64_t live_mask; int n_live;
+
+    __device__ __forceinline__ int live_row(int j) const {
+        if (live_mask == 0) return j;
+        uint64_t m = live_mask;
+        for (int i = 0; i < j; ++i) m &= m - 1;
+        return __builtin_ctzll(m);
+    }
 
     __host__ __device__ __forceinline__ bool q_on_load() const { return q_ss != nullptr || q_rstd != nullptr; }
     __device__ __forceinline__ float q_row_rstd(int b, int row, int HD) const {
diff --git a/ltx-video-gpupoor_amd/csrc/attention.hip b/ltx-video-gpupoor_amd/csrc/attention.hip
--- a/ltx-video-gpupoor_amd/csrc/attention.hip
+++ b/ltx-video-gpupoor_amd/csrc/attention.hip
@@ -44,7 +44,7 @@
     const int xcd = orig & 7, qn = nwg >> 3, rn = nwg & 7;
     const int work = (xcd < rn ? xcd * (qn + 1) : rn * (qn + 1) + (xcd - rn) * qn) + (orig >> 3);
     const int bh = work / p.q_tiles, qt = work % p.q_tiles;
-    const int b = bh / p.H, head = bh % p.H;
+    const int b = p.live_row(bh / p.H), head = bh % p.H;
 
     const uint16_t* qb = p.q + (int64_t)b * p.q_sb + head * DH;
     const uint16_t* kb_ = p.k + (int64_t)b * p.k_sb + head * DH;
@@ -371,7 +371,7 @@
     if (const int rc = reserve_lds((const void*)kern, C::SMEM, &lds_done, "ltxmi_attention_fwd_bf16")) return rc;
     const int q_per_wg = Q_PER_WG * QB;
     p.q_tiles = (p.Lq + q_per_wg - 1) / q_per_wg;
-    const int64_t grid = (int64_t)p.B * p.H * p.q_tiles;
+    const int64_t grid = (int64_t)p.n_live * p.H * p.q_tiles;
     hipLaunchKernelGGL(kern, dim3((unsigned)grid), dim3(256), C::SMEM, stream, p);
     return check_launch("ltxmi_attention_fwd_bf16");
 }
@@ -394,7 +394,7 @@
 
 using namespace ltxmi;
 
-extern "C" int ltxmi_attention_fwd_bf16(const ltxmi_attn_args* a, void* stream) {
+static int attention_fwd(const ltxmi_attn_args* a, const int32_t* key_tiles, uint64_t live_mask, void* stream) {
     LTXMI_REQUIRE(a && a->q && a->k && a->v && a->o, LTXMI_ERR_INVALID_ARG, "ltxmi_attention_fwd_bf16: NULL argument");
     LTXMI_REQUIRE(a->B > 0 && a->H > 0 && a->Lq > 0 && a->Lk > 0, LTXMI_ERR_INVALID_ARG,
                   "ltxmi_attention_fwd_bf16: non-positive shape B=%d H=%d Lq=%d Lk=%d", a->B, a->H, a->Lq, a->Lk);
@@ -428,6 +428,15 @@
     LTXMI_REQUIRE(a->o_segment_len >= 0 && a->o_stride_segment % 8 == 0, LTXMI_ERR_INVALID_ARG,
                   "ltxmi_attention_fwd_bf16: bad output segment geometry");
     p.lse = a->lse; p.lse_sb = a->lse_stride_b; p.lse_sh = a->lse_stride_h;
+    LTXMI_REQUIRE((((uintptr_t)key_tiles) & 3) == 0, LTXMI_ERR_INVALID_ARG, "ltxmi_attention_fwd_live_bf16: key_tiles must be 4-byte aligned");
+    p.key_tiles = key_tiles;
+    p.live_mask = 0; p.n_live = a->B;
+    if (live_mask != 0) {
+        LTXMI_REQUIRE(a->B <= 64 && (a->B == 64 || (live_mask >> a->B) == 0), LTXMI_ERR_INVALID_ARG,
+                      "ltxmi_attention_fwd_live_bf16: batch_live_mask names a row >= B = %d (or B > 64)", a->B);
+        const int n = __builtin_popcountll(live_mask);
+        if (n < a->B) { p.live_mask = live_mask; p.n_live = n; }
+    }
     if (a->lse)
         LTXMI_REQUIRE((((uintptr_t)a->lse) & 3) == 0 && a->lse_stride_h >= a->Lq &&
                           (a->B == 1 ? a->lse_stride_b >= 0 : a->lse_stride_b >= (int64_t)a->H * a->lse_stride_h),
@@ -458,6 +467,13 @@
     }
 }
 
+extern "C" int ltxmi_attention_fwd_bf16(const ltxmi_attn_args* a, void* stream) { return attention_fwd(a, nullptr, 0, stream); }
+
+extern "C" int ltxmi_attention_fwd_live_bf16(const ltxmi_attn_live_args* a, void* stream) {
+    LTXMI_REQUIRE(a, LTXMI_ERR_INVALID_ARG, "ltxmi_attention_fwd_live_bf16: NULL argument");
+    return attention_fwd(&a->attn, a->key_tiles, a->batch_live_mask, stream);
+}
+
 extern "C" int ltxmi_attention_kernel_id(int32_t B, int32_t H, int32_t Lq, int32_t Lk, int32_t head_dim, int32_t has_key_bias,
                                          int64_t k_stride_l, int64_t v_stride_l) {
     if (B <= 0 || H <= 0 || Lq <= 0 || Lk <= 0 || k_stride_l <= 0 || v_stride_l <= 0) return -1;
diff --git a/ltx-video-gpupoor_amd/csrc/attention_cross.hip b/ltx-video-gpupoor_amd/csrc/attention_cross.hip
--- a/ltx-video-gpupoor_amd/csrc/attention_cross.hip
+++ b/ltx-video-gpupoor_amd/csrc/attention_cross.hip
@@ -26,21 +26,12 @@
 __device__ __forceinline__ int k_swz(int row) { return (row >> 1) & 7; }
 
 template <int NT>
-__global__ __launch_bounds__(256, 2) void attn_cross_kernel(AttnParams p, int groups, int rows_per_group, int stagger_from) {
-    extern __shared__ __attribute__((aligned(16))) char smem[];
+__device__ __forceinline__ void attn_cross_body(const AttnParams& p, char* smem, const int b, const int head, const int row_begin,
+                                                const int row_end, const int stagger_from) {
     const int tid = threadIdx.x;
     const int lane = tid & 63;
     const int wave = __builtin_amdgcn_readfirstlane(tid >> 6);
     const int r = lane & 31, hh = lane >> 5;
-
-    const int nwg = gridDim.x, orig = blockIdx.x;
-    const int xcd = orig & 7, qn = nwg >> 3, rn = nwg & 7;
-    const int work = (xcd < rn ? xcd * (qn + 1) : rn * (qn + 1) + (xcd - rn) * qn) + (orig >> 3);
-    const int bh = work / groups, grp = work % groups;
-    const int b = bh / p.H, head = bh % p.H;
-    const int row_begin = grp * rows_per_group;
-    const int row_end = min(p.Lq, row_begin + rows_per_group);
-    if (row_begin >= row_end) return;
     const int n_it = (row_end - row_begin + ROWS_PER_IT - 1) / ROWS_PER_IT;
 
     const uint16_t* qb = p.q + (int64_t)b * p.q_sb + head * DH;
@@ -265,6 +256,50 @@
                 if (q0 + row < row_end) *(u32x4*)(ob + p.o_row(q0 + row) + 32 * d + chunk * 8) = w;
             }
         }
+    }
+}
+
+template <int NT_MAX>
+__global__ __launch_bounds__(256, 2) void attn_cross_kernel(AttnParams p, int groups, int rows_per_group, int stagger_from) {
+    extern __shared__ __attribute__((aligned(16))) char smem[];
+    const int nwg = gridDim.x, orig = blockIdx.x;
+    const int xcd = orig & 7, qn = nwg >> 3, rn = nwg & 7;
+    const int work = (xcd < rn ? xcd * (qn + 1) : rn * (qn + 1) + (xcd - rn) * qn) + (orig >> 3);
+    const int bh = work / groups, grp = work % groups;
+    const int b = p.live_row(bh / p.H), head = bh % p.H;
+    const int row_begin = grp * rows_per_group;
+    const int row_end = min(p.Lq, row_begin + rows_per_group);
+    if (row_begin >= row_end) return;
+    if constexpr (NT_MAX > 1) {
+        if (p.key_tiles != nullptr) {
+            const int kt = __builtin_amdgcn_readfirstlane(p.key_tiles[b]);
+            if (kt == 1) return attn_cross_body<1>(p, smem, b, head, row_begin, row_end, stagger_from);
+            if constexpr (NT_MAX > 2)
+                if (kt == 2) return attn_cross_body<2>(p, smem, b, head, row_begin, row_end, stagger_from);
+            if constexpr (NT_MAX > 3)
+                if (kt == 3) return attn_cross_body<3>(p, smem, b, head, row_begin, row_end, stagger_from);
+        }
+    }
+    attn_cross_body<NT_MAX>(p, smem, b, head, row_begin, row_end, stagger_from);
+}
+
+__global__ __launch_bounds__(256) void key_bias_tile_bound_kernel(const float* __restrict__ bias, int64_t bias_sb, int Lk,
+                                                                  float scale_log2e, float removed_at, int32_t* __restrict__ out) {
+    __shared__ int last_of_wave[4];
+    const float* row = bias + (int64_t)blockIdx.x * bias_sb;
+    int last = -1;
+    for (int j = threadIdx.x; j < Lk; j += 256) {
+        const float v = row[j];
+        const bool removed = v * (LOG2E / scale_log2e) <= ATTN_BIAS_FLOOR || v <= removed_at;
+        if (!removed) last = j;
+    }
+#pragma unroll
+    for (int o = 32; o > 0; o >>= 1) last = max(last, __shfl_xor(last, o, 64));
+    if ((threadIdx.x & 63) == 0) last_of_wave[threadIdx.x >> 6] = last;
+    __syncthreads();
+    if (threadIdx.x == 0) {
+        last = max(max(last_of_wave[0], last_of_wave[1]), max(last_of_wave[2], last_of_wave[3]));
+        out[blockIdx.x] = last < 0 ? (Lk + KV_TILE - 1) / KV_TILE : last / KV_TILE + 1;
     }
 }
 
@@ -283,7 +318,7 @@
     int rows = (p.Lq + groups - 1) / groups;
     rows = (rows + cross::ROWS_PER_IT - 1) / cross::ROWS_PER_IT * cross::ROWS_PER_IT;
     groups = (p.Lq + rows - 1) / rows;
-    const int64_t grid = (int64_t)bh * groups;
+    const int64_t grid = (int64_t)p.n_live * p.H * groups;
     const int nt = (p.Lk + cross::KV_TILE - 1) / cross::KV_TILE;
 #define LTXMI_XATTN_LAUNCH(N)                                                                                              \
     {                                                                                                                      \
@@ -305,3 +340,14 @@
 }
 
 }
+
+extern "C" int ltxmi_key_bias_tile_bound(const float* key_bias, int64_t bias_stride_b, int32_t B, int32_t Lk, float softmax_scale,
+                                         float removed_at, int32_t* key_tiles, void* stream) {
+    using namespace ltxmi;
+    LTXMI_REQUIRE(key_bias && key_tiles, LTXMI_ERR_INVALID_ARG, "ltxmi_key_bias_tile_bound: NULL argument");
+    LTXMI_REQUIRE(B > 0 && Lk > 0 && softmax_scale > 0.f && ((((uintptr_t)key_bias) | ((uintptr_t)key_tiles)) & 3) == 0,
+                  LTXMI_ERR_INVALID_ARG, "ltxmi_key_bias_tile_bound: bad geometry (B %d, Lk %d, scale %g)", B, Lk, (double)softmax_scale);
+    hipLaunchKernelGGL(cross::key_bias_tile_bound_kernel, dim3((unsigned)B), dim3(256), 0, (hipStream_t)stream, key_bias,
+                       bias_stride_b, Lk, softmax_scale * cross::LOG2E, removed_at, key_tiles);
+    return check_launch("ltxmi_key_bias_tile_bound");
+}
diff --git a/ltx-video-gpupoor_amd/csrc/attention_pipe.hip b/ltx-video-gpupoor_amd/csrc/attention_pipe.hip
--- a/ltx-video-gpupoor_amd/csrc/attention_pipe.hip
+++ b/ltx-video-gpupoor_amd/csrc/attention_pipe.hip
@@ -156,7 +156,7 @@
     const int xcd = orig & 7, qn = nwg >> 3, rn = nwg & 7;
     const int work = (xcd < rn ? xcd * (qn + 1) : rn * (qn + 1) + (xcd - rn) * qn) + (orig >> 3);
     const int bh = work / p.q_tiles, qt = work % p.q_tiles;
-    const int b = bh / p.H, head = bh % p.H;
+    const int b = p.live_row(bh / p.H), head = bh % p.H;
 
     const uint16_t* qb = p.q + (int64_t)b * p.q_sb + head * DH;
     const uint16_t* kb_ = p.k + (int64_t)b * p.k_sb + head * DH;
@@ -470,7 +470,7 @@
     static unsigned long long lds_done[4] = {0, 0, 0, 0};
     if (const int rc = reserve_lds((const void*)kern, pipe::SMEM + 16, &lds_done[(p.force_exact ? 2 : 0) + qscaled], "ltxmi_attention_fwd_bf16")) return rc;
     p.q_tiles = (p.Lq + pipe::Q_PER_WG - 1) / pipe::Q_PER_WG;
-    const int64_t grid = (int64_t)p.B * p.H * p.q_tiles;
+    const int64_t grid = (int64_t)p.n_live * p.H * p.q_tiles;
     hipLaunchKernelGGL(kern, dim3((unsigned)grid), dim3(256), pipe::SMEM + 16, stream, p);
     return check_launch("ltxmi_attention_fwd_bf16");
 }
diff --git a/ltx-video-gpupoor_amd/csrc/attention_pipe128.hip b/ltx-video-gpupoor_amd/csrc/attention_pipe128.hip
--- a/ltx-video-gpupoor_amd/csrc/attention_pipe128.hip
+++ b/ltx-video-gpupoor_amd/csrc/attention_pipe128.hip
@@ -158,7 +158,7 @@
     const int xcd = orig & 7, qn = nwg >> 3, rn = nwg & 7;
     const int work = (xcd < rn ? xcd * (qn + 1) : rn * (qn + 1) + (xcd - rn) * qn) + (orig >> 3);
     const int bh = work / p.q_tiles, qt = work % p.q_tiles;
-    const int b = bh / p.H, head = bh % p.H;
+    const int b = p.live_row(bh / p.H), head = bh % p.H;
 
     const uint16_t* qb = p.q + (int64_t)b * p.q_sb + head * DH;
     const uint16_t* kb_ = p.k + (int64_t)b * p.k_sb + head * DH;
@@ -409,7 +409,7 @@
     static unsigned long long lds_done = 0;
     if (const int rc = reserve_lds((const void*)kern, pipe128::SMEM + 16, &lds_done, "ltxmi_attention_fwd_bf16")) return rc;
     p.q_tiles = (p.Lq + pipe128::Q_PER_WG - 1) / pipe128::Q_PER_WG;
-    const int64_t grid = (int64_t)p.B * p.H * p.q_tiles;
+    const int64_t grid = (int64_t)p.n_live * p.H * p.q_tiles;
     hipLaunchKernelGGL(kern, dim3((unsigned)grid), dim3(256), pipe128::SMEM + 16, stream, p);
     return check_launch("ltxmi_attention_fwd_bf16");
 }
diff --git a/ltx-video-gpupoor_amd/ltxmi/_lib.py b/ltx-video-gpupoor_amd/ltxmi/_lib.py
--- a/ltx-video-gpupoor_amd/ltxmi/_lib.py
+++ b/ltx-video-gpupoor_amd/ltxmi/_lib.py
@@ -33,6 +33,10 @@
                 ("q_rstd", c_void_p), ("q_rstd_stride_b", c_int64), ("q_rstd_stride_l", c_int64),
                 ("redo_counter", c_void_p), ("force_exact", c_int),
                 ("lse", c_void_p), ("lse_stride_b", c_int64), ("lse_stride_h", c_int64)]
+
+
+class AttnLiveArgs(ctypes.Structure):
+    _fields_ = [("attn", AttnArgs), ("key_tiles", c_void_p), ("batch_live_mask", ctypes.c_uint64)]
 
 
 ATTN_MERGE_MAX = 8
@@ -75,6 +79,8 @@
     "ltxmi_qkv_norm_rope_pack_bf16": (c_int, [c_void_p, c_int64, c_int, c_int, c_int, c_int, c_void_p, c_void_p, c_float,
                                               c_void_p, c_void_p, c_int64, c_int, c_void_p, c_void_p]),
     "ltxmi_attention_fwd_bf16": (c_int, [ctypes.POINTER(AttnArgs), c_void_p]),
+    "ltxmi_attention_fwd_live_bf16": (c_int, [ctypes.POINTER(AttnLiveArgs), c_void_p]),
+    "ltxmi_key_bias_tile_bound": (c_int, [c_void_p, c_int64, c_int, c_int, c_float, c_float, c_void_p, c_void_p]),
     "ltxmi_attention_merge_bf16": (c_int, [ctypes.POINTER(AttnMergeArgs), c_void_p]),
     "ltxmi_attention_fuses_qnorm": (c_int, [c_int, c_int, c_int, c_int, c_int, c_int]),
     "ltxmi_attention_kernel_id": (c_int, [c_int, c_int, c_int, c_int, c_int, c_int, c_int64, c_int64]),
diff --git a/ltx-video-gpupoor_amd/ltxmi/attention.py b/ltx-video-gpupoor_amd/ltxmi/attention.py
--- a/ltx-video-gpupoor_amd/ltxmi/attention.py
+++ b/ltx-video-gpupoor_amd/ltxmi/attention.py
@@ -11,6 +11,7 @@
 
 
 FUSE_CROSS_ATTENTION_Q = True
+SKIP_MASKED_ROWS = True
 
 
 class SkipLayerStrategy(Enum):
@@ -153,11 +154,13 @@
         return super()._apply(fn, *a, **k)
 
     def forward(self, hidden_states, freqs_cis=None, encoder_hidden_states=None, attention_mask=None,
-                skip_layer_mask=None, skip_layer_strategy=None, fused_residual=None, **cross_attention_kwargs):
+                skip_layer_mask=None, skip_layer_strategy=None, fused_residual=None, key_tiles=None,
+                **cross_attention_kwargs):
         wrapper = hidden_states if isinstance(hidden_states, list) else [hidden_states]
         return self.processor(self, wrapper, freqs_cis=freqs_cis, encoder_hidden_states=encoder_hidden_states,
                               attention_mask=attention_mask, skip_layer_mask=skip_layer_mask,
-                              skip_layer_strategy=skip_layer_strategy, fused_residual=fused_residual)
+                              skip_layer_strategy=skip_layer_strategy, fused_residual=fused_residual,
+                              **({} if key_tiles is None else {"key_tiles": key_tiles}))
 
 
 def _host_mask(mask):
@@ -174,7 +177,7 @@
 
     def __call__(self, attn: Attention, hidden_states_wrapper, freqs_cis, encoder_hidden_states=None,
                  attention_mask=None, temb=None, skip_layer_mask=None, skip_layer_strategy=None,
-                 fused_residual=None, *args, **kwargs):
+                 fused_residual=None, *args, key_tiles=None, **kwargs):
         hidden_states = hidden_states_wrapper[0]
         hidden_states_wrapper.clear()
         if hidden_states.dim() != 3:
@@ -270,10 +273,26 @@
                 if attention_mask.dim() != 3 or attention_mask.shape[1] != 1:
                     raise NotImplementedError("ltxmi.AttnProcessor2_0: attention_mask must be a [B,1,Lk] bias")
                 mask4 = attention_mask.reshape(B, 1, 1, Lk)
+            replaced = (host_mask is not None and any(m != 1.0 for m in host_mask)
+                        and skip_layer_strategy in (SkipLayerStrategy.AttentionValues, SkipLayerStrategy.AttentionSkip))
+            live = None
+            if replaced and SKIP_MASKED_ROWS and not is_cross and hidden_states.is_cuda \
+                    and all(m in (0.0, 1.0) for m in host_mask) and any(host_mask):
+                live = [m == 1.0 for m in host_mask]
+            extra = {}
+            if key_tiles is not None and is_cross:
+                extra["key_tiles"] = key_tiles
+            if live is not None:
+                extra["live_rows"] = live
             a4 = self.attend([q4, k4, v4], is_cross, attention_mask=mask4, softmax_scale=attn.scale,
-                             q_norm=q_fused[0] if q_fused else None, rope=q_fused[1] if q_fused else None)
+                             q_norm=q_fused[0] if q_fused else None, rope=q_fused[1] if q_fused else None, **extra)
             a3 = a4.view(B, N, D)
-            if host_mask is not None and any(m != 1.0 for m in host_mask):
+            if live is not None:
+                src = v3 if skip_layer_strategy == SkipLayerStrategy.AttentionValues else hidden_states
+                for i, on in enumerate(live):
+                    if not on:
+                        a3[i].copy_(src[i])
+            elif replaced:
                 m_dev = skip_layer_mask.reshape(B).to(torch.float32)
                 if skip_layer_strategy == SkipLayerStrategy.AttentionValues:
                     ops.stg_blend_(a3, v3, m_dev)
@@ -334,7 +353,8 @@
 
     def forward(self, hidden_states, freqs_cis=None, attention_mask=None, encoder_hidden_states=None,
                 encoder_attention_mask=None, timestep=None, cross_attention_kwargs=None, class_labels=None,
-                added_cond_kwargs=None, skip_layer_mask=None, skip_layer_strategy: Optional[SkipLayerStrategy] = None):
+                added_cond_kwargs=None, skip_layer_mask=None, skip_layer_strategy: Optional[SkipLayerStrategy] = None,
+                encoder_key_tiles=None):
         if attention_mask is not None:
             raise NotImplementedError("ltxmi.BasicTransformerBlock: a self-attention mask is not on this path")
         B, N, D = hidden_states.shape
@@ -364,7 +384,8 @@
 
         if self.attn2 is not None:
             self.attn2([hidden_states], freqs_cis=freqs_cis, encoder_hidden_states=encoder_hidden_states,
-                       attention_mask=encoder_attention_mask, fused_residual=(hidden_states, None, None, 1))
+                       attention_mask=encoder_attention_mask, fused_residual=(hidden_states, None, None, 1),
+                       key_tiles=encoder_key_tiles)
 
         block_skip = (host_mask is not None and skip_layer_strategy == SkipLayerStrategy.TransformerBlock)
         if block_skip:
diff --git a/ltx-video-gpupoor_amd/ltxmi/attention_seam.py b/ltx-video-gpupoor_amd/ltxmi/attention_seam.py
--- a/ltx-video-gpupoor_amd/ltxmi/attention_seam.py
+++ b/ltx-video-gpupoor_amd/ltxmi/attention_seam.py
@@ -27,11 +27,13 @@
 @torch.compiler.disable()
 def pay_attention(qkv_list, dropout_p=0., softmax_scale=None, causal=False, window_size=(-1, -1),
                   deterministic=False, version=None, force_attention=None, attention_mask=None,
-                  cross_attn=False, q_lens=None, k_lens=None, q_norm=None, rope=None):
+                  cross_attn=False, q_lens=None, k_lens=None, q_norm=None, rope=None, key_tiles=None, live_rows=None):
     q, k, v = qkv_list
     qkv_list.clear()
     if (q_norm is not None or rope is not None) and (q_lens is not None or k_lens is not None):
         raise NotImplementedError("pay_attention: q_norm / rope on load with q_lens / k_lens")
+    if (key_tiles is not None or live_rows is not None) and (q_lens is not None or k_lens is not None):
+        raise NotImplementedError("pay_attention: key_tiles / live_rows with q_lens / k_lens")
     if causal or tuple(window_size) != (-1, -1) or dropout_p != 0.:
         raise NotImplementedError("pay_attention: causal / windowed / dropout attention is not on this path")
     if force_attention not in (None, "sdpa"):
@@ -72,7 +74,8 @@
         q, k, v = q[:, :szq], k[:, :szk], v[:, :szk]
 
     bias = None if attention_mask is None else _key_bias_from_mask(attention_mask, b, k.size(1))
-    x = ops.attention(q, k, v, key_bias=bias, softmax_scale=softmax_scale, q_norm=q_norm, rope=rope)
+    hints = {name: val for name, val in (("key_tiles", key_tiles), ("live_rows", live_rows)) if val is not None}
+    x = ops.attention(q, k, v, key_bias=bias, softmax_scale=softmax_scale, q_norm=q_norm, rope=rope, **hints)
     x = x.type(out_dtype)
     if final_padding > 0:
         x = torch.cat([x, torch.empty((x.shape[0], final_padding, *x.shape[-2:]), dtype=x.dtype, device=x.device)], 1)
diff --git a/ltx-video-gpupoor_amd/ltxmi/ops.py b/ltx-video-gpupoor_amd/ltxmi/ops.py
--- a/ltx-video-gpupoor_amd/ltxmi/ops.py
+++ b/ltx-video-gpupoor_amd/ltxmi/ops.py
@@ -186,7 +186,7 @@
 
 
 def attention(q, k, v, out=None, key_bias=None, softmax_scale=None, q_norm=None, rope=None, out_segments=None,
-              redo_counter=None, force_exact=False, return_lse=False, lse=None):
+              redo_counter=None, force_exact=False, return_lse=False, lse=None, key_tiles=None, live_rows=None):
     _chk_bf16(q, k, v, out)
     B, Lq, H, dh = q.shape
     Lk = k.shape[1]
@@ -199,7 +199,16 @@
         out = torch.empty((B, Lq, H, dh), dtype=BF16, device=q.device)
     if out.dim() != 4 or out.stride(3) != 1 or out.stride(2) != dh:
         raise ValueError("ltxmi.attention: out must be 4-D with (heads, head_dim) contiguous")
-    a = _lib.AttnArgs()
+    live = _lib.AttnLiveArgs()
+    a = live.attn
+    if key_tiles is not None:
+        if key_tiles.dtype != torch.int32 or tuple(key_tiles.shape) != (B,) or key_tiles.stride(0) != 1 or not key_tiles.is_cuda:
+            raise ValueError("ltxmi.attention: key_tiles must be a contiguous CUDA int32 [B]")
+        live.key_tiles = key_tiles.data_ptr()
+    if live_rows is not None:
+        if len(live_rows) != B or B > 64 or not any(live_rows):
+            raise ValueError(f"ltxmi.attention: live_rows needs {B} <= 64 entries, at least one of them true")
+        live.batch_live_mask = sum(1 << i for i, on in enumerate(live_rows) if on)
     if out_segments is not None:
         seg_len, seg_stride = out_segments
         if seg_len <= 0 or Lq % seg_len != 0 or tuple(out.shape) != (B, seg_len, H, dh):
@@ -255,9 +264,23 @@
         _chk_lse(lse, B, H, Lq, "ltxmi.attention: lse")
         a.lse, a.lse_stride_b, a.lse_stride_h = lse.data_ptr(), lse.stride(0), lse.stride(1)
     tok = _prof_begin(("attention", B, H, Lq, Lk, dh))
-    check(lib.ltxmi_attention_fwd_bf16(ctypes.byref(a), _stream()), "ltxmi_attention_fwd_bf16")
+    if key_tiles is not None or live_rows is not None:
+        check(lib.ltxmi_attention_fwd_live_bf16(ctypes.byref(live), _stream()), "ltxmi_attention_fwd_live_bf16")
+    else:
+        check(lib.ltxmi_attention_fwd_bf16(ctypes.byref(a), _stream()), "ltxmi_attention_fwd_bf16")
     _prof_end(tok)
     return (out, lse) if lse is not None else out
+
+
+def key_bias_tile_bound(key_bias, softmax_scale, removed_at=-math.inf, out=None):
+    kb = key_bias[:, 0] if key_bias.dim() == 3 and key_bias.shape[1] == 1 else key_bias
+    if kb.dtype != torch.float32 or kb.dim() != 2 or kb.stride(1) != 1 or not kb.is_cuda:
+        raise ValueError("ltxmi.key_bias_tile_bound: key_bias must be a CUDA fp32 [B, Lk] or [B, 1, Lk] with contiguous keys")
+    B, Lk = kb.shape
+    out = torch.empty((B,), dtype=torch.int32, device=kb.device) if out is None else out
+    check(lib.ltxmi_key_bias_tile_bound(_ptr(kb), kb.stride(0), B, Lk, softmax_scale, removed_at, _ptr(out), _stream()),
+          "ltxmi_key_bias_tile_bound")
+    return out
 
 
 def _chk_lse(lse, B, H, Lq, what):
diff --git a/ltx-video-gpupoor_amd/ltxmi/transformer3d.py b/ltx-video-gpupoor_amd/ltxmi/transformer3d.py
--- a/ltx-video-gpupoor_amd/ltxmi/transformer3d.py
+++ b/ltx-video-gpupoor_amd/ltxmi/transformer3d.py
@@ -197,7 +197,7 @@
 
     def _run_blocks_microbatched(self, hidden_states, slices, freqs_cis, attention_mask, encoder_hidden_states,
                                  encoder_attention_mask, temb, cross_attention_kwargs, class_labels, layer_mask,
-                                 skip_layer_strategy, ltxv_model):
+                                 skip_layer_strategy, ltxv_model, encoder_key_tiles=None):
         B = hidden_states.shape[0]
         on_gpu = hidden_states.is_cuda
         streams = None
@@ -225,7 +225,8 @@
                           encoder_hidden_states=rows(encoder_hidden_states, sl),
                           encoder_attention_mask=rows(encoder_attention_mask, sl), timestep=temb[sl],
                           cross_attention_kwargs=cross_attention_kwargs, class_labels=class_labels,
-                          skip_layer_mask=layer_mask(block_idx, sl), skip_layer_strategy=skip_layer_strategy)
+                          skip_layer_mask=layer_mask(block_idx, sl), skip_layer_strategy=skip_layer_strategy,
+                          encoder_key_tiles=rows(encoder_key_tiles, sl))
             if ltxv_model is not None and ltxv_model._interrupt:
                 interrupted = True
                 break
@@ -233,6 +234,24 @@
             for st in streams:
                 main.wait_stream(st)
         return interrupted
+
+    def _key_tile_bound(self, mask_given, bias, removed_at):
+        blocks = self.transformer_blocks
+        if bias is None or not bias.is_cuda or bias.dim() != 3 or bias.shape[1] != 1 or not len(blocks) \
+                or getattr(blocks[0], "attn2", None) is None:
+            return None
+        scale = float(blocks[0].attn2.scale)
+        m = mask_given
+        key = (m.data_ptr(), tuple(m.shape), tuple(m.stride()), m.dtype, ops.tensor_version(m), scale, removed_at)
+        cache = self.__dict__.setdefault("_key_tiles_cache", {})
+        hit = cache.get(key) if ops.STEP_INVARIANT_CACHING else None
+        if hit is None:
+            if len(cache) >= 4:
+                cache.clear()
+            hit = (ops.key_bias_tile_bound(bias.to(torch.float32), scale, removed_at), m)
+            if ops.STEP_INVARIANT_CACHING:
+                cache[key] = hit
+        return hit[0]
 
     def forward(self, hidden_states: torch.Tensor, freqs_cis: list,
                 encoder_hidden_states: Optional[torch.Tensor] = None, timestep: Optional[torch.Tensor] = None,
@@ -253,8 +272,12 @@
         B, N, _ = hidden_states.shape
         D = self.inner_dim
 
+        mask_given = encoder_attention_mask
+        removed_at = -math.inf
         if encoder_attention_mask is not None and encoder_attention_mask.ndim == 2:
             encoder_attention_mask = ((1 - encoder_attention_mask.to(dtype)) * -10000.0).unsqueeze(1)
+            removed_at = float(torch.tensor(-10000.0, dtype=dtype))
+        key_tiles = self._key_tile_bound(mask_given, encoder_attention_mask, removed_at)
 
         hidden_states = ops.gemm(hidden_states.reshape(B * N, -1), self.patchify_proj.weight,
                                  self.patchify_proj.bias).view(B, N, D)
@@ -315,14 +338,15 @@
                     encoder_hidden_states=encoder_hidden_states[keep],
                     encoder_attention_mask=None if encoder_attention_mask is None else encoder_attention_mask[keep],
                     timestep=temb[keep], cross_attention_kwargs=cross_attention_kwargs, class_labels=class_labels,
-                    skip_layer_mask=layer_mask(block_idx, keep), skip_layer_strategy=skip_layer_strategy)
+                    skip_layer_mask=layer_mask(block_idx, keep), skip_layer_strategy=skip_layer_strategy,
+                    encoder_key_tiles=None if key_tiles is None else key_tiles[keep])
                 if ltxv_model is not None and ltxv_model._interrupt:
                     return [None]
             hidden_states[B - 1].copy_(hidden_states[B - 2])
         if joint_pass and _microbatches and len(_microbatches) > 1 and first_block == 0:
             if self._run_blocks_microbatched(hidden_states, _microbatches, freqs_cis, attention_mask, encoder_hidden_states,
                                              encoder_attention_mask, temb, cross_attention_kwargs, class_labels,
-                                             layer_mask, skip_layer_strategy, ltxv_model):
+                                             layer_mask, skip_layer_strategy, ltxv_model, encoder_key_tiles=key_tiles):
                 return [None]
         elif joint_pass:
             for block_idx, block in enumerate(self.transformer_blocks):
@@ -333,7 +357,7 @@
                                       encoder_attention_mask=encoder_attention_mask, timestep=temb,
                                       cross_attention_kwargs=cross_attention_kwargs, class_labels=class_labels,
                                       skip_layer_mask=layer_mask(block_idx),
-                                      skip_layer_strategy=skip_layer_strategy)
+                                      skip_layer_strategy=skip_layer_strategy, encoder_key_tiles=key_tiles)
                 if ltxv_model is not None and ltxv_model._interrupt:
                     return [None]
         else:
@@ -344,7 +368,8 @@
                           encoder_attention_mask=encoder_attention_mask[i:i + 1], timestep=temb[i:i + 1],
                           cross_attention_kwargs=cross_attention_kwargs, class_labels=class_labels,
                           skip_layer_mask=layer_mask(block_idx, slice(i, i + 1)),
-                          skip_layer_strategy=skip_layer_strategy)
+                          skip_layer_strategy=skip_layer_strategy,
+                          encoder_key_tiles=None if key_tiles is None else key_tiles[i:i + 1])
                     if ltxv_model is not None and ltxv_model._interrupt:
                         return [None]
 
```

Result: no change. 16.72 (median of 6 runs) (+0.9%).
